# MingXiangL/AttentionShift

Measured on AMD Instinct MI355X. Metric: images/sec (1024^2, ViT-B) hot path: backbone attention fwd + attention-shift pseudo-labels, higher is better.
Workload: dtype bf16

## Files before the change

attentionshift_amd/_lib.py:

```python
import ctypes
import os

_HERE = os.path.dirname(os.path.abspath(__file__))
LIB_PATH = os.path.join(_HERE, "libattnshift_hip.so")

AS_F32, AS_BF16 = 0, 1

_c_void_p, _c_int, _c_float, _c_size_t = ctypes.c_void_p, ctypes.c_int, ctypes.c_float, ctypes.c_size_t
_c_double = ctypes.c_double

SIGNATURES = {
    "as_version": (_c_int, []),
    "as_last_error": (ctypes.c_char_p, []),
    "as_npad": (_c_int, [_c_int]),
    "as_linear_fwd": (_c_int, [_c_void_p] * 4 + [_c_int] * 5 + [_c_void_p]),
    "as_linear_small_fwd": (_c_int, [_c_void_p, _c_int, _c_void_p, _c_void_p, _c_void_p] + [_c_int] * 5 + [_c_void_p]),
    "as_linear_sk_workspace_bytes": (_c_size_t, [_c_int] * 3),
    "as_linear_sk_fwd": (_c_int, [_c_void_p] * 4 + [_c_int] * 5 + [_c_void_p, _c_size_t, _c_void_p]),
    "as_linear_gelu_fwd": (_c_int, [_c_void_p] * 5 + [_c_int] * 4 + [_c_void_p]),
    "as_linear_dgelu_fwd": (_c_int, [_c_void_p] * 4 + [_c_int] * 4 + [_c_void_p]),
    "as_deconv2x2_fwd": (_c_int, [_c_void_p] * 4 + [_c_int] * 6 + [_c_void_p]),
    "as_qkv_fwd": (_c_int, [_c_void_p] * 6 + [_c_int] * 5 + [_c_void_p]),
    "as_sdpa_fwd_workspace_bytes": (_c_size_t, [_c_int] * 4),
    "as_sdpa_fwd": (_c_int, [_c_void_p] * 6 + [_c_size_t] + [_c_int] * 4 + [_c_void_p]),
    "as_sdpa_bwd_workspace_bytes": (_c_size_t, [_c_int] * 4),
    "as_sdpa_bwd": (_c_int, [_c_void_p] * 8 + [_c_size_t] + [_c_int] * 4 + [_c_void_p]),
    "as_attn_bwd_workspace_bytes": (_c_size_t, [_c_int] * 5),
    "as_attn_bwd": (_c_int, [_c_void_p] * 15 + [_c_size_t] + [_c_int] * 5 + [_c_void_p]),
    "as_window_attn_fwd": (_c_int, [_c_void_p] * 5 + [_c_int] * 8 + [_c_void_p]),
    "as_add_layernorm_bwd_workspace_bytes": (_c_size_t, [_c_int] * 2),
    "as_add_layernorm_bwd": (_c_int, [_c_void_p] * 4 + [ctypes.c_float] + [_c_void_p] * 5 + [_c_size_t] + [_c_int] * 3 + [_c_void_p]),
    "as_add_layernorm": (_c_int, [_c_void_p] * 4 + [ctypes.c_float] + [_c_void_p] * 2 + [_c_int] * 3 + [_c_void_p]),
    "as_add_layernorm_scaled": (_c_int, [_c_void_p] * 4 + [ctypes.c_float] + [_c_void_p] * 2 + [_c_int] * 3 + [_c_void_p, _c_int, _c_void_p]),
    "as_add_layernorm_bwd_scaled": (_c_int, [_c_void_p] * 4 + [ctypes.c_float] + [_c_void_p] * 5 + [_c_size_t] + [_c_int] * 3
                                    + [_c_void_p, _c_int, _c_void_p]),
    "as_linear_splitk_workspace_bytes": (ctypes.c_size_t, [_c_int] * 3),
    "as_linear_splitk_fwd": (_c_int, [_c_void_p] * 3 + [_c_int] * 5 + [_c_void_p, ctypes.c_size_t, _c_void_p]),
    "as_linear_bwd_workspace_bytes": (ctypes.c_size_t, [_c_int] * 3),
    "as_linear_bwd": (_c_int, [_c_void_p] * 6 + [_c_int] * 5 + [_c_void_p, ctypes.c_size_t, _c_void_p]),
    "as_linear_bwd_dgelu": (_c_int, [_c_void_p] * 7 + [_c_int] * 5 + [_c_void_p, ctypes.c_size_t, _c_void_p]),
    "as_assemble_tokens": (_c_int, [_c_void_p] * 3 + [_c_int] * 5 + [_c_void_p]),
    "as_maxpool_nhwc": (_c_int, [_c_void_p] * 2 + [_c_int] * 5 + [ctypes.c_longlong, _c_void_p]),
    "as_mask_count": (_c_int, [_c_void_p] * 2 + [_c_int] * 2 + [_c_void_p]),
    "as_window_attn_bwd_workspace_bytes": (_c_size_t, [_c_int] * 5),
    "as_window_attn_bwd": (_c_int, [_c_void_p] * 8 + [_c_size_t] + [_c_int] * 8 + [_c_void_p]),
    "as_attn_fwd": (_c_int, [_c_void_p] * 12 + [_c_size_t] + [_c_int] * 5 + [_c_void_p]),
    "as_attn_mean_rows": (_c_int, [_c_void_p] * 4 + [_c_int] * 6 + [_c_void_p]),
    "as_rollout_rfrag_bytes": (_c_size_t, [_c_int] * 3),
    "as_rollout_pack": (_c_int, [_c_void_p] * 2 + [_c_int] * 4 + [_c_void_p]),
    "as_rollout_top": (_c_int, [_c_void_p] * 5 + [_c_int] * 5 + [_c_void_p]),
    "as_rollout_step_workspace_bytes": (_c_size_t, [_c_int] * 3),
    "as_rollout_step": (_c_int, [_c_void_p] * 8 + [_c_size_t] + [_c_int] * 5 + [_c_void_p]),
    "as_ccl_2d": (_c_int, [_c_void_p] * 2 + [_c_int] * 3 + [_c_void_p]),
    "as_cam_boxes_workspace_bytes": (_c_size_t, [_c_int] * 4),
    "as_cam_boxes": (_c_int, [_c_void_p] * 2 + [_c_float] * 2 + [_c_int] * 4 + [_c_void_p] * 5 + [_c_size_t, _c_void_p]),
    "as_cam_sample_masks_workspace_bytes": (_c_size_t, [_c_int] * 4),
    "as_cam_sample_masks": (_c_int, [_c_void_p] * 3 + [_c_int] * 4 + [_c_float] * 2 + [_c_void_p] * 3 + [_c_size_t, _c_void_p]),
    "as_mask_candidates_workspace_bytes": (_c_size_t, [_c_int] * 3),
    "as_mask_candidates": (_c_int, [_c_void_p] * 3 + [_c_float] * 3 + [_c_int] + [_c_void_p] * 5 + [_c_size_t]
                           + [_c_int] * 3 + [_c_void_p]),
    "as_part_select": (_c_int, [_c_void_p] * 7 + [_c_int] * 5 + [_c_void_p] * 8 + [_c_void_p]),
    "as_part_stats": (_c_int, [_c_void_p] * 3 + [_c_float] + [_c_void_p] * 4 + [_c_int] * 3 + [_c_void_p]),
    "as_filter_parts": (_c_int, [_c_void_p] * 2 + [_c_float] * 2 + [_c_void_p] + [_c_int] * 3 + [_c_void_p]),
    "as_draw_distinct": (_c_int, [_c_void_p, _c_int, _c_int] + [_c_void_p] * 5 + [_c_int] * 3 + [_c_void_p]),
    "as_mt_sample_ranks": (_c_int, [_c_void_p] * 4 + [_c_int] * 2 + [_c_void_p]),
    "as_mt_perm_ranks": (_c_int, [_c_void_p] * 4 + [_c_int] * 2 + [_c_void_p]),
    "as_small_attn_fwd": (_c_int, [_c_void_p] * 3 + [_c_int] * 5 + [_c_void_p]),
    "as_small_attn_bwd_workspace_bytes": (_c_size_t, [_c_int] * 3),
    "as_small_attn_bwd": (_c_int, [_c_void_p] * 6 + [_c_size_t] + [_c_int] * 5 + [_c_void_p]),
    "as_roi_align_fwd": (_c_int, [_c_void_p] * 3 + [_c_int] * 6 + [_c_float] + [_c_int] * 2 + [_c_void_p]),
    "as_roi_align_bwd": (_c_int, [_c_void_p] * 3 + [_c_int] * 6 + [_c_float] + [_c_int] * 2 + [_c_void_p]),
    "as_chamfer_2d_fwd": (_c_int, [_c_void_p] * 6 + [_c_int] * 3 + [_c_void_p]),
    "as_chamfer_2d_bwd": (_c_int, [_c_void_p] * 8 + [_c_int] * 3 + [_c_void_p]),
    "as_merge_plan": (_c_int, [_c_void_p] * 4 + [_c_int] * 2 + [_c_void_p]),
    "as_semantic_prestage": (_c_int, [_c_void_p, _c_float] + [_c_int] * 5 + [_c_void_p] * 4),
    "as_cosine_shift_workspace_bytes": (_c_size_t, [_c_int] * 6),
    "as_cosine_shift": (_c_int, [_c_void_p] * 5 + [_c_double] * 2 + [_c_int] + [_c_void_p] * 4 + [_c_size_t]
                        + [_c_int] * 6 + [_c_void_p]),
    "as_cosine_shift_strided": (_c_int, [_c_void_p, ctypes.c_longlong] + [_c_void_p] * 4 + [_c_double] * 2 + [_c_int] + [_c_void_p] * 4
                                + [_c_size_t] + [_c_int] * 6 + [_c_void_p]),
    "as_refine_similarity_workspace_bytes": (_c_size_t, [_c_int] * 3),
    "as_refine_similarity": (_c_int, [_c_void_p] * 3 + [_c_int] * 3 + [_c_float, _c_int] + [_c_void_p] * 3
                             + [_c_size_t] + [_c_int] * 3 + [_c_void_p]),
    "as_instance_maps_workspace_bytes": (_c_size_t, [_c_int] * 2),
    "as_crop_threshold_erode_workspace_bytes": (_c_size_t, [_c_int] * 3),
    "as_crop_threshold_erode": (_c_int, [_c_void_p] * 2 + [_c_float, _c_int, _c_int] + [_c_void_p] * 3 + [_c_size_t]
                                + [_c_int] * 3 + [_c_void_p]),
    "as_rank_select_workspace_bytes": (_c_size_t, [_c_int] * 2),
    "as_rank_select": (_c_int, [_c_void_p] * 4 + [_c_size_t] + [_c_int] * 3 + [_c_void_p]),
    "as_rank_select_xy": (_c_int, [_c_void_p] * 4 + [_c_size_t] + [_c_int] * 5 + [_c_void_p]),
    "as_merge_parts": (_c_int, [_c_void_p] * 2 + [_c_float] + [_c_void_p] * 3 + [_c_int] * 4 + [_c_void_p]),
    "as_select_median_boxes": (_c_int, [_c_void_p] * 2 + [_c_int] * 2 + [_c_void_p] * 8 + [_c_int, _c_void_p]),
    "as_rank_draw_xy": (_c_int, [_c_void_p, _c_int] + [_c_void_p] * 4 + [_c_int, _c_int, ctypes.c_int64, _c_int, _c_void_p, _c_size_t]
                        + [_c_int] * 5 + [_c_void_p]),
    "as_instance_maps": (_c_int, [_c_void_p] * 2 + [_c_int] * 6 + [_c_void_p] * 3 + [_c_size_t, _c_void_p]),
    "as_nms_workspace_bytes": (_c_size_t, [_c_int]),
    "as_nms": (_c_int, [_c_void_p, _c_int, _c_float, _c_int] + [_c_void_p] * 3 + [_c_size_t, _c_void_p]),
    "as_paste_masks": (_c_int, [_c_void_p] * 4 + [_c_int] * 8 + [_c_float, _c_void_p]),
    "as_rle_tile": (_c_int, [_c_void_p] * 2),
    "as_rle_workspace_bytes": (_c_size_t, [_c_int] * 3),
    "as_rle_count": (_c_int, [_c_void_p] + [_c_int] * 3 + [_c_void_p] * 2 + [_c_size_t, _c_void_p]),
    "as_rle_encode": (_c_int, [_c_void_p] + [_c_int] * 3 + [_c_void_p] * 2 + [_c_size_t, _c_void_p, _c_size_t, _c_void_p, _c_size_t,
                               _c_void_p, _c_void_p]),
    "as_rpn_candidates_workspace_bytes": (_c_size_t, [_c_int] * 2),
    "as_rpn_candidates": (_c_int, [_c_void_p] + [_c_int] * 3 + [_c_void_p] * 2 + [_c_int, _c_float, _c_void_p, _c_float, _c_int]
                          + [_c_void_p] * 7 + [_c_size_t, _c_void_p]),
    "as_rpn_assign_workspace_bytes": (_c_size_t, [_c_int] * 3),
    "as_rpn_assign": (_c_int, [_c_void_p] + [_c_int] * 3 + [_c_void_p] * 3 + [_c_int] * 2 + [_c_void_p] + [_c_float] * 3
                      + [_c_int] * 2 + [_c_void_p] * 4 + [_c_size_t, _c_void_p]),
    "as_rpn_sample": (_c_int, [_c_int] * 4 + [_c_void_p] * 4 + [_c_size_t, _c_void_p, _c_void_p]),
    "as_rpn_targets": (_c_int, [_c_void_p] + [_c_int] * 3 + [_c_void_p] * 3 + [_c_int] + [_c_void_p] * 2 + [_c_int] * 2
                       + [_c_void_p] * 3 + [_c_void_p]),
}


class RpnLevel(ctypes.Structure):
    _fields_ = [("cls", _c_void_p), ("reg", _c_void_p), ("H", _c_int), ("W", _c_int), ("stride_x", _c_int), ("stride_y", _c_int)]

_lib = None


class AttnShiftError(RuntimeError):
    pass


def load():
    global _lib
    if _lib is not None:
        return _lib
    if not os.path.exists(LIB_PATH):
        raise AttnShiftError(
            f"{LIB_PATH} is missing: build it with `python -m attentionshift_amd.csrc.build` "
            "(hipcc --offload-arch=gfx950).  There is no CPU fallback for the hot path.")
    lib = ctypes.CDLL(LIB_PATH)
    for name, (res, args) in SIGNATURES.items():
        fn = getattr(lib, name)
        fn.restype, fn.argtypes = res, args
    _lib = lib
    return lib


def check(rc, what):
    if rc != 0:
        msg = load().as_last_error()
        raise AttnShiftError(f"{what} failed (rc={rc}): {msg.decode() if msg else ''}")
```

attentionshift_amd/backbone.py:

```python
import math
import os

import torch
import torch.nn as nn
import torch.nn.functional as F

from . import ops
from .registry import BACKBONES


def trunc_normal_(tensor, std=0.02):
    return nn.init.trunc_normal_(tensor, std=std, a=-2 * std, b=2 * std)


class Mlp(nn.Module):
    def __init__(self, dim, hidden):
        super().__init__()
        self.fc1 = nn.Linear(dim, hidden)
        self.fc2 = nn.Linear(hidden, dim)


class Attention(nn.Module):
    def __init__(self, dim, num_heads, qkv_bias):
        super().__init__()
        self.num_heads = num_heads
        self.qkv = nn.Linear(dim, dim * 3, bias=qkv_bias)
        self.proj = nn.Linear(dim, dim)


class Block(nn.Module):

    def __init__(self, dim, num_heads, mlp_ratio, qkv_bias, eps):
        super().__init__()
        self.norm1 = nn.LayerNorm(dim, eps=eps)
        self.attn = Attention(dim, num_heads, qkv_bias)
        self.norm2 = nn.LayerNorm(dim, eps=eps)
        self.mlp = Mlp(dim, int(dim * mlp_ratio))


class PatchEmbed(nn.Module):
    def __init__(self, img_size, patch_size, in_chans, embed_dim):
        super().__init__()
        if isinstance(img_size, int):
            img_size = [img_size, img_size]
        self.num_patches = (img_size[0] // patch_size) * (img_size[1] // patch_size)
        self.patch_size = patch_size
        self.proj = nn.Conv2d(in_chans, embed_dim, kernel_size=patch_size, stride=patch_size)


class MLP(nn.Module):

    def __init__(self, input_dim, hidden_dim, output_dim, num_layers):
        super().__init__()
        self.num_layers = num_layers
        h = [hidden_dim] * (num_layers - 1)
        self.layers = nn.ModuleList(nn.Linear(n, k) for n, k in zip([input_dim] + h, h + [output_dim]))

    def forward(self, x):
        for i, layer in enumerate(self.layers):
            x = F.relu(layer(x)) if i < self.num_layers - 1 else layer(x)
        return x


class DeferredFPN:

    def __init__(self, backbone, features, taps):
        self._bb, self._features, self._taps = backbone, list(features), list(taps)
        self._out, self._event, self._joined = None, None, False

    def launch(self):
        if self._out is not None:
            return self
        bb = self._bb
        main = torch.cuda.current_stream()
        if bb._fpn_stream is None:
            bb._fpn_stream = torch.cuda.Stream()
        side = bb._fpn_stream
        side.wait_stream(main)
        with torch.cuda.stream(side):
            for t in self._features + self._taps:
                t.record_stream(side)
            self._out = tuple(bb._fpn(i, self._features[i], self._taps[i]) for i in range(len(self._features)))
            self._event = side.record_event()
        return self

    def result(self):
        self.launch()
        if not self._joined:
            main = torch.cuda.current_stream()
            main.wait_event(self._event)
            for t in self._out:
                t.record_stream(main)
            self._joined = True
            self._features, self._taps = [], []
        return self._out

    def __len__(self):
        return len(self._features) if self._out is None else len(self._out)

    def __iter__(self):
        return iter(self.result())

    def __getitem__(self, i):
        return self.result()[i]


@BACKBONES.register_module()
class VisionTransformerDet(nn.Module):
    def __init__(self, img_size, patch_size, embed_dim, in_chans=3, with_fpn=True, frozen_stages=-1,
                 out_indices=(3, 5, 7, 11), use_checkpoint=False, learnable_pos_embed=True, last_feat=False,
                 recompute_last_feat=False, point_tokens_num=100, num_classes=20, return_attention=False,
                 with_point_head=True, depth=12, num_heads=12, mlp_ratio=4., qkv_bias=False, qk_scale=None,
                 drop_rate=0., attn_drop_rate=0., drop_path_rate=0., norm_eps=1e-6, init_values=0,
                 compute_dtype=torch.bfloat16, **unused):
        super().__init__()
        assert not with_fpn or patch_size in (8, 16)
        assert not recompute_last_feat or last_feat
        if qk_scale is not None or attn_drop_rate or drop_rate or init_values:
            raise NotImplementedError("qk_scale / dropout / layer-scale are unused by every reference config")
        if embed_dim != num_heads * ops.HEAD_DIM:
            raise NotImplementedError(f"head dim must be {ops.HEAD_DIM}")
        self.embed_dim = self.num_features = embed_dim
        self.patch_size, self.depth, self.num_heads = patch_size, depth, num_heads
        self.last_feat, self.recompute_last_feat = last_feat, recompute_last_feat
        self.with_fpn, self.frozen_stages = with_fpn, frozen_stages
        self.out_indices = tuple(out_indices)
        self.use_checkpoint = use_checkpoint
        self.drop_path_rate = drop_path_rate
        self.return_attention = return_attention
        self.point_tokens_num = point_tokens_num
        self.with_point_head = with_point_head
        self.compute_dtype = compute_dtype
        self.defer_fpn = bool(unused.pop("defer_fpn", False))
        self._fpn_stream = None
        self._point_pack = None
        self.point_head_stream = bool(unused.pop("point_head_stream", False))
        self._point_stream = None

        self.patch_embed = PatchEmbed(img_size, patch_size, in_chans, embed_dim)
        n_patches = self.patch_embed.num_patches
        self.cls_token = nn.Parameter(torch.zeros(1, 1, embed_dim))
        self.pos_embed = nn.Parameter(torch.zeros(1, n_patches + 1, embed_dim), requires_grad=learnable_pos_embed)
        self.blocks = nn.ModuleList(Block(embed_dim, num_heads, mlp_ratio, qkv_bias, norm_eps) for _ in range(depth))
        if with_fpn and patch_size == 16:
            self.fpn1 = nn.Sequential(nn.ConvTranspose2d(embed_dim, embed_dim, 2, 2), nn.BatchNorm2d(embed_dim), nn.GELU(),
                                      nn.ConvTranspose2d(embed_dim, embed_dim, 2, 2))
            self.fpn2 = nn.Sequential(nn.ConvTranspose2d(embed_dim, embed_dim, 2, 2))
            self.fpn3 = nn.Identity()
            self.fpn4 = nn.MaxPool2d(2, 2)
        elif with_fpn and patch_size == 8:
            self.fpn1 = nn.Sequential(nn.ConvTranspose2d(embed_dim, embed_dim, 2, 2))
            self.fpn2 = nn.Identity()
            self.fpn3 = nn.Sequential(nn.MaxPool2d(2, 2))
            self.fpn4 = nn.Sequential(nn.MaxPool2d(4, 4))
        self.point_token = nn.Parameter(torch.zeros(1, point_tokens_num, embed_dim))
        self.point_pos_embed = nn.Parameter(torch.zeros(1, point_tokens_num, embed_dim))
        if with_point_head:
            self.class_embed = MLP(embed_dim, embed_dim, num_classes, 3)
            self.bbox_embed = MLP(embed_dim, embed_dim, 2, 3)
        trunc_normal_(self.pos_embed)
        trunc_normal_(self.cls_token)
        trunc_normal_(self.point_token)
        trunc_normal_(self.point_pos_embed)
        self.apply(self._init_weights)
        self._wcache = {}

    @staticmethod
    def _init_weights(m):
        if isinstance(m, nn.Linear):
            trunc_normal_(m.weight)
            if m.bias is not None:
                nn.init.constant_(m.bias, 0)
        elif isinstance(m, nn.LayerNorm):
            nn.init.constant_(m.bias, 0)
            nn.init.constant_(m.weight, 1.0)

    def init_weights(self, pretrained=None):
        if pretrained is not None and not isinstance(pretrained, str):
            raise TypeError("pretrained must be a str or None")
        self.apply(self._init_weights)
        if isinstance(pretrained, str):
            import os
            if os.path.isfile(pretrained):
                from .checkpoint import load_checkpoint
                load_checkpoint(self, pretrained, strict=False)
            else:
                print(f"checkpoint path {pretrained} is invalid, we skip it and initialize net randomly")
        self.invalidate_cache()

    def train(self, mode=True):
        super().train(mode)
        self._freeze_stages()
        return self

    def _freeze_stages(self):
        if self.frozen_stages >= 0:
            self.patch_embed.eval()
            for p in self.patch_embed.parameters():
                p.requires_grad = False
            self.cls_token.requires_grad = False
            self.pos_embed.requires_grad = False
        for i in range(1, self.frozen_stages + 1):
            m = self.blocks[i - 1]
            m.eval()
            for p in m.parameters():
                p.requires_grad = False

    def invalidate_cache(self):
        self._wcache = {}

    def _w(self, p):
        if p.dtype == self.compute_dtype:
            return p
        if torch.is_grad_enabled() and p.requires_grad:
            return p.to(self.compute_dtype)
        key = id(p)
        hit = self._wcache.get(key)
        if hit is None or hit[0] != p._version or hit[1].device != p.device:
            hit = (p._version, p.detach().to(self.compute_dtype).contiguous())
            self._wcache[key] = hit
        return hit[1]

    def _derived(self, p, tag, fn):
        if torch.is_grad_enabled() and p.requires_grad:
            return fn(p).to(self.compute_dtype).contiguous()
        key = (id(p), tag)
        hit = self._wcache.get(key)
        if hit is None or hit[0] != p._version or hit[1].device != p.device:
            hit = (p._version, fn(p.detach()).to(self.compute_dtype).contiguous())
            self._wcache[key] = hit
        return hit[1]

    def _deconv2x2(self, x_nhwc, conv, bn=None, act="none"):
        B, h, w, cin = x_nhwc.shape
        cout = conv.weight.shape[1]
        srcs = [conv.weight, conv.bias] + ([bn.weight, bn.bias, bn.running_mean, bn.running_var] if bn is not None else [])
        stamp = tuple(-1 if t is None else t._version for t in srcs) + (x_nhwc.device,)
        key = (id(conv), "deconv")
        hit = self._wcache.get(key)
        if hit is None or hit[0] != stamp:
            with torch.no_grad():
                wmat = conv.weight.detach().float().permute(2, 3, 1, 0).reshape(4 * cout, cin)
                bias = torch.zeros(cout, device=wmat.device) if conv.bias is None else conv.bias.detach().float()
                if bn is not None:
                    scale = bn.weight.detach().float() * torch.rsqrt(bn.running_var.float() + bn.eps)
                    wmat = wmat * scale.repeat(4)[:, None]
                    bias = (bias - bn.running_mean.float()) * scale + bn.bias.detach().float()
                hit = (stamp, wmat.to(self.compute_dtype).contiguous(), bias.repeat(4).contiguous())
            self._wcache[key] = hit
        _, wmat, bias4 = hit
        if x_nhwc.is_cuda and self.compute_dtype == torch.bfloat16 and cin % 32 == 0 and cout % 8 == 0:
            return ops.deconv2x2(x_nhwc.contiguous(), wmat, bias4, act=act)
        y = ops.linear(x_nhwc.reshape(B * h * w, cin), wmat, bias4, act=act)
        return y.reshape(B, h, w, 2, 2, cout).permute(0, 1, 3, 2, 4, 5).reshape(B, 2 * h, 2 * w, cout)

    def _deconv2x2_train(self, x_nhwc, conv):
        B, h, w, cin = x_nhwc.shape
        cout = conv.weight.shape[1]
        cd = self.compute_dtype
        from .autograd import linear_in
        wmat = conv.weight.permute(2, 3, 1, 0).reshape(4 * cout, cin)
        bias = None if conv.bias is None else conv.bias.repeat(4)
        y = linear_in(x_nhwc.reshape(B * h * w, cin), wmat, bias, cd)
        return y.reshape(B, h, w, 2, 2, cout).permute(0, 1, 3, 2, 4, 5).reshape(B, 2 * h, 2 * w, cout)

    def _fpn_train(self, i, feat_nchw, tok):
        B, D, hp, wp = feat_nchw.shape
        op = [self.fpn1, self.fpn2, self.fpn3, self.fpn4][i]
        if isinstance(op, nn.Sequential) and isinstance(op[0], nn.ConvTranspose2d):
            y = self._deconv2x2_train(tok.to(self.compute_dtype).reshape(B, hp, wp, D), op[0]).permute(0, 3, 1, 2)
            if len(op) == 4:
                y = op[2](op[1](y.float())).to(self.compute_dtype)
                y = self._deconv2x2_train(y.permute(0, 2, 3, 1), op[3]).permute(0, 3, 1, 2)
            return y
        return op(feat_nchw)

    def _fpn(self, i, feat_nchw, tok):
        B, D, hp, wp = feat_nchw.shape
        ops_ = [self.fpn1, self.fpn2, self.fpn3, self.fpn4]
        op = ops_[i]
        if isinstance(op, nn.Sequential) and isinstance(op[0], nn.ConvTranspose2d):
            x0 = tok.to(self.compute_dtype).reshape(B, hp, wp, D)
            if len(op) == 4:
                bn = op[1]
                if isinstance(bn, nn.modules.batchnorm._BatchNorm) and not bn.training and bn.running_mean is not None \
                        and isinstance(op[2], nn.GELU) and getattr(op[2], "approximate", "none") == "none":
                    y = self._deconv2x2(x0, op[0], bn=bn, act="gelu")
                else:
                    y = self._deconv2x2(x0, op[0]).permute(0, 3, 1, 2)
                    y = op[2](op[1](y.float())).to(self.compute_dtype).permute(0, 2, 3, 1)
                return self._deconv2x2(y, op[3]).permute(0, 3, 1, 2)
            return self._deconv2x2(x0, op[0]).permute(0, 3, 1, 2)
        pool = op[0] if isinstance(op, nn.Sequential) and len(op) == 1 else op
        if isinstance(pool, nn.MaxPool2d) and tok.is_cuda and tok.dtype == torch.float32 and tok.stride()[1:] == (D, 1):
            k = pool.kernel_size if isinstance(pool.kernel_size, int) else pool.kernel_size[0]
            s_ = pool.stride if isinstance(pool.stride, int) else pool.stride[0]
            if k == s_ and pool.padding in (0, (0, 0)) and not pool.ceil_mode and hp % k == 0 and wp % k == 0 and D % 4 == 0:
                return ops.maxpool_nhwc(tok.reshape(B, hp, wp, D), k).permute(0, 3, 1, 2)
        return op(feat_nchw)

    def _point_head_packable(self, x):
        ls = list(self.class_embed.layers) + list(self.bbox_embed.layers)
        return (len(self.class_embed.layers) == 3 and len(self.bbox_embed.layers) == 3 and hasattr(torch, "_addmm_activation")
                and all(l.weight.dtype == x.dtype and l.bias is not None for l in ls)
                and self.class_embed.layers[0].in_features == self.bbox_embed.layers[0].in_features)

    def _point_head_packed(self, x):
        c, b = self.class_embed.layers, self.bbox_embed.layers
        key = tuple((t.data_ptr(), t._version) for t in (c[0].weight, c[0].bias, b[0].weight, b[0].bias))
        pk = self._point_pack
        if pk is None or pk["key"] != key:
            with torch.no_grad():
                w1 = torch.cat((c[0].weight, b[0].weight)).contiguous()
                pk = dict(key=key, w1=w1, w1t=w1.t().contiguous(), b1=torch.cat((c[0].bias, b[0].bias)))
            self._point_pack = pk
        B, T, D = x.shape
        hc = c[0].out_features
        x2 = x.reshape(B * T, D)
        if ops.linear_small_applies(x2, pk["w1"]) and hc % 16 == 0 and hc >= 64:
            h1 = ops.linear_small(x2, pk["w1"], pk["b1"], act="relu")
            h2c = ops.linear_small(h1[:, :hc], c[1].weight, c[1].bias, act="relu")
            h2b = ops.linear_small(h1[:, hc:], b[1].weight, b[1].bias, act="relu")
            cls = ops.linear_small(h2c, c[2].weight, c[2].bias).reshape(B, T, -1)
            reg = ops.linear_small(h2b, b[2].weight, b[2].bias, act="sigmoid").reshape(B, T, -1)
            return cls, reg
        h1 = torch._addmm_activation(pk["b1"], x2, pk["w1t"])
        h2c = torch._addmm_activation(c[1].bias, h1[:, :hc], c[1].weight.t())
        h2b = torch._addmm_activation(b[1].bias, h1[:, hc:], b[1].weight.t())
        cls = torch.addmm(c[2].bias, h2c, c[2].weight.t()).reshape(B, T, -1)
        reg = torch.addmm(b[2].bias, h2b, b[2].weight.t()).reshape(B, T, -1).sigmoid()
        return cls, reg

    def interpolate_pos_encoding(self, n_patch_tokens, w, h):
        n0 = self.pos_embed.shape[1] - 1
        if n_patch_tokens == n0 and w == h:
            return self.pos_embed
        dim = self.pos_embed.shape[-1]
        w0, h0 = w // self.patch_size + 0.1, h // self.patch_size + 0.1
        s = int(math.sqrt(n0))
        grid = self.pos_embed[:, 1:].reshape(1, s, s, dim).permute(0, 3, 1, 2)
        grid = F.interpolate(grid, scale_factor=(w0 / math.sqrt(n0), h0 / math.sqrt(n0)), mode="bicubic")
        assert int(w0) == grid.shape[-2] and int(h0) == grid.shape[-1]
        return torch.cat((self.pos_embed[:, :1], grid.permute(0, 2, 3, 1).reshape(1, -1, dim)), dim=1)

    def prepare_tokens(self, img):
        B, C, w, h = img.shape
        ps = self.patch_size
        hp, wp = w // ps, h // ps
        patches = torch.empty(B, hp, wp, C, ps, ps, device=img.device, dtype=self.compute_dtype)
        patches.copy_(img.reshape(B, C, hp, ps, wp, ps).permute(0, 2, 4, 1, 3, 5))
        wmat = self._derived(self.patch_embed.proj.weight, "patch", lambda t: t.reshape(self.embed_dim, -1))
        emb = ops.linear(patches.view(B, hp * wp, C * ps * ps), wmat, self.patch_embed.proj.bias.float())
        return ops.assemble_tokens(emb, self._token_table(hp * wp, w, h))

    def _token_table(self, Np, w, h):
        srcs = (self.pos_embed, self.cls_token, self.point_token, self.point_pos_embed)
        stamp = tuple(t._version for t in srcs) + (Np, w, h, self.pos_embed.device)
        hit = self._wcache.get("token_table")
        if hit is None or hit[0] != stamp:
            with torch.no_grad():
                pos = self.interpolate_pos_encoding(Np, w, h)
                table = torch.cat((self.cls_token + pos[:, :1], pos[:, 1:], self.point_token + self.point_pos_embed), dim=1)
            hit = (stamp, table[0].float().contiguous())
            self._wcache["token_table"] = hit
        return hit[1]

    def _block(self, blk, x, delta, keep_state, need_x, on_full=None, full_out=None, x_out=None):
        cd = self.compute_dtype
        x, y = ops.add_layernorm(x, delta, blk.norm1.weight, blk.norm1.bias, blk.norm1.eps, cd,
                                 x_out=full_out if delta is not None else None)
        if on_full is not None:
            on_full(x)
        a, st = ops.attention_fwd(y, self._w(blk.attn.qkv.weight),
                                  None if blk.attn.qkv.bias is None else blk.attn.qkv.bias.float(),
                                  self._w(blk.attn.proj.weight), blk.attn.proj.bias.float(), self.num_heads,
                                  keep_state=keep_state)
        x, z = ops.add_layernorm(x, a, blk.norm2.weight, blk.norm2.bias, blk.norm2.eps, cd)
        z = ops.linear(z, self._w(blk.mlp.fc1.weight), blk.mlp.fc1.bias.float(), act="gelu")
        z = ops.linear(z, self._w(blk.mlp.fc2.weight), blk.mlp.fc2.bias.float())
        if need_x:
            x, _ = ops.add_layernorm(x, z, None, None, 0.0, cd, want_y=False, x_out=x_out)
            z = None
        return x, z, st

    def _grad_path(self):
        return torch.is_grad_enabled() and self.training and any(p.requires_grad for p in self.blocks.parameters())

    def _drop_path(self, x, i):
        rate = self.drop_path_rate * i / max(self.depth - 1, 1)
        if rate == 0.0 or not self.training:
            return x
        keep = 1.0 - rate
        mask = torch.rand(x.shape[0], 1, 1, device=x.device, dtype=x.dtype).add_(keep).floor_()
        return x / keep * mask

    def _drop_scale(self, batch, i, device):
        rate = self.drop_path_rate * i / max(self.depth - 1, 1)
        if rate == 0.0 or not self.training:
            return None
        keep = 1.0 - rate
        return torch.rand(batch, device=device, dtype=torch.float32).add_(keep).floor_().div_(keep)

    def _prepare_tokens_train(self, img):
        B, C, w, h = img.shape
        ps = self.patch_size
        hp, wp = w // ps, h // ps
        cd = self.compute_dtype
        patches = img.reshape(B, C, hp, ps, wp, ps).permute(0, 2, 4, 1, 3, 5).reshape(B, hp * wp, C * ps * ps)
        from .autograd import linear_in
        x = linear_in(patches.to(cd), self.patch_embed.proj.weight.reshape(self.embed_dim, -1), self.patch_embed.proj.bias,
                      cd).float()
        x = torch.cat((self.cls_token.expand(B, -1, -1), x), dim=1)
        x = x + self.interpolate_pos_encoding(x.shape[1] - 1, w, h)
        pt = (self.point_token + self.point_pos_embed).expand(B, -1, -1)
        return torch.cat((x, pt), dim=1)

    def _block_train(self, blk, x, delta, i, sink, delta_scale=None):
        from . import autograd as AG
        cd = self.compute_dtype
        sh = self._train_shadow
        w = lambda p: sh[id(p)] if id(p) in sh else p.to(cd)
        x, y = AG.add_layernorm(x, delta, blk.norm1.weight, blk.norm1.bias, blk.norm1.eps, cd, delta_scale)
        a = AG.attention(y, w(blk.attn.qkv.weight), None if blk.attn.qkv.bias is None else blk.attn.qkv.bias.float(),
                         w(blk.attn.proj.weight), blk.attn.proj.bias.float(), self.num_heads, sink)
        x, z = AG.add_layernorm(x, a, blk.norm2.weight, blk.norm2.bias, blk.norm2.eps, cd, self._drop_scale(x.shape[0], i, x.device))
        if AG.mlp_applies(z, w(blk.mlp.fc1.weight), w(blk.mlp.fc2.weight)):
            z = AG.mlp(z, w(blk.mlp.fc1.weight), blk.mlp.fc1.bias, w(blk.mlp.fc2.weight), blk.mlp.fc2.bias)
        elif AG.linear_applies(z, w(blk.mlp.fc1.weight)):
            z = F.gelu(AG.linear(z, w(blk.mlp.fc1.weight), blk.mlp.fc1.bias))
            z = AG.linear(z, w(blk.mlp.fc2.weight), blk.mlp.fc2.bias)
        else:
            z = F.gelu(F.linear(z, w(blk.mlp.fc1.weight), w(blk.mlp.fc1.bias)))
            z = F.linear(z, w(blk.mlp.fc2.weight), w(blk.mlp.fc2.bias))
        return x, z, self._drop_scale(x.shape[0], i, x.device)

    def forward(self, x):
        B, _, H, W = x.shape
        hp, wp = H // self.patch_size, W // self.patch_size
        T = self.point_tokens_num
        grad_path = self._grad_path()
        x = self._prepare_tokens_train(x) if grad_path else self.prepare_tokens(x)
        if self.recompute_last_feat:
            last_feat = x
        features, taps, attns = [], [], []
        store = []
        delta = None
        dscale = None
        if not grad_path:
            x = x.contiguous()

        def take_tap(xf):
            taps.append(xf[:, 1:-T])
            tap = xf[:, 1:, :][:, :-T].permute(0, 2, 1).unflatten(2, (hp, wp))
            if grad_path:
                features.append(tap if os.environ.get("AS_TAP_VIEW", "1") != "0" else tap.contiguous())
                return
            if xf.data_ptr() != tap_slot(len(features)).data_ptr():
                tap_slot(len(features)).copy_(xf)
            features.append(store[0][len(features)][:, 1:-T].unflatten(1, (hp, wp)).permute(0, 3, 1, 2))

        def tap_slot(k):
            if not store:
                store.append(torch.empty(len(self.out_indices), *x.shape, device=x.device, dtype=torch.float32))
            return store[0][k]

        tap_due = False
        nblk = len(self.blocks)
        self._train_shadow = {}
        if grad_path and self.compute_dtype != torch.float32 and not os.environ.get("AS_NO_PARAM_SHADOW"):
            from .autograd import cast_params
            from . import autograd as _AG
            lib_mlp = _AG._LIBRARY_LINEAR or self.embed_dim % 32 != 0
            ps = []
            for blk in self.blocks:
                ps += [blk.attn.qkv.weight, blk.attn.proj.weight, blk.mlp.fc1.weight, blk.mlp.fc2.weight]
                if lib_mlp:
                    ps += [blk.mlp.fc1.bias, blk.mlp.fc2.bias]
            self._train_shadow = cast_params([p for p in ps if p.dtype != self.compute_dtype], self.compute_dtype)
        for i, blk in enumerate(self.blocks):
            if grad_path:
                sink = [] if self.return_attention else None
                x, delta, dscale = self._block_train(blk, x.float() if x.dtype != torch.float32 else x, delta, i, sink, dscale)
                if i in self.out_indices or i == nblk - 1:
                    x = x + (delta if dscale is None else delta * dscale[:, None, None])
                    delta, dscale = None, None
                st = sink[0] if sink else None
                if i in self.out_indices:
                    take_tap(x)
            else:
                last_tap = i in self.out_indices and i == nblk - 1
                x, delta, st = self._block(blk, x, delta, self.return_attention, i == nblk - 1,
                                           take_tap if tap_due else None,
                                           full_out=tap_slot(len(features)) if tap_due and x.dtype == torch.float32 else None,
                                           x_out=tap_slot(len(features) + int(tap_due)) if last_tap and x.dtype == torch.float32
                                           else None)
                tap_due = i in self.out_indices and i != nblk - 1
                if i in self.out_indices and i == nblk - 1:
                    take_tap(x)
            if self.return_attention:
                attns.append(st)
            if self.last_feat and not self.recompute_last_feat and i == nblk - 1:
                last_feat = x[:, :-T]
        self._train_shadow = {}
        org_features = store[0][:, :, 1:-T].unflatten(2, (hp, wp)).permute(1, 0, 4, 2, 3) if store else None
        if org_features is None:
            org_features = torch.stack(features, dim=1)
        if self.with_fpn and grad_path:
            features = [self._fpn_train(i, features[i], taps[i]) for i in range(len(features))]
        elif self.with_fpn and self.defer_fpn and x.is_cuda:
            features = DeferredFPN(self, features, taps)
        elif self.with_fpn:
            features = [self._fpn(i, features[i], taps[i]) for i in range(len(features))]
        point_tokens = x[:, -T:]
        out = dict(org_feats=org_features, feature=features if isinstance(features, DeferredFPN) else tuple(features),
                   point_tokens=point_tokens)
        if self.with_point_head and not grad_path and point_tokens.is_cuda and self._point_head_packable(point_tokens):
            if self.point_head_stream:
                if self._point_stream is None:
                    self._point_stream = torch.cuda.Stream()
                main = torch.cuda.current_stream()
                self._point_stream.wait_stream(main)
                with torch.cuda.stream(self._point_stream):
                    cls, reg = self._point_head_packed(point_tokens)
                    out["point_head_ready"] = self._point_stream.record_event()
                for t in (point_tokens, cls, reg):
                    t.record_stream(main)
                    t.record_stream(self._point_stream)
            else:
                cls, reg = self._point_head_packed(point_tokens)
            out.update(outputs_class=cls, outputs_coord=reg)
        elif self.with_point_head:
            out.update(outputs_class=self.class_embed(point_tokens), outputs_coord=self.bbox_embed(point_tokens).sigmoid())
        if self.return_attention and self.last_feat:
            out.update(attns=attns)
        if self.last_feat:
            out.update(last_feat=last_feat)
        return out
```

attentionshift_amd/csrc/layernorm.hip:

```cpp
#include "common.h"

namespace {

template <typename T, int VPL>
__global__ __launch_bounds__(256) void add_layernorm_kernel(const float* __restrict__ x_in, const T* __restrict__ delta,
                                                            const float* __restrict__ gamma, const float* __restrict__ beta,
                                                            float* __restrict__ x_out, T* __restrict__ y_out, int M, int D,
                                                            float eps, const float* __restrict__ dscale, int rps) {
  const int row = blockIdx.x * 4 + (threadIdx.x >> 6), lane = threadIdx.x & 63;
  if (row >= M) return;
  const size_t base = (size_t)row * D;
  const float ds = dscale != nullptr ? dscale[row / rps] : 1.0f;
  float v[VPL][4];
  float s = 0.0f;
#pragma unroll
  for (int i = 0; i < VPL; ++i) {
    const int c = (i * 64 + lane) * 4;
    if (c < D) {
      const float4 a = *reinterpret_cast<const float4*>(x_in + base + c);
      v[i][0] = a.x; v[i][1] = a.y; v[i][2] = a.z; v[i][3] = a.w;
      if (delta != nullptr) {
#pragma unroll
        for (int t = 0; t < 4; ++t) v[i][t] = dscale != nullptr ? fmaf(ds, to_f32<T>(delta[base + c + t]), v[i][t])
                                                                     : v[i][t] + to_f32<T>(delta[base + c + t]);
      }
      s += (v[i][0] + v[i][1]) + (v[i][2] + v[i][3]);
    } else {
      v[i][0] = v[i][1] = v[i][2] = v[i][3] = 0.0f;
    }
  }
  const float mean = wave_sum(s) / (float)D;
  float q = 0.0f;
#pragma unroll
  for (int i = 0; i < VPL; ++i) {
    const int c = (i * 64 + lane) * 4;
    if (c < D) {
#pragma unroll
      for (int t = 0; t < 4; ++t) {
        const float d = v[i][t] - mean;
        q = fmaf(d, d, q);
      }
    }
  }
  const float rstd = rsqrtf(wave_sum(q) / (float)D + eps);
#pragma unroll
  for (int i = 0; i < VPL; ++i) {
    const int c = (i * 64 + lane) * 4;
    if (c < D) {
      if (x_out != nullptr) *reinterpret_cast<float4*>(x_out + base + c) = make_float4(v[i][0], v[i][1], v[i][2], v[i][3]);
      if (y_out != nullptr) {
        const float4 g = *reinterpret_cast<const float4*>(gamma + c);
        const float4 b = *reinterpret_cast<const float4*>(beta + c);
        const float y0 = (v[i][0] - mean) * rstd * g.x + b.x, y1 = (v[i][1] - mean) * rstd * g.y + b.y;
        const float y2 = (v[i][2] - mean) * rstd * g.z + b.z, y3 = (v[i][3] - mean) * rstd * g.w + b.w;
        T* yp = y_out + base + c;
        yp[0] = from_f32<T>(y0); yp[1] = from_f32<T>(y1); yp[2] = from_f32<T>(y2); yp[3] = from_f32<T>(y3);
      }
    }
  }
}

template <typename T>
int launch_add_ln(const float* x_in, const void* delta, const float* gamma, const float* beta, float* x_out, void* y_out,
                  int M, int D, float eps, const float* dscale, int rps, hipStream_t s) {
  const int vpl = as_ceil_div(D, 256);
  dim3 grid(as_ceil_div(M, 4));
#define AS_LN(V)                                                                                                   \
  hipLaunchKernelGGL((add_layernorm_kernel<T, V>), grid, dim3(256), 0, s, x_in, (const T*)delta, gamma, beta, x_out, \
                     (T*)y_out, M, D, eps, dscale, rps)
  switch (vpl) {
    case 1: AS_LN(1); break;
    case 2: AS_LN(2); break;
    case 3: AS_LN(3); break;
    case 4: AS_LN(4); break;
    case 5: AS_LN(5); break;
    case 6: AS_LN(6); break;
    case 7: AS_LN(7); break;
    case 8: AS_LN(8); break;
    case 9: case 10: AS_LN(10); break;
    case 11: case 12: AS_LN(12); break;
    default: AS_REQUIRE(false, AS_E_UNSUPPORTED, "as_add_layernorm: D=%d (max 3072)", D);
  }
#undef AS_LN
  AS_CHECK_LAUNCH("add_layernorm");
  return AS_OK;
}

}

namespace {

template <typename T, int VPL>
__global__ __launch_bounds__(256) void add_layernorm_bwd_kernel(const float* __restrict__ x, const T* __restrict__ dy,
                                                                const float* __restrict__ dx_res,
                                                                const float* __restrict__ gamma, float* __restrict__ dx_out,
                                                                T* __restrict__ ddelta_out, float* __restrict__ part, int M,
                                                                int D, float eps, const float* __restrict__ dscale, int rps) {
  __shared__ float red[2][4][VPL * 256];
  const int wave = threadIdx.x >> 6, lane = threadIdx.x & 63;
  float dg[VPL][4], db[VPL][4], gm[VPL][4];
#pragma unroll
  for (int i = 0; i < VPL; ++i) {
    const int c = (i * 64 + lane) * 4;
#pragma unroll
    for (int t = 0; t < 4; ++t) { dg[i][t] = 0.0f; db[i][t] = 0.0f; gm[i][t] = (gamma != nullptr && c < D) ? gamma[c + t] : 1.0f; }
  }
  for (int row = blockIdx.x * 4 + wave; row < M; row += gridDim.x * 4) {
    const size_t base = (size_t)row * D;
    float v[VPL][4], g[VPL][4];
    float s = 0.0f;
#pragma unroll
    for (int i = 0; i < VPL; ++i) {
      const int c = (i * 64 + lane) * 4;
      if (c < D) {
        const float4 a = *reinterpret_cast<const float4*>(x + base + c);
        v[i][0] = a.x; v[i][1] = a.y; v[i][2] = a.z; v[i][3] = a.w;
        if (dy == nullptr) {
#pragma unroll
          for (int t = 0; t < 4; ++t) g[i][t] = 0.0f;
        } else if constexpr (sizeof(T) == 2) {
          const bf16x4 d4 = *reinterpret_cast<const bf16x4*>(dy + base + c);
#pragma unroll
          for (int t = 0; t < 4; ++t) g[i][t] = (float)d4[t];
        } else {
          const float4 d4 = *reinterpret_cast<const float4*>(dy + base + c);
          g[i][0] = d4.x; g[i][1] = d4.y; g[i][2] = d4.z; g[i][3] = d4.w;
        }
        s += (v[i][0] + v[i][1]) + (v[i][2] + v[i][3]);
      } else {
#pragma unroll
        for (int t = 0; t < 4; ++t) { v[i][t] = 0.0f; g[i][t] = 0.0f; }
      }
    }
    const float mean = wave_sum(s) / (float)D;
    float q = 0.0f;
#pragma unroll
    for (int i = 0; i < VPL; ++i) {
      const int c = (i * 64 + lane) * 4;
      if (c < D) {
#pragma unroll
        for (int t = 0; t < 4; ++t) { const float d = v[i][t] - mean; q = fmaf(d, d, q); }
      }
    }
    const float rstd = rsqrtf(wave_sum(q) / (float)D + eps);
    float sg = 0.0f, sgx = 0.0f;
#pragma unroll
    for (int i = 0; i < VPL; ++i) {
      const int c = (i * 64 + lane) * 4;
      if (c < D) {
#pragma unroll
        for (int t = 0; t < 4; ++t) {
          const float xh = (v[i][t] - mean) * rstd;
          dg[i][t] = fmaf(g[i][t], xh, dg[i][t]);
          db[i][t] += g[i][t];
          const float gg = g[i][t] * gm[i][t];
          g[i][t] = gg;
          v[i][t] = xh;
          sg += gg;
          sgx = fmaf(gg, xh, sgx);
        }
      }
    }
    const float mg = wave_sum(sg) / (float)D, mgx = wave_sum(sgx) / (float)D;
#pragma unroll
    for (int i = 0; i < VPL; ++i) {
      const int c = (i * 64 + lane) * 4;
      if (c < D) {
        float o[4];
        float4 r4 = make_float4(0.0f, 0.0f, 0.0f, 0.0f);
        if (dx_res != nullptr) r4 = *reinterpret_cast<const float4*>(dx_res + base + c);
        const float r[4] = {r4.x, r4.y, r4.z, r4.w};
#pragma unroll
        for (int t = 0; t < 4; ++t) {
          o[t] = rstd * (g[i][t] - mg - v[i][t] * mgx);
          if (dx_res != nullptr) o[t] += r[t];
        }
        if (dx_out != nullptr) *reinterpret_cast<float4*>(dx_out + base + c) = make_float4(o[0], o[1], o[2], o[3]);
        if (ddelta_out != nullptr) {
          const float ds = dscale != nullptr ? dscale[row / rps] : 1.0f;
          if constexpr (sizeof(T) == 2) {
            bf16x4 w4;
#pragma unroll
            for (int t = 0; t < 4; ++t) w4[t] = (__bf16)(ds * o[t]);
            *reinterpret_cast<bf16x4*>(ddelta_out + base + c) = w4;
          } else {
            *reinterpret_cast<float4*>(ddelta_out + base + c) = make_float4(ds * o[0], ds * o[1], ds * o[2], ds * o[3]);
          }
        }
      }
    }
  }
#pragma unroll
  for (int i = 0; i < VPL; ++i)
#pragma unroll
    for (int t = 0; t < 4; ++t) {
      red[0][wave][(i * 64 + lane) * 4 + t] = dg[i][t];
      red[1][wave][(i * 64 + lane) * 4 + t] = db[i][t];
    }
  __syncthreads();
  for (int c = threadIdx.x; c < D; c += 256) {
    part[((size_t)blockIdx.x * 2 + 0) * D + c] = ((red[0][0][c] + red[0][1][c]) + red[0][2][c]) + red[0][3][c];
    part[((size_t)blockIdx.x * 2 + 1) * D + c] = ((red[1][0][c] + red[1][1][c]) + red[1][2][c]) + red[1][3][c];
  }
}

__global__ __launch_bounds__(1024) void add_layernorm_bwd_reduce_kernel(const float* __restrict__ part,
                                                                        float* __restrict__ dgamma, float* __restrict__ dbeta,
                                                                        int nblk, int D) {
  __shared__ float red[16][64];
  const int cl = threadIdx.x & 63, grp = threadIdx.x >> 6, c = blockIdx.x * 64 + cl, which = blockIdx.y;
  float a0 = 0.0f, a1 = 0.0f, a2 = 0.0f, a3 = 0.0f;
  if (c < D) {
    int i = grp;
    for (; i + 48 < nblk; i += 64) {
      a0 += part[((size_t)i * 2 + which) * D + c];
      a1 += part[((size_t)(i + 16) * 2 + which) * D + c];
      a2 += part[((size_t)(i + 32) * 2 + which) * D + c];
      a3 += part[((size_t)(i + 48) * 2 + which) * D + c];
    }
    for (; i < nblk; i += 16) a0 += part[((size_t)i * 2 + which) * D + c];
  }
  red[grp][cl] = (a0 + a1) + (a2 + a3);
  __syncthreads();
  if (grp != 0 || c >= D) return;
  float t = 0.0f;
#pragma unroll
  for (int g = 0; g < 16; ++g) t += red[g][cl];
  float* dst = which == 0 ? dgamma : dbeta;
  if (dst != nullptr) dst[c] = t;
}

constexpr int LNB_BLOCKS = 1024;

template <typename T>
int launch_add_ln_bwd(const float* x, const void* dy, const float* dx_res, const float* gamma, float* dx_out, void* ddelta,
                      float* dgamma, float* dbeta, float* part, int M, int D, float eps, const float* dscale, int rps,
                      hipStream_t s) {
  const int vpl = as_ceil_div(D, 256);
  const int nblk = as_ceil_div(M, 4) < LNB_BLOCKS ? as_ceil_div(M, 4) : LNB_BLOCKS;
#define AS_LNB(V)                                                                                                    \
  hipLaunchKernelGGL((add_layernorm_bwd_kernel<T, V>), dim3(nblk), dim3(256), 0, s, x, (const T*)dy, dx_res, gamma, dx_out, \
                     (T*)ddelta, part, M, D, eps, dscale, rps)
  switch (vpl) {
    case 1: AS_LNB(1); break;
    case 2: AS_LNB(2); break;
    case 3: AS_LNB(3); break;
    case 4: AS_LNB(4); break;
    case 5: AS_LNB(5); break;
    case 6: AS_LNB(6); break;
    case 7: AS_LNB(7); break;
    case 8: AS_LNB(8); break;
    default: AS_REQUIRE(false, AS_E_UNSUPPORTED, "as_add_layernorm_bwd: D=%d (max 2048)", D);
  }
#undef AS_LNB
  AS_CHECK_LAUNCH("add_layernorm_bwd");
  if (dgamma != nullptr || dbeta != nullptr) {
    hipLaunchKernelGGL(add_layernorm_bwd_reduce_kernel, dim3(as_ceil_div(D, 64), 2), dim3(1024), 0, s, (const float*)part,
                       dgamma, dbeta, nblk, D);
    AS_CHECK_LAUNCH("add_layernorm_bwd_reduce");
  }
  return AS_OK;
}

}

extern "C" size_t as_add_layernorm_bwd_workspace_bytes(int M, int D) {
  if (M <= 0 || D <= 0) return 0;
  return (size_t)LNB_BLOCKS * 2 * D * sizeof(float);
}

extern "C" int as_add_layernorm_bwd(const float* x, const void* dy, const float* dx_res, const float* gamma, float eps,
                                    float* dx_out, void* ddelta_out, float* dgamma, float* dbeta, void* workspace,
                                    size_t workspace_bytes, int M, int D, int dtype, as_stream_t stream) {
  return as_add_layernorm_bwd_scaled(x, dy, dx_res, gamma, eps, dx_out, ddelta_out, dgamma, dbeta, workspace, workspace_bytes,
                                     M, D, dtype, nullptr, 1, stream);
}

extern "C" int as_add_layernorm_bwd_scaled(const float* x, const void* dy, const float* dx_res, const float* gamma, float eps,
                                           float* dx_out, void* ddelta_out, float* dgamma, float* dbeta, void* workspace,
                                           size_t workspace_bytes, int M, int D, int dtype, const float* delta_scale,
                                           int rows_per_scale, as_stream_t stream) {
  AS_REQUIRE(x && (dy || dx_res) && (dx_out || ddelta_out) && workspace, AS_E_BADARG, "as_add_layernorm_bwd: null pointer");
  AS_REQUIRE(rows_per_scale > 0, AS_E_BADARG, "as_add_layernorm_bwd: rows_per_scale must be positive");
  AS_REQUIRE(M > 0 && D > 0 && D % 4 == 0, AS_E_BADARG, "as_add_layernorm_bwd: need M > 0 and D %% 4 == 0 (D=%d)", D);
  AS_REQUIRE(workspace_bytes >= as_add_layernorm_bwd_workspace_bytes(M, D), AS_E_WORKSPACE,
             "as_add_layernorm_bwd: workspace too small");
  hipStream_t s = (hipStream_t)stream;
  if (dtype == AS_BF16)
    return launch_add_ln_bwd<__bf16>(x, dy, dx_res, gamma, dx_out, ddelta_out, dgamma, dbeta, (float*)workspace, M, D, eps,
                                     delta_scale, rows_per_scale, s);
  if (dtype == AS_F32)
    return launch_add_ln_bwd<float>(x, dy, dx_res, gamma, dx_out, ddelta_out, dgamma, dbeta, (float*)workspace, M, D, eps,
                                    delta_scale, rows_per_scale, s);
  AS_REQUIRE(false, AS_E_UNSUPPORTED, "as_add_layernorm_bwd: dtype %d", dtype);
}

extern "C" int as_add_layernorm(const float* x_in, const void* delta, const float* gamma, const float* beta, float eps,
                                float* x_out, void* y_out, int M, int D, int dtype, as_stream_t stream) {
  return as_add_layernorm_scaled(x_in, delta, gamma, beta, eps, x_out, y_out, M, D, dtype, nullptr, 1, stream);
}

extern "C" int as_add_layernorm_scaled(const float* x_in, const void* delta, const float* gamma, const float* beta, float eps,
                                       float* x_out, void* y_out, int M, int D, int dtype, const float* delta_scale,
                                       int rows_per_scale, as_stream_t stream) {
  AS_REQUIRE(x_in && (x_out || y_out), AS_E_BADARG, "as_add_layernorm: null pointer");
  AS_REQUIRE(rows_per_scale > 0 && (!delta_scale || delta), AS_E_BADARG, "as_add_layernorm: delta_scale needs delta, rows_per_scale > 0");
  AS_REQUIRE(!y_out || (gamma && beta), AS_E_BADARG, "as_add_layernorm: y_out needs gamma and beta");
  AS_REQUIRE(M > 0 && D > 0 && D % 4 == 0, AS_E_BADARG, "as_add_layernorm: need M > 0 and D %% 4 == 0 (D=%d)", D);
  hipStream_t s = (hipStream_t)stream;
  if (dtype == AS_BF16) return launch_add_ln<__bf16>(x_in, delta, gamma, beta, x_out, y_out, M, D, eps, delta_scale, rows_per_scale, s);
  if (dtype == AS_F32) return launch_add_ln<float>(x_in, delta, gamma, beta, x_out, y_out, M, D, eps, delta_scale, rows_per_scale, s);
  AS_REQUIRE(false, AS_E_UNSUPPORTED, "as_add_layernorm: dtype %d", dtype);
}


namespace {
__global__ __launch_bounds__(256) void maxpool_nhwc_kernel(const float* __restrict__ x, float* __restrict__ out, int B, int H,
                                                           int W, int C, int k, size_t xbs) {
  const int Ho = H / k, Wo = W / k, C4 = C >> 2;
  const size_t total = (size_t)B * Ho * Wo * C4;
  for (size_t i = (size_t)blockIdx.x * blockDim.x + threadIdx.x; i < total; i += (size_t)gridDim.x * blockDim.x) {
    const int c4 = (int)(i % C4);
    size_t r = i / C4;
    const int ow = (int)(r % Wo);
    r /= Wo;
    const int oh = (int)(r % Ho), b = (int)(r / Ho);
    const float* src = x + (size_t)b * xbs + (((size_t)oh * k) * W + (size_t)ow * k) * C + c4 * 4;
    float4 m = *reinterpret_cast<const float4*>(src);
    for (int dy = 0; dy < k; ++dy)
      for (int dx = 0; dx < k; ++dx) {
        const float4 v = *reinterpret_cast<const float4*>(src + ((size_t)dy * W + dx) * C);
        m.x = (v.x > m.x || v.x != v.x) ? v.x : m.x; m.y = (v.y > m.y || v.y != v.y) ? v.y : m.y;
        m.z = (v.z > m.z || v.z != v.z) ? v.z : m.z; m.w = (v.w > m.w || v.w != v.w) ? v.w : m.w;
      }
    *reinterpret_cast<float4*>(out + i * 4) = m;
  }
}
}

extern "C" int as_maxpool_nhwc(const float* x, float* out, int B, int H, int W, int C, int k, long long x_batch_stride,
                               as_stream_t stream) {
  AS_REQUIRE(x && out, AS_E_BADARG, "as_maxpool_nhwc: null pointer");
  AS_REQUIRE(B > 0 && H > 0 && W > 0 && C > 0 && k > 0, AS_E_BADARG, "as_maxpool_nhwc: bad sizes");
  AS_REQUIRE(x_batch_stride >= (long long)H * W * C && x_batch_stride % 4 == 0, AS_E_BADARG,
             "as_maxpool_nhwc: batch stride %lld (elements) must be >= H*W*C and a multiple of 4", x_batch_stride);
  AS_REQUIRE(C % 4 == 0 && H % k == 0 && W % k == 0, AS_E_UNSUPPORTED,
             "as_maxpool_nhwc: C %% 4 == 0 and H, W multiples of k only (C=%d H=%d W=%d k=%d)", C, H, W, k);
  const size_t total = (size_t)B * (H / k) * (W / k) * (C / 4);
  const int grid = (int)((total + 255) / 256 < 4096 ? (total + 255) / 256 : 4096);
  hipLaunchKernelGGL(maxpool_nhwc_kernel, dim3(grid), dim3(256), 0, (hipStream_t)stream, x, out, B, H, W, C, k,
                     (size_t)x_batch_stride);
  AS_CHECK_LAUNCH("maxpool_nhwc");
  return AS_OK;
}

namespace {
template <typename T>
__global__ __launch_bounds__(256) void assemble_tokens_kernel(const T* __restrict__ emb, const float* __restrict__ table,
                                                              float* __restrict__ out, int B, int Np, int N, int D) {
  const int D4 = D >> 2;
  const size_t total = (size_t)B * N * D4;
  for (size_t i = (size_t)blockIdx.x * blockDim.x + threadIdx.x; i < total; i += (size_t)gridDim.x * blockDim.x) {
    const int c = (int)(i % D4) * 4;
    const size_t r = i / D4;
    const int n = (int)(r % N), b = (int)(r / N);
    float4 v = *reinterpret_cast<const float4*>(table + (size_t)n * D + c);
    if (n >= 1 && n <= Np) {
      const T* e = emb + ((size_t)b * Np + (n - 1)) * D + c;
      if (sizeof(T) == 2) {
        const bf16x4 e4 = *reinterpret_cast<const bf16x4*>(e);
        v.x = (float)e4[0] + v.x; v.y = (float)e4[1] + v.y; v.z = (float)e4[2] + v.z; v.w = (float)e4[3] + v.w;
      } else {
        const float4 e4 = *reinterpret_cast<const float4*>(e);
        v.x = e4.x + v.x; v.y = e4.y + v.y; v.z = e4.z + v.z; v.w = e4.w + v.w;
      }
    }
    *reinterpret_cast<float4*>(out + i * 4) = v;
  }
}
}

extern "C" int as_assemble_tokens(const void* emb, const float* table, float* out, int B, int Np, int N, int D, int dtype,
                                  as_stream_t stream) {
  AS_REQUIRE(emb && table && out, AS_E_BADARG, "as_assemble_tokens: null pointer");
  AS_REQUIRE(B > 0 && Np > 0 && N > Np && D > 0 && D % 4 == 0, AS_E_BADARG, "as_assemble_tokens: B=%d Np=%d N=%d D=%d", B, Np, N, D);
  const size_t total = (size_t)B * N * (D / 4);
  const int grid = (int)((total + 255) / 256 < 8192 ? (total + 255) / 256 : 8192);
  if (dtype == AS_BF16)
    hipLaunchKernelGGL(assemble_tokens_kernel<__bf16>, dim3(grid), dim3(256), 0, (hipStream_t)stream, (const __bf16*)emb, table, out,
                       B, Np, N, D);
  else if (dtype == AS_F32)
    hipLaunchKernelGGL(assemble_tokens_kernel<float>, dim3(grid), dim3(256), 0, (hipStream_t)stream, (const float*)emb, table, out,
                       B, Np, N, D);
  else
    AS_REQUIRE(false, AS_E_UNSUPPORTED, "as_assemble_tokens: dtype %d", dtype);
  AS_CHECK_LAUNCH("assemble_tokens");
  return AS_OK;
}
```

attentionshift_amd/csrc/rollout.hip:

```cpp
#include <stdlib.h>
#include "common.h"
#include "lds_asm.h"

namespace {

constexpr int HD = 64, RO_NT = 256;
constexpr float LOG2E = 1.44269504088896340736f;

template <typename T> struct KjCfg { static constexpr int PITCH = HD * (int)sizeof(T) + 16; };

__device__ __forceinline__ size_t rf_slot(int b, int nkb, int i, int k) {
  const int rem = k & 31, s2 = rem >> 4, r16 = rem & 15;
  const int lane = (i & 31) + 32 * ((r16 & 7) >> 2), t = (r16 >> 3) * 4 + (r16 & 3);
  return ((((((size_t)b * nkb + (k >> 5)) * 4 + (i >> 5)) * 2 + s2) * 64) + lane) * 8 + t;
}
__device__ __forceinline__ size_t rf_frag(int b, int nkb, int kb, int ib, int s2, int lane) {
  return ((((((size_t)b * nkb + kb) * 4 + ib) * 2 + s2) * 64) + lane) * 8;
}

template <typename T>
__device__ __forceinline__ f32x16 pbar_tile(const T* __restrict__ q, const T* __restrict__ k,
                                            const float* __restrict__ lse, const char* kj_lds, int b, int h,
                                            int N, int Npad, int i0, int j0, int li, int half) {
  f32x16 pbar;
#pragma unroll
  for (int r = 0; r < 16; ++r) pbar[r] = 0.0f;
  const int irow = min(i0 + li, N - 1);
  const int jrow = min(j0 + li, N - 1);
  for (int hh = 0; hh < h; ++hh) {
    const size_t bh = (size_t)b * h + hh;
    f32x16 s;
#pragma unroll
    for (int r = 0; r < 16; ++r) s[r] = 0.0f;
#pragma unroll
    for (int ks = 0; ks < 4; ++ks) {
      Frag<T> fa, fb;
      fa.load16B(q + qf_frag(bh, Npad, irow, ks, half));
      if (kj_lds != nullptr)
        fb.load16B(reinterpret_cast<const T*>(kj_lds + ((size_t)hh * 32 + li) * KjCfg<T>::PITCH) + ks * 16 + half * 8);
      else
        fb.load16B(k + (bh * Npad + jrow) * HD + ks * 16 + half * 8);
      s = mma32(fa, fb, s);
    }
    const float* lrow = lse + bh * N;
#pragma unroll
    for (int r = 0; r < 16; ++r) {
      const int row = min(i0 + acc_row(r, half), N - 1);
      pbar[r] += __builtin_amdgcn_exp2f(s[r] - lrow[row] * LOG2E);
    }
  }
  const float inv_h = 1.0f / (float)h;
#pragma unroll
  for (int r = 0; r < 16; ++r) pbar[r] *= inv_h;
  return pbar;
}

template <typename T, bool TOP>
__global__ __launch_bounds__(RO_NT) void attn_mean_rows_kernel(const T* __restrict__ q, const T* __restrict__ k,
                                                               const float* __restrict__ lse,
                                                               float* __restrict__ out, T* __restrict__ rf_out, int B,
                                                               int N, int Npad, int h, int row0, int nrows) {
  const int lane = threadIdx.x & 63, wave = threadIdx.x >> 6;
  const int li = lane & 31, half = lane >> 5;
  const int jb = blockIdx.x * 4 + wave, ib = blockIdx.y, b = blockIdx.z;
  const int j0 = jb * 32, i0 = ib * 32;
  if (j0 >= N) return;
  const f32x16 p = pbar_tile<T>(q, k, lse, nullptr, b, h, N, Npad, row0 + i0, j0, li, half);
  const int j = j0 + li;
  const int nkb = (N + 31) / 32;
#pragma unroll
  for (int r = 0; r < 16; ++r) {
    const int i = i0 + acc_row(r, half);
    float v = p[r];
    if (TOP) v = 0.5f * (v + ((row0 + i) == j ? 1.0f : 0.0f));
    const bool live = i < nrows && j < N;
    if (live) out[((size_t)b * nrows + i) * N + j] = v;
    if (rf_out != nullptr && i < 128) rf_out[rf_slot(b, nkb, i, j)] = from_f32<T>(live ? v : 0.0f);
  }
}

template <typename T> struct Kj2 {
  static constexpr int PITCH = sizeof(T) == 2 ? 128 : (HD * 4 + 16);
  __device__ static __forceinline__ int off(int row, int elem) {
    if (sizeof(T) == 2) return row * 128 + ((((elem >> 3) ^ (row & 7))) << 4);
    return row * PITCH + elem * 4;
  }
};

template <typename T, int HPW>
__global__ __launch_bounds__(RO_NT) void rollout_step2_kernel(const T* __restrict__ q, const T* __restrict__ k,
                                                              const float* __restrict__ lse,
                                                              const float* __restrict__ Rin, const T* __restrict__ rf_in,
                                                              float* __restrict__ Rout, T* __restrict__ rf_out,
                                                              float* __restrict__ part, int B, int N, int Npad, int h,
                                                              int Trows, int nsplit, int xbufs) {
  extern __shared__ __attribute__((aligned(16))) char smem[];
  constexpr bool PREFETCH = sizeof(T) == 2;
  const int tid = threadIdx.x, lane = tid & 63, wave = tid >> 6;
  const int li = lane & 31, half = lane >> 5;
  const int j0 = blockIdx.x * 32, b = blockIdx.y, split = blockIdx.z;
  char* kj = smem;
  float4* xchg = reinterpret_cast<float4*>(smem + (size_t)h * 32 * Kj2<T>::PITCH);

  {
    constexpr int CPR = HD * (int)sizeof(T) / 16;
    const int total = h * 32 * CPR;
    for (int c = tid; c < total; c += RO_NT) {
      const int hh = c / (32 * CPR), rem = c % (32 * CPR);
      const int jr = rem / CPR, ch = rem % CPR;
      const int jrow = min(j0 + jr, N - 1);
      const uint4 u = *reinterpret_cast<const uint4*>(
          reinterpret_cast<const char*>(k + (((size_t)b * h + hh) * Npad + jrow) * HD) + ch * 16);
      const int elem = ch * (16 / (int)sizeof(T));
      const int base = Kj2<T>::off(hh * 32 + jr, elem & ~7);
      *reinterpret_cast<uint4*>(kj + base + (elem & 7) * (int)sizeof(T)) = u;
    }
  }
  __syncthreads();

  const int nkb = (N + 31) / 32;
  const float inv_h = 1.0f / (float)h;
  const bool own_rows = wave * 32 < Trows;

  f32x16 acc;
#pragma unroll
  for (int r = 0; r < 16; ++r) acc[r] = 0.0f;

  struct Fetch {
    Frag<T> fq[HPW][4];
    float l8[HPW];
    Frag<T> fr[2];
  };
  auto fetch = [&](int kb, Fetch& f) {
    const int row = min(kb * 32 + li, N - 1);
#pragma unroll
    for (int t = 0; t < HPW; ++t) {
      const int hh = min(wave + 4 * t, h - 1);
#pragma unroll
      for (int ks = 0; ks < 4; ++ks) f.fq[t][ks].load16B(q + qf_frag((size_t)b * h + hh, Npad, row, ks, half));
      f.l8[t] = -LOG2E * lse[((size_t)b * h + hh) * N + row];
    }
    if (own_rows) {
#pragma unroll
      for (int s2 = 0; s2 < 2; ++s2) f.fr[s2].load16B(rf_in + rf_frag(b, nkb, kb, wave, s2, lane));
    }
  };
  const int kb0 = (int)((long long)nkb * split / nsplit), kb1 = (int)((long long)nkb * (split + 1) / nsplit);
  Fetch cur, nxt;
  if (PREFETCH && kb0 < kb1) fetch(kb0, nxt);

  for (int kb = kb0; kb < kb1; ++kb) {
    const int k0 = kb * 32;
    if (PREFETCH) {
      cur = nxt;
      if (kb + 1 < kb1) fetch(kb + 1, nxt);
    } else {
      fetch(kb, cur);
    }

    f32x16 pbar;
#pragma unroll
    for (int r = 0; r < 16; ++r) pbar[r] = 0.0f;
#pragma unroll
    for (int t = 0; t < HPW; ++t) {
      const int hh = wave + 4 * t;
      if (hh < h) {
        const float l8 = cur.l8[t];
        f32x16 sc;
#pragma unroll
        for (int r = 0; r < 16; ++r) sc[r] = 0.0f;
        sc = __builtin_amdgcn_mfma_f32_32x32x2f32(half == 0 ? l8 : 0.0f, 1.0f, sc, 0, 0, 0);
#pragma unroll
        for (int ks = 0; ks < 4; ++ks) {
          Frag<T> fk;
          fk.load16B(reinterpret_cast<const T*>(kj + Kj2<T>::off(hh * 32 + li, ks * 16 + half * 8)));
          sc = mma32(cur.fq[t][ks], fk, sc);
        }
#pragma unroll
        for (int r = 0; r < 16; ++r) pbar[r] += __builtin_amdgcn_exp2f(sc[r]);
      }
    }
    float4* slab = xchg + (size_t)(xbufs == 2 ? (kb - kb0) & 1 : 0) * 4 * 4 * 64;
#pragma unroll
    for (int g = 0; g < 4; ++g)
      slab[(wave * 4 + g) * 64 + lane] = make_float4(pbar[4 * g], pbar[4 * g + 1], pbar[4 * g + 2], pbar[4 * g + 3]);
    __syncthreads();
    if (own_rows) {
      Frag<T> fp[2];
#pragma unroll
      for (int g = 0; g < 4; ++g) {
        float4 v = slab[(0 * 4 + g) * 64 + lane];
#pragma unroll
        for (int w = 1; w < 4; ++w) {
          const float4 u = slab[(w * 4 + g) * 64 + lane];
          v.x += u.x; v.y += u.y; v.z += u.z; v.w += u.w;
        }
        const float e[4] = {v.x, v.y, v.z, v.w};
#pragma unroll
        for (int x = 0; x < 4; ++x) {
          const int r = 4 * g + x;
          const bool live = k0 + acc_row(r, half) < N;
          fp[r >> 3].set(r & 7, live ? e[x] * inv_h : 0.0f);
        }
      }
#pragma unroll
      for (int s2 = 0; s2 < 2; ++s2) acc = mma32(cur.fr[s2], fp[s2], acc);
    }
    if (xbufs == 1) __syncthreads();
  }

  if (own_rows) {
    const int j = j0 + li;
#pragma unroll
    for (int r = 0; r < 16; ++r) {
      const int i = wave * 32 + acc_row(r, half);
      const bool live = i < Trows && j < N;
      if (nsplit > 1) {
        if (live) part[(((size_t)split * B + b) * Trows + i) * N + j] = acc[r];
        continue;
      }
      float v = 0.0f;
      if (live) {
        const size_t idx = ((size_t)b * Trows + i) * N + j;
        v = 0.5f * (acc[r] + Rin[idx]);
        Rout[idx] = v;
      }
      if (rf_out != nullptr) rf_out[rf_slot(b, nkb, i, j)] = from_f32<T>(v);
    }
  }
}

#ifndef AS_ROLLOUT_ABLATE
#define AS_ROLLOUT_ABLATE 0
#endif
template <typename T> __device__ __forceinline__ f32x16 inject_rows(float x, int half);
template <> __device__ __forceinline__ f32x16 inject_rows<float>(float x, int half) {
  f32x16 z;
#pragma unroll
  for (int r = 0; r < 16; ++r) z[r] = 0.0f;
  return __builtin_amdgcn_mfma_f32_32x32x2f32(half == 0 ? x : 0.0f, 1.0f, z, 0, 0, 0);
}
template <> __device__ __forceinline__ f32x16 inject_rows<__bf16>(float x, int half) {
  f32x16 z;
#pragma unroll
  for (int r = 0; r < 16; ++r) z[r] = 0.0f;
  x = half == 0 ? x : 0.0f;
  const __bf16 hi = (__bf16)x;
  const float r1 = x - (float)hi;
  const __bf16 mid = (__bf16)r1;
  const __bf16 lo = (__bf16)(r1 - (float)mid);
  const __bf16 zero = (__bf16)0.0f, one = (__bf16)1.0f;
  Frag<__bf16> fa, fb;
  fa.v = bf16x8{hi, mid, lo, zero, zero, zero, zero, zero};
  fb.v = bf16x8{one, one, one, zero, zero, zero, zero, zero};
  return mma32(fa, fb, z);
}

template <typename T>
__global__ __launch_bounds__(RO_NT, 3) void rollout_step3_kernel(const T* __restrict__ q, const T* __restrict__ k,
                                                                 const float* __restrict__ lse,
                                                                 const float* __restrict__ Rin, const T* __restrict__ rf_in,
                                                                 float* __restrict__ Rout, T* __restrict__ rf_out,
                                                                 float* __restrict__ part, int B, int N, int Npad, int h,
                                                                 int Trows, int nsplit) {
  extern __shared__ __attribute__((aligned(16))) char smem[];
  const int tid = threadIdx.x, lane = tid & 63, wave = tid >> 6;
  const int li = lane & 31, half = lane >> 5;
  const int j0 = blockIdx.x * 32, b = blockIdx.y, split = blockIdx.z;
  char* kj = smem;
  {
    constexpr int CPR = HD * (int)sizeof(T) / 16;
    const int total = h * 32 * CPR;
    for (int c = tid; c < total; c += RO_NT) {
      const int hh = c / (32 * CPR), rem = c % (32 * CPR);
      const int jr = rem / CPR, ch = rem % CPR;
      const int jrow = min(j0 + jr, N - 1);
      const uint4 u = *reinterpret_cast<const uint4*>(
          reinterpret_cast<const char*>(k + (((size_t)b * h + hh) * Npad + jrow) * HD) + ch * 16);
      const int elem = ch * (16 / (int)sizeof(T));
      const int base = Kj2<T>::off(hh * 32 + jr, elem & ~7);
      *reinterpret_cast<uint4*>(kj + base + (elem & 7) * (int)sizeof(T)) = u;
    }
  }
  __syncthreads();

  const int nkb = (N + 31) / 32;
  const int nib = (Trows + 31) / 32;
  const float inv_h = 1.0f / (float)h;
  const int kb0 = (int)((long long)nkb * split / nsplit), kb1 = (int)((long long)nkb * (split + 1) / nsplit);

  f32x16 acc[4];
#pragma unroll
  for (int ib = 0; ib < 4; ++ib)
#pragma unroll
    for (int r = 0; r < 16; ++r) acc[ib][r] = 0.0f;

  for (int kb = kb0 + wave; kb < kb1; kb += 4) {
    const int k0 = kb * 32;
    const int row = min(k0 + li, N - 1);
    Frag<T> fq[4];
    float l8;
#pragma unroll
    for (int ks = 0; ks < 4; ++ks) fq[ks].load16B(q + qf_frag((size_t)b * h, Npad, row, ks, half));
    l8 = -LOG2E * lse[((size_t)b * h) * N + row];
    f32x16 pbar;
#pragma unroll
    for (int r = 0; r < 16; ++r) pbar[r] = 0.0f;
    auto head = [&](int hh) {
      f32x16 sc = inject_rows<T>(AS_ROLLOUT_ABLATE == 3 ? 0.0f : l8, half);
#pragma unroll
      for (int ks = 0; ks < 4; ++ks) {
        Frag<T> fk;
        fk.load16B(reinterpret_cast<const T*>(kj + Kj2<T>::off(hh * 32 + li, ks * 16 + half * 8)));
        if (AS_ROLLOUT_ABLATE != 4) sc = mma32(fq[ks], fk, sc);
        else sc[ks] += (float)fk.v[0];
      }
#pragma unroll
      for (int r = 0; r < 16; ++r) pbar[r] += AS_ROLLOUT_ABLATE == 2 ? sc[r] : __builtin_amdgcn_exp2f(sc[r]);
    };
    for (int hh = 0; hh + 1 < h; ++hh) {
      Frag<T> fn[4];
#pragma unroll
      for (int ks = 0; ks < 4; ++ks) {
        if (AS_ROLLOUT_ABLATE == 1) fn[ks] = fq[ks];
        else fn[ks].load16B(q + qf_frag((size_t)b * h + hh + 1, Npad, row, ks, half));
      }
      const float l8n = AS_ROLLOUT_ABLATE == 1 ? l8 : -LOG2E * lse[((size_t)b * h + hh + 1) * N + row];
      head(hh);
#pragma unroll
      for (int ks = 0; ks < 4; ++ks) fq[ks] = fn[ks];
      l8 = l8n;
    }
    Frag<T> fr[4][2];
#pragma unroll
    for (int ib = 0; ib < 4; ++ib) {
      const int ibc = min(ib, nib - 1);
#pragma unroll
      for (int s2 = 0; s2 < 2; ++s2) fr[ib][s2].load16B(rf_in + rf_frag(b, nkb, kb, ibc, s2, lane));
    }
    head(h - 1);
    Frag<T> fp[2];
#pragma unroll
    for (int r = 0; r < 16; ++r) {
      const bool live = k0 + acc_row(r, half) < N;
      fp[r >> 3].set(r & 7, live ? pbar[r] * inv_h : 0.0f);
    }
#pragma unroll
    for (int ib = 0; ib < 4; ++ib)
      if (ib < nib) {
#pragma unroll
        for (int s2 = 0; s2 < 2; ++s2) acc[ib] = mma32(fr[ib][s2], fp[s2], acc[ib]);
      }
  }

  float* red = reinterpret_cast<float*>(smem);
  f32x16 mine;
#pragma unroll
  for (int r = 0; r < 16; ++r) mine[r] = 0.0f;
#pragma unroll
  for (int pass = 0; pass < 2; ++pass) {
    __syncthreads();
#pragma unroll
    for (int x = 0; x < 2; ++x)
#pragma unroll
      for (int r = 0; r < 16; ++r) red[((wave * 2 + x) * 16 + r) * 64 + lane] = acc[pass * 2 + x][r];
    __syncthreads();
    if ((wave >> 1) == pass) {
      const int x = wave & 1;
#pragma unroll
      for (int r = 0; r < 16; ++r)
        mine[r] = ((red[((0 * 2 + x) * 16 + r) * 64 + lane] + red[((1 * 2 + x) * 16 + r) * 64 + lane]) +
                   red[((2 * 2 + x) * 16 + r) * 64 + lane]) + red[((3 * 2 + x) * 16 + r) * 64 + lane];
    }
  }
  if (wave * 32 < Trows) {
    const int j = j0 + li;
#pragma unroll
    for (int r = 0; r < 16; ++r) {
      const int i = wave * 32 + acc_row(r, half);
      const bool live = i < Trows && j < N;
      if (nsplit > 1) {
        if (live) part[(((size_t)split * B + b) * Trows + i) * N + j] = mine[r];
        continue;
      }
      float v = 0.0f;
      if (live) {
        const size_t idx = ((size_t)b * Trows + i) * N + j;
        v = 0.5f * (mine[r] + Rin[idx]);
        Rout[idx] = v;
      }
      if (rf_out != nullptr) rf_out[rf_slot(b, nkb, i, j)] = from_f32<T>(v);
    }
  }
}

constexpr int R4_HPG = 4;
constexpr int R4_QBYTES = R4_HPG * 4 * 1024;
constexpr int R4_LSE = R4_QBYTES + 8 * 1024;
constexpr int R4_STAGE = R4_LSE + 1024;
#ifndef AS_R4_OCC1
#define AS_R4_OCC1 3
#endif
template <int NIB> struct R4Cfg { static constexpr int NSTAGE = NIB == 1 ? 2 : 3, OCC = NIB == 1 ? AS_R4_OCC1 : 2; };


template <int NIB>
__global__ __launch_bounds__(RO_NT, R4Cfg<NIB>::OCC) void rollout_step4_kernel(const __bf16* __restrict__ q, const __bf16* __restrict__ k,
                                                                 const float* __restrict__ lse, const __bf16* __restrict__ rf_in,
                                                                 float* __restrict__ part, int B, int N, int Npad, int h,
                                                                 int Trows, int ksplit) {
  extern __shared__ __attribute__((aligned(16))) char smem[];
  constexpr int R4_NSTAGE = R4Cfg<NIB>::NSTAGE;
  const int tid = threadIdx.x, lane = tid & 63, wave = __builtin_amdgcn_readfirstlane(tid >> 6);
  const int li = lane & 31, half = lane >> 5;
  const int ngroups = h / R4_HPG;
  const int j0 = blockIdx.x * 128 + wave * 32, b = blockIdx.y;
  const int hg = blockIdx.z % ngroups, split = blockIdx.z / ngroups;
  const int nkb = (N + 31) / 32;
  const int nib = min((Trows + 31) / 32, NIB);
  const int kb0 = (int)((long long)nkb * split / ksplit), kb1 = (int)((long long)nkb * (split + 1) / ksplit);
  const int nblk = kb1 - kb0;
  const size_t bh0 = (size_t)b * h + hg * R4_HPG;

  Frag<__bf16> fk[R4_HPG][4];
  {
    const int jrow = min(j0 + li, N - 1);
#pragma unroll
    for (int hh = 0; hh < R4_HPG; ++hh)
#pragma unroll
      for (int ks = 0; ks < 4; ++ks) fk[hh][ks].load16B(k + ((bh0 + hh) * Npad + jrow) * HD + ks * 16 + half * 8);
  }
  const int ibw = min(wave, nib - 1);
  const unsigned smem_u = lds_addr(smem);
  const unsigned voff = lane * 16;
  const char* q_w = reinterpret_cast<const char*>(q) + ((bh0 + wave) * (size_t)(Npad >> 5)) * 4096;
  const char* r_w = reinterpret_cast<const char*>(rf_in) + rf_frag(b, nkb, 0, ibw, 0, 0) * sizeof(__bf16);
  const char* l_w = reinterpret_cast<const char*>(lse + (bh0 + wave) * N);
  auto stage = [&](int kb, int buf) {
    const unsigned base = smem_u + buf * R4_STAGE;
    const char* qs = q_w + (size_t)kb * 4096;
#pragma unroll
    for (int ks = 0; ks < 4; ++ks) lds_dma16(voff, qs + ks * 1024, base + (wave * 4 + ks) * 1024);
    if (NIB == 4 || wave == 0) {
      const char* rs = r_w + (size_t)kb * (4 * 2 * 1024);
#pragma unroll
      for (int s2 = 0; s2 < 2; ++s2) lds_dma16(voff, rs + s2 * 1024, base + R4_QBYTES + (wave * 2 + s2) * 1024);
    }
    lds_dma4((unsigned)min(kb * 32 + li, N - 1) * 4u, l_w, base + R4_LSE + wave * 256);
  };

  f32x16 acc[NIB];
#pragma unroll
  for (int ib = 0; ib < NIB; ++ib)
#pragma unroll
    for (int r = 0; r < 16; ++r) acc[ib][r] = 0.0f;
  const float inv_h = 1.0f / (float)h;
  const unsigned lbase = lds_addr(smem) + lane * 16;

  if (nblk > 0) stage(kb0, 0);
  if (R4_NSTAGE > 2 && nblk > 1) stage(kb0 + 1, 1);

  for (int it = 0; it < nblk; ++it) {
    const int kb = kb0 + it, buf = it % R4_NSTAGE;
    if (AS_ROLLOUT_ABLATE != 11) {
      if (R4_NSTAGE == 2 || it + 1 >= nblk) asm volatile("s_waitcnt vmcnt(0)" ::: "memory");
      else if (NIB == 4 || wave == 0) asm volatile("s_waitcnt vmcnt(7)" ::: "memory");
      else asm volatile("s_waitcnt vmcnt(5)" ::: "memory");
    }
    {
      float own;
      const unsigned a_own = lds_addr(smem) + buf * R4_STAGE + R4_LSE + wave * 256 + lane * 4;
      asm volatile("ds_read_b32 %0, %1\n\ts_waitcnt lgkmcnt(0)" : "=v"(own) : "v"(a_own) : "memory");
      own *= -LOG2E;
      asm volatile("ds_write_b32 %0, %1\n\ts_waitcnt lgkmcnt(0)" :: "v"(a_own), "v"(own) : "memory");
    }
    if (AS_ROLLOUT_ABLATE != 14) __builtin_amdgcn_s_barrier();
    if (AS_ROLLOUT_ABLATE != 11 && it + R4_NSTAGE - 1 < nblk) stage(kb + R4_NSTAGE - 1, (it + R4_NSTAGE - 1) % R4_NSTAGE);
    const unsigned sb = lbase + buf * R4_STAGE;
    const unsigned cb = lds_addr(smem) + buf * R4_STAGE + R4_LSE + half * 16;
    u32x4 fc[2][4];
    auto read_c = [&](int hh, u32x4 (&c)[4]) {
      const unsigned a = cb + hh * 256;
      lds_read128(c[0], a);
      lds_read128_i<32>(c[1], a);
      lds_read128_i<64>(c[2], a);
      lds_read128_i<96>(c[3], a);
    };
    f32x16 pbar;
#pragma unroll
    for (int r = 0; r < 16; ++r) pbar[r] = 0.0f;
    u32x4 fa[2][4];
    read_c(0, fc[0]);
    lds_read128(fa[0][0], sb);
    lds_read128_i<1024>(fa[0][1], sb);
    lds_read128_i<2048>(fa[0][2], sb);
    lds_read128_i<3072>(fa[0][3], sb);
    {
      const unsigned a1 = sb + 4096;
      read_c(1, fc[1]);
      lds_read128(fa[1][0], a1);
      lds_read128_i<1024>(fa[1][1], a1);
      lds_read128_i<2048>(fa[1][2], a1);
      lds_read128_i<3072>(fa[1][3], a1);
    }
    lds_wait<8>(fa[0][0], fa[0][1], fa[0][2], fa[0][3], fc[0][0], fc[0][1], fc[0][2], fc[0][3]);
    auto qk = [&](int hh, u32x4 (&f)[4], u32x4 (&c)[4]) {
      f32x16 sc;
#pragma unroll
      for (int r = 0; r < 16; ++r) sc[r] = __uint_as_float(c[r >> 2][r & 3]);
#pragma unroll
      for (int ks = 0; ks < 4; ++ks) {
        Frag<__bf16> fq;
        fq.v = *reinterpret_cast<bf16x8*>(&f[ks]);
        if (AS_ROLLOUT_ABLATE != 13) sc = mma32(fq, fk[hh][ks], sc);
        else sc[ks] += (float)fq.v[0];
      }
      return sc;
    };
    f32x16 sc_cur = qk(0, fa[0], fc[0]);
    u32x4 fr[NIB][2];
#pragma unroll
    for (int hh = 0; hh < R4_HPG; ++hh) {
      f32x16 sc_next;
      if (hh + 1 < R4_HPG) {
        const int nx = (hh + 1) & 1;
        lds_wait<0>(fa[nx][0], fa[nx][1], fa[nx][2], fa[nx][3], fc[nx][0], fc[nx][1], fc[nx][2], fc[nx][3]);
        sc_next = qk(hh + 1, fa[nx], fc[nx]);
        if (hh + 2 < R4_HPG) {
          const unsigned a2 = sb + (hh + 2) * 4096;
          read_c(hh + 2, fc[hh & 1]);
          lds_read128(fa[hh & 1][0], a2);
          lds_read128_i<1024>(fa[hh & 1][1], a2);
          lds_read128_i<2048>(fa[hh & 1][2], a2);
          lds_read128_i<3072>(fa[hh & 1][3], a2);
        }
      } else {
#pragma unroll
        for (int ib = 0; ib < NIB; ++ib) {
          const unsigned a = sb + R4_QBYTES + min(ib, nib - 1) * 2048;
          lds_read128(fr[ib][0], a);
          lds_read128_i<1024>(fr[ib][1], a);
        }
      }
#pragma unroll
      for (int r = 0; r < 16; ++r) pbar[r] += AS_ROLLOUT_ABLATE == 12 ? sc_cur[r] : __builtin_amdgcn_exp2f(sc_cur[r]);
      if (hh + 1 < R4_HPG) sc_cur = sc_next;
    }
    Frag<__bf16> fp[2];
    if (kb * 32 + 32 <= N) {
#pragma unroll
      for (int r = 0; r < 16; ++r) fp[r >> 3].set(r & 7, pbar[r]);
    } else {
#pragma unroll
      for (int r = 0; r < 16; ++r) fp[r >> 3].set(r & 7, kb * 32 + acc_row(r, half) < N ? pbar[r] : 0.0f);
    }
    if constexpr (NIB == 1) lds_wait<0>(fr[0][0], fr[0][1]);
    else lds_wait<0>(fr[0][0], fr[0][1], fr[1][0], fr[1][1], fr[2][0], fr[2][1], fr[3][0], fr[3][1]);
#pragma unroll
    for (int s2 = 0; s2 < 2; ++s2)
#pragma unroll
      for (int ib = 0; ib < NIB; ++ib)
        if (ib < nib) {
          Frag<__bf16> f;
          f.v = *reinterpret_cast<bf16x8*>(&fr[ib][s2]);
          if (AS_ROLLOUT_ABLATE != 15) acc[ib] = mma32(f, fp[s2], acc[ib]);
          else acc[ib][0] += (float)f.v[0] + (float)fp[s2].v[0];
        }
  }

  const int pidx = split * ngroups + hg;
  const int j = j0 + li;
  if (j < N) {
#pragma unroll
    for (int ib = 0; ib < NIB; ++ib)
#pragma unroll
      for (int r = 0; r < 16; ++r) {
        const int i = ib * 32 + acc_row(r, half);
        if (i < Trows) part[(((size_t)pidx * B + b) * Trows + i) * N + j] = acc[ib][r] * inv_h;
      }
  }
}

bool rollout_force_v3() {
  static const bool v = getenv("AS_ROLLOUT_V3") != nullptr;
  return v;
}

constexpr int R4_MAXPARTS = 16;
int rollout4_ksplit(int B, int N, int h, int slots) {
  static const int forced = [] { const char* e = getenv("AS_R4_KS"); return e ? atoi(e) : 0; }();
  if (forced > 0 && forced * (h / R4_HPG) <= 16) return forced;
  const int units = as_ceil_div(N, 128) * B * (h / R4_HPG);
  int best = 1;
  float best_eff = 0.0f;
  for (int ks = 1; ks * (h / R4_HPG) <= R4_MAXPARTS && ks <= 8; ++ks) {
    const int wgs = units * ks;
    const float eff = (float)wgs / (float)(as_ceil_div(wgs, slots) * slots);
    if (eff > best_eff + 0.02f) { best_eff = eff; best = ks; }
  }
  return best;
}

template <typename T>
__global__ __launch_bounds__(64) void rollout_finish_kernel(const float* __restrict__ part, const float* __restrict__ Rin,
                                                            float* __restrict__ Rout, T* __restrict__ rf_out, int B, int N,
                                                            int Trows, int nsplit) {
  const int nkb = (N + 31) / 32;
  const int j = blockIdx.x * 64 + threadIdx.x, i = blockIdx.y, b = blockIdx.z;
  if (j >= nkb * 32) return;
  float v = 0.0f;
  if (i < Trows && j < N) {
    const size_t idx = ((size_t)b * Trows + i) * N + j;
    float a = 0.0f;
    for (int sp = 0; sp < nsplit; ++sp) a += part[(size_t)sp * B * Trows * N + idx];
    v = 0.5f * (a + Rin[idx]);
    Rout[idx] = v;
  }
  if (rf_out != nullptr) rf_out[rf_slot(b, nkb, i, j)] = from_f32<T>(v);
}

template <typename T>
int launch_rollout_step2(const void* q, const void* k, const float* lse, const float* Rin, const void* rf_in, float* Rout,
                         void* rf_out, float* part, int nsplit, int B, int N, int h, int Trows, hipStream_t s) {
  const int Npad = as_round_up(N, 64);
  const int hpw = as_ceil_div(h, 4);
  dim3 grid(as_ceil_div(N, 32), B, nsplit);
  const size_t kbytes = (size_t)h * 32 * Kj2<T>::PITCH, slab = 4 * 4 * 64 * sizeof(float4);
  const int xbufs = kbytes + 2 * slab <= 160 * 1024 ? 2 : 1;
  const size_t lds = kbytes + xbufs * slab;
  AS_REQUIRE(lds <= 160 * 1024, AS_E_UNSUPPORTED, "rollout_step: LDS %zu B exceeds 160 KiB (h=%d)", lds, h);
#define AS_RO2(HPW)                                                                                            \
  do {                                                                                                         \
    (void)hipFuncSetAttribute((const void*)rollout_step2_kernel<T, HPW>, hipFuncAttributeMaxDynamicSharedMemorySize, \
                              (int)lds);                                                                       \
    hipLaunchKernelGGL((rollout_step2_kernel<T, HPW>), grid, dim3(RO_NT), lds, s, (const T*)q, (const T*)k, lse, Rin, \
                       (const T*)rf_in, Rout, (T*)rf_out, part, B, N, Npad, h, Trows, nsplit, xbufs);          \
  } while (0)
  if (sizeof(T) == 2 && h % R4_HPG == 0 && part != nullptr && nsplit == R4_MAXPARTS && !rollout_force_v3()) {
    const int ng = h / R4_HPG;
    const int ks = rollout4_ksplit(B, N, h, 512);
    const size_t lds4 = (size_t)(Trows <= 32 ? R4Cfg<1>::NSTAGE : R4Cfg<4>::NSTAGE) * R4_STAGE;
    if (Trows <= 32) {
      (void)hipFuncSetAttribute((const void*)rollout_step4_kernel<1>, hipFuncAttributeMaxDynamicSharedMemorySize, (int)lds4);
      hipLaunchKernelGGL(rollout_step4_kernel<1>, dim3(as_ceil_div(N, 128), B, ks * ng), dim3(RO_NT), lds4, s, (const __bf16*)q,
                         (const __bf16*)k, lse, (const __bf16*)rf_in, part, B, N, Npad, h, Trows, ks);
    } else {
      (void)hipFuncSetAttribute((const void*)rollout_step4_kernel<4>, hipFuncAttributeMaxDynamicSharedMemorySize, (int)lds4);
      hipLaunchKernelGGL(rollout_step4_kernel<4>, dim3(as_ceil_div(N, 128), B, ks * ng), dim3(RO_NT), lds4, s, (const __bf16*)q,
                         (const __bf16*)k, lse, (const __bf16*)rf_in, part, B, N, Npad, h, Trows, ks);
    }
    AS_CHECK_LAUNCH("rollout_step4");
    dim3 fg(as_ceil_div(as_ceil_div(N, 32) * 32, 64), as_round_up(Trows, 32), B);
    hipLaunchKernelGGL((rollout_finish_kernel<T>), fg, dim3(64), 0, s, (const float*)part, Rin, Rout, (T*)rf_out, B, N,
                       Trows, ks * ng);
    AS_CHECK_LAUNCH("rollout_finish");
    return AS_OK;
  }
  if (sizeof(T) == 2 && h >= 8 && (getenv("AS_ROLLOUT_V2") == nullptr)) {
    const size_t lds3 = (size_t)h * 32 * Kj2<T>::PITCH;
    (void)hipFuncSetAttribute((const void*)rollout_step3_kernel<T>, hipFuncAttributeMaxDynamicSharedMemorySize, (int)lds3);
    hipLaunchKernelGGL((rollout_step3_kernel<T>), grid, dim3(RO_NT), lds3, s, (const T*)q, (const T*)k, lse, Rin,
                       (const T*)rf_in, Rout, (T*)rf_out, part, B, N, Npad, h, Trows, nsplit);
  } else {
  switch (hpw) {
    case 1: AS_RO2(1); break;
    case 2: AS_RO2(2); break;
    case 3: AS_RO2(3); break;
    case 4: AS_RO2(4); break;
    default: AS_REQUIRE(false, AS_E_UNSUPPORTED, "rollout_step: h=%d heads (max 16)", h);
  }
  }
#undef AS_RO2
  AS_CHECK_LAUNCH("rollout_step2");
  if (nsplit > 1) {
    dim3 fg(as_ceil_div(as_ceil_div(N, 32) * 32, 64), as_round_up(Trows, 32), B);
    hipLaunchKernelGGL((rollout_finish_kernel<T>), fg, dim3(64), 0, s, (const float*)part, Rin, Rout, (T*)rf_out, B, N,
                       Trows, nsplit);
    AS_CHECK_LAUNCH("rollout_finish");
  }
  return AS_OK;
}

int rollout_nsplit(int B, int N) {
  const int wgs = as_ceil_div(N, 32) * B;
  int ns = 1;
  while (ns < 16 && wgs * ns < 2048) ns *= 2;
  return wgs >= 2048 ? 1 : ns;
}

template <typename T>
int launch_mean_rows(const void* q, const void* k, const float* lse, float* out, void* rf_out, int B, int N, int h,
                     int row0, int nrows, bool top, hipStream_t s) {
  const int Npad = as_round_up(N, 64);
  dim3 grid(as_ceil_div(as_ceil_div(N, 32), 4), as_ceil_div(nrows, 32), B);
  if (top)
    hipLaunchKernelGGL((attn_mean_rows_kernel<T, true>), grid, dim3(RO_NT), 0, s, (const T*)q, (const T*)k, lse,
                       out, (T*)rf_out, B, N, Npad, h, row0, nrows);
  else
    hipLaunchKernelGGL((attn_mean_rows_kernel<T, false>), grid, dim3(RO_NT), 0, s, (const T*)q, (const T*)k, lse,
                       out, (T*)rf_out, B, N, Npad, h, row0, nrows);
  AS_CHECK_LAUNCH("attn_mean_rows");
  return AS_OK;
}

}

extern "C" size_t as_rollout_rfrag_bytes(int B, int N, int dtype) {
  if (B <= 0 || N <= 0) return 0;
  return (size_t)B * as_ceil_div(N, 32) * 4 * 2 * 64 * 8 * (dtype == AS_BF16 ? 2 : 4);
}

extern "C" int as_attn_mean_rows(const void* q, const void* k, const float* lse, float* out, int B, int N, int h,
                                 int row0, int nrows, int dtype, as_stream_t stream) {
  AS_REQUIRE(q && k && lse && out, AS_E_BADARG, "as_attn_mean_rows: null pointer");
  AS_REQUIRE(B > 0 && N > 0 && h > 0 && row0 >= 0 && nrows > 0 && row0 + nrows <= N, AS_E_BADARG,
             "as_attn_mean_rows: bad row range %d+%d of %d", row0, nrows, N);
  hipStream_t s = (hipStream_t)stream;
  if (dtype == AS_BF16) return launch_mean_rows<__bf16>(q, k, lse, out, nullptr, B, N, h, row0, nrows, false, s);
  if (dtype == AS_F32) return launch_mean_rows<float>(q, k, lse, out, nullptr, B, N, h, row0, nrows, false, s);
  AS_REQUIRE(false, AS_E_UNSUPPORTED, "as_attn_mean_rows: dtype %d", dtype);
}

extern "C" int as_rollout_top(const void* q, const void* k, const float* lse, float* R_out, void* rf_out, int B, int N,
                              int h, int T, int dtype, as_stream_t stream) {
  AS_REQUIRE(q && k && lse && R_out, AS_E_BADARG, "as_rollout_top: null pointer");
  AS_REQUIRE(B > 0 && h > 0 && T > 0 && T <= N && T <= 128, AS_E_BADARG, "as_rollout_top: bad sizes N=%d T=%d", N, T);
  hipStream_t s = (hipStream_t)stream;
  if (dtype == AS_BF16) return launch_mean_rows<__bf16>(q, k, lse, R_out, rf_out, B, N, h, N - T, T, true, s);
  if (dtype == AS_F32) return launch_mean_rows<float>(q, k, lse, R_out, rf_out, B, N, h, N - T, T, true, s);
  AS_REQUIRE(false, AS_E_UNSUPPORTED, "as_rollout_top: dtype %d", dtype);
}

namespace {
template <typename T>
__global__ __launch_bounds__(64) void rollout_pack_kernel(const float* __restrict__ R, T* __restrict__ rf, int B, int N, int Trows) {
  const int nkb = (N + 31) / 32;
  const int j = blockIdx.x * 64 + threadIdx.x, i = blockIdx.y, b = blockIdx.z;
  if (j >= nkb * 32) return;
  const float v = (i < Trows && j < N) ? R[((size_t)b * Trows + i) * N + j] : 0.0f;
  rf[rf_slot(b, nkb, i, j)] = from_f32<T>(v);
}
}

extern "C" int as_rollout_pack(const float* R, void* rf, int B, int N, int T, int dtype, as_stream_t stream) {
  AS_REQUIRE(R && rf, AS_E_BADARG, "as_rollout_pack: null pointer");
  AS_REQUIRE(B > 0 && N > 0 && T > 0 && T <= 128, AS_E_BADARG, "as_rollout_pack: bad sizes N=%d T=%d", N, T);
  dim3 grid(as_ceil_div(as_ceil_div(N, 32) * 32, 64), as_round_up(T, 32), B);
  if (dtype == AS_BF16)
    hipLaunchKernelGGL(rollout_pack_kernel<__bf16>, grid, dim3(64), 0, (hipStream_t)stream, R, (__bf16*)rf, B, N, T);
  else if (dtype == AS_F32)
    hipLaunchKernelGGL(rollout_pack_kernel<float>, grid, dim3(64), 0, (hipStream_t)stream, R, (float*)rf, B, N, T);
  else
    AS_REQUIRE(false, AS_E_UNSUPPORTED, "as_rollout_pack: dtype %d", dtype);
  AS_CHECK_LAUNCH("rollout_pack");
  return AS_OK;
}

extern "C" size_t as_rollout_step_workspace_bytes(int B, int N, int T) {
  if (B <= 0 || N <= 0 || T <= 0) return 0;
  return (size_t)R4_MAXPARTS * B * T * N * sizeof(float);
}

extern "C" int as_rollout_step(const void* q, const void* k, const float* lse, const float* R_in, const void* rf_in,
                               float* R_out, void* rf_out, void* workspace, size_t workspace_bytes, int B, int N, int h,
                               int T, int dtype, as_stream_t stream) {
  AS_REQUIRE(q && k && lse && R_in && rf_in && R_out && R_in != R_out && rf_in != rf_out, AS_E_BADARG,
             "as_rollout_step: null/aliased pointer");
  AS_REQUIRE(B > 0 && h > 0 && h <= 16 && T > 0 && T <= N && T <= 128, AS_E_BADARG,
             "as_rollout_step: bad sizes N=%d T=%d h=%d", N, T, h);
  hipStream_t s = (hipStream_t)stream;
  const size_t need = as_rollout_step_workspace_bytes(B, N, T);
  const bool have_ws = workspace != nullptr && workspace_bytes >= need && need > 0;
  const bool stream4 = have_ws && dtype == AS_BF16 && h % R4_HPG == 0 && !rollout_force_v3();
  const int ns = stream4 ? R4_MAXPARTS : (have_ws ? rollout_nsplit(B, N) : 1);
  float* part = ns > 1 ? (float*)workspace : nullptr;
  if (dtype == AS_BF16)
    return launch_rollout_step2<__bf16>(q, k, lse, R_in, rf_in, R_out, rf_out, part, ns, B, N, h, T, s);
  if (dtype == AS_F32) return launch_rollout_step2<float>(q, k, lse, R_in, rf_in, R_out, rf_out, part, ns, B, N, h, T, s);
  AS_REQUIRE(false, AS_E_UNSUPPORTED, "as_rollout_step: dtype %d", dtype);
}
```

attentionshift_amd/ops.py:

```python
import ctypes
import os

import threading

import numpy as np
import torch

from . import _lib
from ._lib import AS_BF16, AS_F32, AttnShiftError

HEAD_DIM = 64


def _dt(t):
    if t.dtype == torch.float32:
        return AS_F32
    if t.dtype == torch.bfloat16:
        return AS_BF16
    raise AttnShiftError(f"unsupported dtype {t.dtype} (float32 or bfloat16)")


def _chk(*tensors, dtype=None):
    for t in tensors:
        if t is None:
            continue
        if not t.is_cuda:
            raise AttnShiftError("hot-path ops need device (HBM) tensors; there is no CPU fallback")
        if not t.is_contiguous():
            raise AttnShiftError("hot-path ops need contiguous row-major tensors")
        if dtype is not None and t.dtype != dtype:
            raise AttnShiftError(f"expected {dtype}, got {t.dtype}")


def _p(t):
    return 0 if t is None else t.data_ptr()


_RAW_STREAM = getattr(torch._C, "_cuda_getCurrentRawStream", None)
_DEV = [None]


def _stream():
    if _RAW_STREAM is None:
        return torch.cuda.current_stream().cuda_stream
    d = _DEV[0]
    if d is None:
        d = _DEV[0] = torch.cuda.current_device()
    return _RAW_STREAM(d)


_TIMED = None


def enable_timing(names):
    global _TIMED
    _TIMED = {n: [] for n in names}


def disable_timing():
    global _TIMED
    _TIMED = None


def collect_timing():
    out = {}
    for n, evs in (_TIMED or {}).items():
        if n.endswith(":bytes"):
            out[n] = (len(evs), float(sum(evs)) / max(len(evs), 1))
        elif evs:
            ms = [a.elapsed_time(b) for a, b in evs]
            out[n] = (len(ms), sum(ms) / len(ms))
    return out


class _timed:
    def __init__(self, name):
        self.on = _TIMED is not None and name in _TIMED
        self.name = name

    def __enter__(self):
        if self.on:
            self.a, self.b = torch.cuda.Event(enable_timing=True), torch.cuda.Event(enable_timing=True)
            self.a.record(torch.cuda.current_stream())

    def __exit__(self, *exc):
        if self.on:
            self.b.record(torch.cuda.current_stream())
            _TIMED[self.name].append((self.a, self.b))


def npad(n):
    return _lib.load().as_npad(int(n))


_SK_BYTES = {}
_SK_WS = {}


def _sk_bytes(lib, M, Nout, K):
    key = (M, Nout, K, os.environ.get("AS_GEMM_SK"))
    v = _SK_BYTES.get(key)
    if v is None:
        v = _SK_BYTES[key] = int(lib.as_linear_sk_workspace_bytes(M, Nout, K))
    return v


def _sk_workspace(device, nbytes):
    key = (device, torch.cuda.current_stream(device).cuda_stream)
    ws = _SK_WS.get(key)
    if ws is None or ws.numel() < nbytes:
        ws = _SK_WS[key] = torch.empty(nbytes, device=device, dtype=torch.uint8)
    return ws


def linear(x, weight, bias=None, act="none"):
    lib = _lib.load()
    K = x.shape[-1]
    x2 = x.reshape(-1, K)
    _chk(x2, weight)
    if bias is not None:
        _chk(bias, dtype=torch.float32)
    if weight.dtype != x.dtype or weight.shape[1] != K:
        raise AttnShiftError("linear: weight must be [Nout, K] in the dtype of x")
    out = torch.empty(x2.shape[0], weight.shape[0], device=x.device, dtype=x.dtype)
    code = {"none": 0, "gelu": 1, "relu": 4}[act]
    M, Nout = x2.shape[0], weight.shape[0]
    need = _sk_bytes(lib, M, Nout, K) if x.dtype == torch.bfloat16 else 0
    if need:
        ws = _sk_workspace(x.device, need)
        _lib.check(lib.as_linear_sk_fwd(_p(x2), _p(weight), _p(bias), _p(out), M, Nout, K, _dt(x), code, _p(ws), ws.numel(),
                                        _stream()), "as_linear_sk_fwd")
    else:
        _lib.check(lib.as_linear_fwd(_p(x2), _p(weight), _p(bias), _p(out), M, Nout, K, _dt(x), code, _stream()), "as_linear_fwd")
    return out.reshape(*x.shape[:-1], Nout)


def linear_small(x, weight, bias=None, act="none", out=None):
    lib = _lib.load()
    if x.dim() != 2 or x.dtype != torch.float32 or weight.dtype != torch.float32 or x.stride(1) != 1 or not weight.is_contiguous():
        raise AttnShiftError("linear_small: x [M, K] fp32 with unit column stride, weight [Nout, K] fp32 contiguous")
    M, K = x.shape
    Nout = weight.shape[0]
    if weight.shape[1] != K:
        raise AttnShiftError("linear_small: weight must be [Nout, K]")
    if bias is not None:
        _chk(bias, dtype=torch.float32)
    if out is None:
        out = torch.empty(M, Nout, device=x.device, dtype=torch.float32)
    elif out.shape != (M, Nout) or out.dtype != torch.float32 or out.stride(1) != 1:
        raise AttnShiftError("linear_small: out must be [M, Nout] fp32 with unit column stride")
    code = {"none": 0, "gelu": 1, "relu": 4, "sigmoid": 5}[act]
    _lib.check(lib.as_linear_small_fwd(_p(x), x.stride(0), _p(weight), _p(bias), _p(out), out.stride(0), M, Nout, K, code, _stream()),
               "as_linear_small_fwd")
    return out


def linear_small_applies(x, weight):
    return (x.is_cuda and x.dtype == torch.float32 and weight.dtype == torch.float32 and x.dim() == 2 and 0 < x.shape[0] <= 1024
            and x.shape[1] >= 64 and x.shape[1] % 16 == 0 and x.stride(1) == 1 and x.stride(0) % 4 == 0 and weight.is_contiguous()
            and x.data_ptr() % 16 == 0 and weight.data_ptr() % 16 == 0)


def linear_gelu(x, weight, bias=None):
    lib = _lib.load()
    _chk(x, weight, dtype=torch.bfloat16)
    if bias is not None:
        _chk(bias, dtype=torch.float32)
    M, K = x.shape
    Nout = weight.shape[0]
    if weight.shape[1] != K:
        raise AttnShiftError("linear_gelu: weight must be [Nout, K]")
    out = torch.empty(M, Nout, device=x.device, dtype=torch.bfloat16)
    pre = torch.empty_like(out)
    _lib.check(lib.as_linear_gelu_fwd(_p(x), _p(weight), _p(bias), _p(out), _p(pre), M, Nout, K, AS_BF16, _stream()),
               "as_linear_gelu_fwd")
    return out, pre


def linear_gelu_applies(x, weight):
    return x.is_cuda and x.numel() > 0 and weight.shape[0] % 32 == 0 and weight.shape[1] % 32 == 0


def linear_splitk(x, weight, out_dtype=None):
    lib = _lib.load()
    _chk(x, weight, dtype=torch.bfloat16)
    M, K = x.shape
    Nout = weight.shape[0]
    if weight.shape[1] != K:
        raise AttnShiftError("linear_splitk: weight must be [Nout, K]")
    out_dtype = out_dtype or torch.bfloat16
    out = torch.empty(M, Nout, device=x.device, dtype=out_dtype)
    nbytes = int(lib.as_linear_splitk_workspace_bytes(M, Nout, K))
    ws = torch.empty(max(nbytes, 4) // 4, device=x.device, dtype=torch.float32)
    _lib.check(lib.as_linear_splitk_fwd(_p(x), _p(weight), _p(out), M, Nout, K, AS_BF16, 1 if out_dtype == torch.float32 else 0,
                                        _p(ws), nbytes, _stream()), "as_linear_splitk_fwd")
    return out


_LINEAR_BWD_WS = {}


def linear_bwd(x, weight, dy, need_dx=True, need_dw=True, need_db=True, dw_dtype=None, gelu_pre=None):
    lib = _lib.load()
    _chk(x, weight, dy, dtype=torch.bfloat16)
    M, K = x.shape
    Nout = weight.shape[0]
    if weight.shape[1] != K or tuple(dy.shape) != (M, Nout):
        raise AttnShiftError("linear_bwd: shapes must be x [M,K], weight [Nout,K], dy [M,Nout]")
    dw_dtype = dw_dtype or torch.bfloat16
    dx = torch.empty(M, K, device=x.device, dtype=torch.bfloat16) if need_dx else None
    dW = torch.empty(Nout, K, device=x.device, dtype=dw_dtype) if need_dw else None
    db = torch.empty(Nout, device=x.device, dtype=torch.float32) if need_db else None
    nbytes = int(lib.as_linear_bwd_workspace_bytes(M, Nout, K))
    key = (x.device, torch.cuda.current_stream(x.device).cuda_stream)
    ws = _LINEAR_BWD_WS.get(key)
    if ws is None or ws.numel() * 4 < nbytes:
        ws = _LINEAR_BWD_WS[key] = torch.empty((nbytes + 3) // 4, device=x.device, dtype=torch.float32)
    if gelu_pre is not None:
        _chk(gelu_pre, dtype=torch.bfloat16)
        if tuple(gelu_pre.shape) != (M, K) or not need_dx:
            raise AttnShiftError("linear_bwd: gelu_pre must be [M,K] and needs dx")
        _lib.check(lib.as_linear_bwd_dgelu(_p(x), _p(weight), _p(dy), _p(gelu_pre), _p(dx), _p(dW), _p(db), M, Nout, K, AS_BF16,
                                           1 if dw_dtype == torch.float32 else 0, _p(ws), nbytes, _stream()), "as_linear_bwd_dgelu")
        return dx, dW, db
    _lib.check(lib.as_linear_bwd(_p(x), _p(weight), _p(dy), _p(dx), _p(dW), _p(db), M, Nout, K, AS_BF16,
                                 1 if dw_dtype == torch.float32 else 0, _p(ws), nbytes, _stream()), "as_linear_bwd")
    return dx, dW, db


def deconv2x2(x_nhwc, w4, bias4=None, act="none"):
    lib = _lib.load()
    B, h, w, cin = x_nhwc.shape
    cout = w4.shape[0] // 4
    _chk(x_nhwc, w4)
    if bias4 is not None:
        _chk(bias4, dtype=torch.float32)
    out = torch.empty(B, 2 * h, 2 * w, cout, device=x_nhwc.device, dtype=x_nhwc.dtype)
    _lib.check(lib.as_deconv2x2_fwd(_p(x_nhwc), _p(w4), _p(bias4), _p(out), B * h * w, w, cin, cout, _dt(x_nhwc),
                                    1 if act == "gelu" else 0, _stream()), "as_deconv2x2_fwd")
    return out


def _scale_arg(delta_scale, x, delta):
    if delta_scale is None:
        return None, 1
    if delta is None or x.dim() != 3 or delta_scale.numel() != x.shape[0]:
        raise AttnShiftError("add_layernorm: delta_scale needs delta and x [B, N, D] with one scale per image")
    _chk(delta_scale, dtype=torch.float32)
    return delta_scale, x.shape[1]


def add_layernorm(x, delta, gamma, beta, eps, out_dtype, want_x=True, want_y=True, delta_scale=None, x_out=None):
    lib = _lib.load()
    D = x.shape[-1]
    x2 = x.reshape(-1, D)
    _chk(x2, dtype=torch.float32)
    _chk(delta)
    _chk(gamma, beta, dtype=torch.float32)
    if delta is not None and delta.dtype != out_dtype:
        raise AttnShiftError("add_layernorm: delta must have the output dtype")
    if x_out is not None:
        if not (want_x and delta is not None) or x_out.shape != x.shape:
            raise AttnShiftError("add_layernorm: x_out needs want_x, a delta and x's shape")
        _chk(x_out, dtype=torch.float32)
        x_out = x_out.view(-1, D)
    else:
        x_out = torch.empty_like(x2) if (want_x and delta is not None) else None
    y = torch.empty(x2.shape, device=x.device, dtype=out_dtype) if want_y else None
    dt = AS_BF16 if out_dtype == torch.bfloat16 else AS_F32
    sc, rps = _scale_arg(delta_scale, x, delta)
    _lib.check(lib.as_add_layernorm_scaled(_p(x2), _p(delta), _p(gamma), _p(beta), float(eps), _p(x_out), _p(y), x2.shape[0], D,
                                           dt, _p(sc), rps, _stream()), "as_add_layernorm")
    xo = x if (delta is None or not want_x) else x_out.reshape(x.shape)
    return (xo if want_x else None), (None if y is None else y.reshape(x.shape))


def assemble_tokens(emb, table):
    lib = _lib.load()
    emb = emb.contiguous()
    _chk(emb)
    _chk(table, dtype=torch.float32)
    B, Np, D = emb.shape
    N = table.shape[0]
    x = torch.empty(B, N, D, device=emb.device, dtype=torch.float32)
    _lib.check(lib.as_assemble_tokens(_p(emb), _p(table), _p(x), B, Np, N, D, _dt(emb), _stream()), "as_assemble_tokens")
    return x


def maxpool_nhwc(x_nhwc, k):
    lib = _lib.load()
    B, H, W, C = x_nhwc.shape
    if not (x_nhwc.is_cuda and x_nhwc.dtype == torch.float32):
        raise AttnShiftError("maxpool_nhwc: fp32 device tensor expected")
    if x_nhwc.stride()[1:] != (W * C, C, 1) or (B > 1 and x_nhwc.stride(0) % 4):
        x_nhwc = x_nhwc.contiguous()
    bs = x_nhwc.stride(0) if B > 1 else H * W * C
    out = torch.empty(B, H // k, W // k, C, device=x_nhwc.device, dtype=torch.float32)
    _lib.check(lib.as_maxpool_nhwc(_p(x_nhwc), _p(out), B, H, W, C, int(k), int(bs), _stream()), "as_maxpool_nhwc")
    return out


def add_layernorm_bwd(x_out, dy, dx_res, gamma, eps, dtype, want_dx=True, want_ddelta=True, want_affine=True, delta_scale=None):
    lib = _lib.load()
    D = x_out.shape[-1]
    x2 = x_out.reshape(-1, D)
    _chk(x2, dx_res, gamma, dtype=torch.float32)
    _chk(dy, dtype=dtype)
    M = x2.shape[0]
    dev = x_out.device
    scratch = not want_dx and not want_ddelta
    dx = torch.empty_like(x2) if (want_dx or scratch) else None
    dd = torch.empty(x2.shape, device=dev, dtype=dtype) if want_ddelta else None
    affine = want_affine and dy is not None
    dg = torch.empty(D, device=dev, dtype=torch.float32) if affine else None
    db = torch.empty(D, device=dev, dtype=torch.float32) if affine else None
    nbytes = lib.as_add_layernorm_bwd_workspace_bytes(M, D)
    ws = torch.empty(nbytes, device=dev, dtype=torch.uint8)
    dt = AS_BF16 if dtype == torch.bfloat16 else AS_F32
    sc, rps = (None, 1) if delta_scale is None else (delta_scale, x_out.shape[1] if x_out.dim() == 3 else 1)
    if sc is not None and (x_out.dim() != 3 or sc.numel() != x_out.shape[0]):
        raise AttnShiftError("add_layernorm_bwd: delta_scale needs x_out [B, N, D] with one scale per image")
    _lib.check(lib.as_add_layernorm_bwd_scaled(_p(x2), _p(dy), _p(dx_res), _p(gamma), float(eps), _p(dx), _p(dd), _p(dg), _p(db),
                                               _p(ws), nbytes, M, D, dt, _p(sc), rps, _stream()), "as_add_layernorm_bwd")
    return (None if dx is None or scratch else dx.reshape(x_out.shape), None if dd is None else dd.reshape(x_out.shape), dg, db)


class AttnLayerState:

    __slots__ = ("q", "k", "vt", "lse", "B", "N", "h", "dtype", "o")

    def __init__(self, q, k, vt, lse, B, N, h, dtype, o=None):
        self.q, self.k, self.vt, self.lse, self.B, self.N, self.h, self.dtype = q, k, vt, lse, B, N, h, dtype
        self.o = o


def _sdpa_ws(lib, B, N, h, like):
    n = lib.as_sdpa_fwd_workspace_bytes(B, N, h, _dt(like))
    return (torch.empty(n, device=like.device, dtype=torch.uint8), n) if n else (None, 0)


def attention_fwd(x, w_qkv, b_qkv, w_proj, b_proj, num_heads, keep_state=True, keep_o=False):
    lib = _lib.load()
    B, N, D = x.shape
    _chk(x, w_qkv, w_proj)
    if D != num_heads * HEAD_DIM:
        raise AttnShiftError(f"head dim must be {HEAD_DIM} (D={D}, heads={num_heads})")
    Np_ = npad(N)
    dev, dt = x.device, x.dtype
    q = torch.empty(B, num_heads, Np_, HEAD_DIM, device=dev, dtype=dt)
    k = torch.empty_like(q)
    vt = torch.empty(B, num_heads, HEAD_DIM, Np_, device=dev, dtype=dt)
    o = torch.empty(B, N, D, device=dev, dtype=dt)
    out = torch.empty(B, N, D, device=dev, dtype=dt)
    lse = torch.empty(B, num_heads, N, device=dev, dtype=torch.float32)
    ws, wbytes = _sdpa_ws(lib, B, N, num_heads, x)
    if _TIMED is None:
        _lib.check(lib.as_attn_fwd(_p(x), _p(w_qkv), _p(b_qkv), _p(w_proj), _p(b_proj), _p(out), _p(lse), _p(q), _p(k),
                                   _p(vt), _p(o), _p(ws), wbytes, B, N, D, num_heads, _dt(x), _stream()), "as_attn_fwd")
    else:
        with _timed("qkv_gemm"):
            _lib.check(lib.as_qkv_fwd(_p(x), _p(w_qkv), _p(b_qkv), _p(q), _p(k), _p(vt), B, N, D, num_heads, _dt(x),
                                      _stream()), "as_qkv_fwd")
        with _timed("sdpa_fwd"):
            _lib.check(lib.as_sdpa_fwd(_p(q), _p(k), _p(vt), _p(o), _p(lse), _p(ws), wbytes, B, N, num_heads, _dt(x),
                                       _stream()), "as_sdpa_fwd")
        with _timed("proj_gemm"):
            _lib.check(lib.as_linear_fwd(_p(o), _p(w_proj), _p(b_proj), _p(out), B * N, D, D, _dt(x), 0, _stream()),
                       "as_linear_fwd")
    return out, (AttnLayerState(q, k, vt, lse, B, N, num_heads, dt, o if keep_o else None) if keep_state else None)


def attention_bwd(x, w_qkv, w_proj, dout, state, want_bias=(True, True)):
    lib = _lib.load()
    B, N, D = x.shape
    if state.o is None:
        raise AttnShiftError("attention_bwd needs the forward's pre-projection output: call attention_fwd(keep_o=True)")
    _chk(x, w_qkv, w_proj, dout, state.q, state.k, state.vt, state.o, state.lse)
    dev, dt = x.device, x.dtype
    dx = torch.empty_like(x)
    dwqkv = torch.empty_like(w_qkv)
    dwproj = torch.empty_like(w_proj)
    dbqkv = torch.empty(3 * D, device=dev, dtype=torch.float32) if want_bias[0] else None
    dbproj = torch.empty(D, device=dev, dtype=torch.float32) if want_bias[1] else None
    nbytes = lib.as_attn_bwd_workspace_bytes(B, N, D, state.h, _dt(x))
    ws = torch.empty(nbytes, device=dev, dtype=torch.uint8)
    with _timed("attn_bwd"):
        _lib.check(lib.as_attn_bwd(_p(x), _p(w_qkv), _p(w_proj), _p(dout), _p(state.q), _p(state.k), _p(state.vt),
                                   _p(state.o), _p(state.lse), _p(dx), _p(dwqkv), _p(dbqkv), _p(dwproj), _p(dbproj),
                                   _p(ws), nbytes, B, N, D, state.h, _dt(x), _stream()), "as_attn_bwd")
    return dx, dwqkv, dbqkv, dwproj, dbproj


QSCALE = 0.125 * 1.4426950408889634
LN2 = 0.6931471805599453


def q_to_fragment_major(q_rows):
    B, h, Np_, d = q_rows.shape
    t = q_rows.reshape(B, h, Np_ // 32, 32, 4, 2, 8)
    return t.permute(0, 1, 2, 4, 5, 3, 6).contiguous().reshape(B, h, Np_, d)


def q_from_fragment_major(q_frag):
    B, h, Np_, d = q_frag.shape
    t = q_frag.reshape(B, h, Np_ // 32, 4, 2, 32, 8)
    return t.permute(0, 1, 2, 5, 3, 4, 6).contiguous().reshape(B, h, Np_, d)


def qkv_fwd(x, w_qkv, b_qkv, num_heads):
    lib = _lib.load()
    B, N, D = x.shape
    _chk(x, w_qkv)
    Np_ = npad(N)
    q = torch.empty(B, num_heads, Np_, HEAD_DIM, device=x.device, dtype=x.dtype)
    k = torch.empty_like(q)
    vt = torch.empty(B, num_heads, HEAD_DIM, Np_, device=x.device, dtype=x.dtype)
    _lib.check(lib.as_qkv_fwd(_p(x), _p(w_qkv), _p(b_qkv), _p(q), _p(k), _p(vt), B, N, D, num_heads, _dt(x), _stream()),
               "as_qkv_fwd")
    return q, k, vt


def sdpa_fwd(q, k, vt, N):
    lib = _lib.load()
    B, h = q.shape[0], q.shape[1]
    _chk(q, k, vt)
    o = torch.empty(B, N, h * HEAD_DIM, device=q.device, dtype=q.dtype)
    lse = torch.empty(B, h, N, device=q.device, dtype=torch.float32)
    ws, wbytes = _sdpa_ws(lib, B, N, h, q)
    _lib.check(lib.as_sdpa_fwd(_p(q), _p(k), _p(vt), _p(o), _p(lse), _p(ws), wbytes, B, N, h, _dt(q), _stream()),
               "as_sdpa_fwd")
    return o, lse


def sdpa_bwd(q, k, vt, o, d_o, lse, N):
    lib = _lib.load()
    B, h = q.shape[0], q.shape[1]
    _chk(q, k, vt, o, d_o, lse)
    dqkv = torch.empty(B, N, 3 * h * HEAD_DIM, device=q.device, dtype=q.dtype)
    nbytes = lib.as_sdpa_bwd_workspace_bytes(B, N, h, _dt(q))
    ws = torch.empty(nbytes, device=q.device, dtype=torch.uint8)
    _lib.check(lib.as_sdpa_bwd(_p(q), _p(k), _p(vt), _p(o), _p(d_o), _p(lse), _p(dqkv), _p(ws), nbytes, B, N, h,
                               _dt(q), _stream()), "as_sdpa_bwd")
    return dqkv


def window_attention_fwd(qkv, b_qkv, table, num_heads, ws, shift, return_attn=False):
    lib = _lib.load()
    B, H, W, C3 = qkv.shape
    C = C3 // 3
    _chk(qkv)
    _chk(b_qkv, table, dtype=torch.float32)
    out = torch.empty(B, H, W, C, device=qkv.device, dtype=qkv.dtype)
    nW = -(-H // ws) * -(-W // ws)
    attn = torch.empty(B * nW, num_heads, ws * ws, ws * ws, device=qkv.device, dtype=torch.float32) if return_attn else None
    with _timed("window_attn_fwd"):
        _lib.check(lib.as_window_attn_fwd(_p(qkv), _p(b_qkv), _p(table), _p(out), _p(attn), B, H, W, C, num_heads, int(ws),
                                          int(shift), _dt(qkv), _stream()), "as_window_attn_fwd")
    if _TIMED is not None and "window_attn_fwd" in _TIMED:
        _TIMED.setdefault("window_attn_fwd:bytes", []).append(qkv.numel() * qkv.element_size() + out.numel() * out.element_size())
    return out, attn


def window_attention_bwd(qkv, b_qkv, table, d_out, num_heads, ws, shift):
    lib = _lib.load()
    B, H, W, C3 = qkv.shape
    C = C3 // 3
    _chk(qkv, d_out)
    _chk(b_qkv, table, dtype=torch.float32)
    dqkv = torch.zeros_like(qkv)
    dtable = torch.empty_like(table)
    dpad = torch.empty(C3, device=qkv.device, dtype=torch.float32)
    nbytes = lib.as_window_attn_bwd_workspace_bytes(B, H, W, num_heads, int(ws))
    wsbuf = torch.empty(nbytes, device=qkv.device, dtype=torch.uint8)
    _lib.check(lib.as_window_attn_bwd(_p(qkv), _p(b_qkv), _p(table), _p(d_out), _p(dqkv), _p(dtable), _p(dpad), _p(wsbuf),
                                      nbytes, B, H, W, C, num_heads, int(ws), int(shift), _dt(qkv), _stream()),
               "as_window_attn_bwd")
    return dqkv, dtable, dpad


def attn_mean_rows(state, row0, nrows):
    lib = _lib.load()
    out = torch.empty(state.B, nrows, state.N, device=state.q.device, dtype=torch.float32)
    _lib.check(lib.as_attn_mean_rows(_p(state.q), _p(state.k), _p(state.lse), _p(out), state.B, state.N, state.h,
                                     int(row0), int(nrows), _dt(state.q), _stream()), "as_attn_mean_rows")
    return out


def rollout_rows(states, num_point_tokens, rows=None, use_workspace=True):
    lib = _lib.load()
    top = states[-1]
    T = int(num_point_tokens)
    dev, dt = top.q.device, _dt(top.q)
    nbytes = lib.as_rollout_rfrag_bytes(top.B, top.N, dt)
    outs = []
    R = torch.empty(top.B, T, top.N, device=dev, dtype=torch.float32)
    lower = list(reversed(states[:-1]))
    subset = rows is not None and len(lower) > 0
    rf = torch.empty(nbytes, device=dev, dtype=torch.uint8) if not subset else None
    _lib.check(lib.as_rollout_top(_p(top.q), _p(top.k), _p(top.lse), _p(R), _p(rf), top.B, top.N, top.h, T, dt, _stream()),
               "as_rollout_top")
    if rows is not None:
        R = torch.gather(R, 1, rows[:, :, None].expand(-1, -1, top.N)).contiguous()
        T = R.shape[1]
        if subset:
            rf = torch.empty(nbytes, device=dev, dtype=torch.uint8)
            _lib.check(lib.as_rollout_pack(_p(R), _p(rf), top.B, top.N, T, dt, _stream()), "as_rollout_pack")
    outs.append(R)
    wbytes = lib.as_rollout_step_workspace_bytes(top.B, top.N, T) if (lower and use_workspace) else 0
    ws = torch.empty(wbytes, device=dev, dtype=torch.uint8) if wbytes else None
    for n, st in enumerate(lower):
        Rn = torch.empty_like(R)
        rfn = torch.empty_like(rf) if n + 1 < len(lower) else None
        _lib.check(lib.as_rollout_step(_p(st.q), _p(st.k), _p(st.lse), _p(R), _p(rf), _p(Rn), _p(rfn), _p(ws), wbytes,
                                       st.B, st.N, st.h, T, dt, _stream()), "as_rollout_step")
        outs.append(Rn)
        R, rf = Rn, rfn
    return torch.stack(outs, dim=1)


def rollout_rows_dense(states, num_point_tokens, rows=None):
    T = int(num_point_tokens)
    run, outs = None, []
    for st in reversed(states):
        a = attn_mean_rows(st, 0, st.N)
        a.diagonal(dim1=1, dim2=2).add_(1.0)
        a /= a.sum(-1, keepdim=True)
        if run is None:
            run = a[:, st.N - T:, :]
            if rows is not None:
                run = torch.gather(run, 1, rows[:, :, None].expand(-1, -1, st.N))
        else:
            run = torch.bmm(run, a)
        outs.append(run.contiguous())
        del a
    return torch.stack(outs, dim=1)


def ccl_2d(binary):
    lib = _lib.load()
    squeeze = binary.dim() == 2
    img = binary[None] if squeeze else binary
    _chk(img, dtype=torch.uint8)
    M, H, W = img.shape
    labels = torch.empty(M, H, W, device=img.device, dtype=torch.int32)
    _lib.check(lib.as_ccl_2d(_p(img), _p(labels), M, H, W, _stream()), "as_ccl_2d")
    return labels[0] if squeeze else labels


def cam_boxes(cams, points, cam_thr, area_ratio, up=16, return_upsampled=False, return_minmax=False):
    lib = _lib.load()
    _chk(cams, points, dtype=torch.float32)
    M, Hp, Wp = cams.shape
    boxes = torch.empty(M, 4, device=cams.device, dtype=torch.float32)
    status = torch.empty(M, device=cams.device, dtype=torch.int32)
    cams_up = torch.empty(M, Hp * up, Wp * up, device=cams.device, dtype=torch.float32) if return_upsampled else None
    minmax = torch.empty(M, 2, device=cams.device, dtype=torch.float32) if (return_upsampled or return_minmax) else None
    nbytes = lib.as_cam_boxes_workspace_bytes(M, Hp, Wp, up)
    ws = torch.empty(nbytes, device=cams.device, dtype=torch.uint8)
    _lib.check(lib.as_cam_boxes(_p(cams), _p(points), float(cam_thr), float(area_ratio), M, Hp, Wp, up, _p(boxes),
                                _p(status), _p(cams_up), _p(minmax), _p(ws), nbytes, _stream()), "as_cam_boxes")
    if return_upsampled:
        return boxes, status, cams_up, minmax
    return (boxes, status, minmax) if return_minmax else (boxes, status)


def cam_sample_masks(cams, map_idx, minmax, thr_bg, thr_fg, up=16, want_counts=True):
    lib = _lib.load()
    _chk(cams, minmax, dtype=torch.float32)
    _chk(map_idx, dtype=torch.int32)
    M, Hp, Wp = cams.shape
    G = map_idx.shape[0]
    masks = torch.empty(2 * G + 1, Hp * up, Wp * up, device=cams.device, dtype=torch.uint8)
    counts = torch.empty(2 * G + 1, device=cams.device, dtype=torch.int32) if want_counts else None
    nbytes = lib.as_cam_sample_masks_workspace_bytes(G, Hp, Wp, up)
    ws = torch.empty(nbytes, device=cams.device, dtype=torch.uint8) if nbytes else None
    _lib.check(lib.as_cam_sample_masks(_p(cams), _p(map_idx), _p(minmax), G, Hp, Wp, up, float(thr_bg), float(thr_fg),
                                       _p(masks), _p(counts), _p(ws), nbytes, _stream()), "as_cam_sample_masks")
    return masks, counts


def semantic_prestage(map_fg, thr, k=11, up=16, want_counts=True):
    lib = _lib.load()
    _chk(map_fg, dtype=torch.float32)
    G, H, W = map_fg.shape
    hp, wp = H // up, W // up
    fg_inter = torch.empty(G, hp, wp, device=map_fg.device, dtype=torch.float32)
    mask = torch.empty(G, hp, wp, device=map_fg.device, dtype=torch.uint8)
    counts = torch.empty(G, device=map_fg.device, dtype=torch.int32) if want_counts else None
    _lib.check(lib.as_semantic_prestage(_p(map_fg), float(thr), int(k), G, hp, wp, up, _p(fg_inter), _p(mask), _p(counts),
                                        _stream()), "as_semantic_prestage")
    return fg_inter, mask, counts


_shift_ws = {}
_shift_ws_lock = threading.Lock()
_SHIFT_WS_MAX_BYTES = 256 << 20


def cosine_shift(feat, box_patch, obj_img, prot, n_shift, hp, wp, tau0=0.1, temp=0.1, return_trace=False):
    lib = _lib.load()
    _chk(prot, dtype=torch.float32)
    _chk(box_patch, obj_img, dtype=torch.int32)
    B, Np_, C = feat.shape
    G, P, _ = prot.shape
    if Np_ != hp * wp:
        raise AttnShiftError("cosine_shift: Np != hp*wp")
    if not (feat.is_cuda and feat.dtype == torch.float32 and feat.stride(2) == 1 and feat.stride(1) == C
            and (B == 1 or (feat.stride(0) >= Np_ * C and feat.stride(0) % 4 == 0)) and feat.data_ptr() % 16 == 0):
        raise AttnShiftError("cosine_shift: feat must be fp32 [B,Np,C] on the device with contiguous, 16-byte aligned image blocks")
    fbs = feat.stride(0) if B > 1 else Np_ * C
    prot_out = torch.empty_like(prot)
    sim = torch.empty(G, P, Np_, device=feat.device, dtype=torch.float32)
    assign = torch.empty(max(n_shift, 1), G, Np_, device=feat.device, dtype=torch.int32) if return_trace else None
    tau = torch.empty(max(n_shift, 1), G, P, device=feat.device, dtype=torch.float32) if return_trace else None
    key = (feat.device, torch.cuda.current_stream(feat.device).cuda_stream, B, C, hp, wp, G, P)
    with _shift_ws_lock:
        ws = _shift_ws.get(key)
        if ws is None:
            nbytes = lib.as_cosine_shift_workspace_bytes(B, C, hp, wp, G, P)
            if sum(t.numel() for t in _shift_ws.values()) + nbytes > _SHIFT_WS_MAX_BYTES:
                _shift_ws.clear()
            ws = torch.empty(nbytes, device=feat.device, dtype=torch.uint8)
            _shift_ws[key] = ws
    with _timed("cosine_shift"):
        _lib.check(lib.as_cosine_shift_strided(_p(feat), int(fbs), _p(box_patch), _p(obj_img), _p(prot), _p(prot_out), float(tau0),
                                               float(temp), int(n_shift), _p(sim), _p(assign), _p(tau), _p(ws), ws.numel(), B, C,
                                               hp, wp, G, P, _stream()), "as_cosine_shift")
    if return_trace:
        return prot_out, sim, assign[:n_shift], tau[:n_shift]
    return prot_out, sim


def refine_similarity(feat, seeds, boxes_patch, num_obj, refine_times, tau, is_select, hp, wp):
    lib = _lib.load()
    _chk(feat, seeds, dtype=torch.float32)
    if boxes_patch is not None:
        _chk(boxes_patch, dtype=torch.int32)
    Np_, C = feat.shape
    Gp = seeds.shape[0]
    maps = torch.empty(refine_times + 1, Gp, Np_, device=feat.device, dtype=torch.float32)
    seeds_out = seeds if refine_times == 0 else torch.empty(Gp, C, device=feat.device, dtype=torch.float32)
    nbytes = lib.as_refine_similarity_workspace_bytes(C, Np_, Gp)
    ws = torch.empty(nbytes, device=feat.device, dtype=torch.uint8)
    n_select = (Gp if is_select else 0) if isinstance(is_select, bool) else int(is_select)
    _lib.check(lib.as_refine_similarity(_p(feat), _p(seeds), _p(boxes_patch), int(num_obj), Gp, int(refine_times),
                                        float(tau), n_select, _p(maps), _p(seeds_out), _p(ws), nbytes, C,
                                        hp, wp, _stream()), "as_refine_similarity")
    return maps, seeds_out


def instance_maps(sim_fg, sim_bg, num_obj, hp, wp, up=16):
    lib = _lib.load()
    _chk(sim_fg, sim_bg, dtype=torch.float32)
    L, Gp, _ = sim_fg.shape
    G = int(num_obj)
    H, W = hp * up, wp * up
    map_fg = torch.empty(L, G, H, W, device=sim_fg.device, dtype=torch.float32)
    map_bg = torch.empty(L, G, H, W, device=sim_fg.device, dtype=torch.float32)
    nbytes = lib.as_instance_maps_workspace_bytes(L, G)
    ws = torch.empty(nbytes, device=sim_fg.device, dtype=torch.uint8)
    _lib.check(lib.as_instance_maps(_p(sim_fg), _p(sim_bg), L, G, Gp, hp, wp, up, _p(map_fg), _p(map_bg), _p(ws), nbytes,
                                    _stream()), "as_instance_maps")
    return map_fg, map_bg


def crop_threshold_erode(maps, crops, thr, relative, k):
    lib = _lib.load()
    _chk(maps, dtype=torch.float32)
    if crops is not None:
        _chk(crops, dtype=torch.int32)
    M, H, W = maps.shape
    mask = torch.empty(M, H, W, device=maps.device, dtype=torch.uint8)
    counts = torch.empty(M, device=maps.device, dtype=torch.int32)
    nbytes = lib.as_crop_threshold_erode_workspace_bytes(M, H, W)
    ws = torch.empty(nbytes, device=maps.device, dtype=torch.uint8)
    _lib.check(lib.as_crop_threshold_erode(_p(maps), _p(crops), float(thr), 1 if relative else 0, int(k), _p(mask),
                                           _p(counts), _p(ws), nbytes, M, H, W, _stream()), "as_crop_threshold_erode")
    return mask, counts


def mask_candidates(map_fg, map_bg, crops, pos_thr, neg_thr, mask_thr, k):
    lib = _lib.load()
    _chk(map_fg, map_bg, dtype=torch.float32)
    _chk(crops, dtype=torch.int32)
    G, H, W = map_fg.shape
    pos, neg, pseudo = (torch.empty(G, H, W, device=map_fg.device, dtype=torch.uint8) for _ in range(3))
    counts = torch.empty(3, G, device=map_fg.device, dtype=torch.int32)
    nbytes = lib.as_mask_candidates_workspace_bytes(G, H, W)
    ws = torch.empty(nbytes, device=map_fg.device, dtype=torch.uint8)
    _lib.check(lib.as_mask_candidates(_p(map_fg), _p(map_bg), _p(crops), float(pos_thr), float(neg_thr), float(mask_thr),
                                      int(k), _p(pos), _p(neg), _p(pseudo), _p(counts), _p(ws), nbytes, G, H, W,
                                      _stream()), "as_mask_candidates")
    return pos, neg, pseudo, counts


def part_stats_raw(maps, rois, owner, stride=16):
    lib = _lib.load()
    maps = maps.contiguous()
    rois = rois.contiguous().float()
    own = owner.to(torch.int32).contiguous()
    _chk(maps, rois, dtype=torch.float32)
    M, hp, wp = maps.shape
    c = torch.empty(M, 2, device=maps.device, dtype=torch.float32)
    yx = torch.empty(M, 2, device=maps.device, dtype=torch.int32)
    area = torch.empty(M, device=maps.device, dtype=torch.int32)
    inside = torch.empty(M, device=maps.device, dtype=torch.uint8)
    _lib.check(lib.as_part_stats(_p(maps), _p(rois), _p(own), float(stride), _p(c), _p(yx), _p(area), _p(inside), M, hp, wp,
                                 _stream()), "as_part_stats")
    return c, yx, area, inside


def part_stats(maps, rois, owner, stride=16):
    c, yx, area, inside = part_stats_raw(maps, rois, owner, stride)
    return c, yx.long(), area.long(), inside.bool()


def part_select(area, inside, ngroups, c, yx, labels, feat_tok, G, P, wp, num_points):
    lib = _lib.load()
    _chk(c, feat_tok, dtype=torch.float32)
    _chk(area, yx, ngroups, dtype=torch.int32)
    _chk(inside, dtype=torch.uint8)
    _chk(labels, dtype=torch.int64)
    dev, M, C = c.device, G * P, feat_tok.shape[-1]
    coords = torch.empty(2, M, 2, device=dev, dtype=torch.float32)
    lab = torch.empty(3, M, device=dev, dtype=torch.int64)
    feats = torch.empty(M, C, device=dev, dtype=torch.float32)
    ints = torch.empty(M + G + 1, device=dev, dtype=torch.int32)
    _lib.check(lib.as_part_select(_p(area), _p(inside), _p(ngroups), _p(c), _p(yx), _p(labels), _p(feat_tok), G, P, C, int(wp),
                                  int(num_points), _p(coords[0]), _p(coords[1]), _p(lab[0]), _p(lab[1]), _p(lab[2]), _p(feats),
                                  _p(ints[:M]), _p(ints[M:]), _stream()), "as_part_select")
    return coords[0], coords[1], lab[0], lab[1], lab[2], feats, ints[M:]


def filter_parts(sim, fg_inter, sim_thr=0.8, pos_thr=0.85):
    lib = _lib.load()
    sim = sim.contiguous()
    fg = fg_inter.contiguous()
    _chk(sim, fg, dtype=torch.float32)
    G, P = sim.shape[:2]
    keep = torch.empty(G, P, device=sim.device, dtype=torch.uint8)
    _lib.check(lib.as_filter_parts(_p(sim), _p(fg), float(sim_thr), float(pos_thr), _p(keep), G, P, sim[0, 0].numel(),
                                   _stream()), "as_filter_parts")
    return keep.view(torch.bool)


def draw_distinct(counts, u, k, flag=None):
    lib = _lib.load()
    if counts.dtype != torch.int32:
        counts = counts.to(torch.int32)
    if tuple(counts.shape) != (u.shape[0], 2):
        raise AttnShiftError(f"draw_distinct: counts {tuple(counts.shape)} for {u.shape[0]} objects")
    sg, sk = counts.stride()
    if sg <= 0 or sk <= 0:
        counts = counts.contiguous()
        sg, sk = 2, 1
    if not counts.is_cuda:
        raise AttnShiftError("hot-path ops need device (HBM) tensors; there is no CPU fallback")
    u = u.contiguous()
    _chk(u, dtype=torch.float32)
    G, M = u.shape
    rp = torch.empty(G, k, device=u.device, dtype=torch.int32)
    rn = torch.empty(G, k, device=u.device, dtype=torch.int32)
    ip = torch.empty(G, k, device=u.device, dtype=torch.uint8)
    if flag is None:
        flag = torch.zeros(1, device=u.device, dtype=torch.int32)
    _lib.check(lib.as_draw_distinct(_p(counts), sg, sk, _p(u), _p(rp), _p(rn), _p(ip), _p(flag), G, M, int(k), _stream()),
               "as_draw_distinct")
    return rp, rn, ip.view(torch.bool), flag


def small_attention_fwd(qkv):
    lib = _lib.load()
    qkv = qkv.contiguous()
    _chk(qkv)
    Bp, N, _, h, d = qkv.shape
    out = torch.empty(Bp, N, h * d, device=qkv.device, dtype=qkv.dtype)
    lse = torch.empty(Bp, h, N, device=qkv.device, dtype=torch.float32)
    _lib.check(lib.as_small_attn_fwd(_p(qkv), _p(out), _p(lse), Bp, N, h, d, _dt(qkv), _stream()), "as_small_attn_fwd")
    return out, lse


def small_attention_bwd(qkv, out, d_out, lse):
    lib = _lib.load()
    qkv, out, d_out = qkv.contiguous(), out.contiguous(), d_out.contiguous().to(qkv.dtype)
    _chk(qkv, out, d_out)
    Bp, N, _, h, d = qkv.shape
    dqkv = torch.empty_like(qkv)
    nbytes = lib.as_small_attn_bwd_workspace_bytes(Bp, N, h)
    ws = torch.empty(nbytes, device=qkv.device, dtype=torch.uint8)
    _lib.check(lib.as_small_attn_bwd(_p(qkv), _p(out), _p(d_out), _p(lse), _p(dqkv), _p(ws), nbytes, Bp, N, h, d, _dt(qkv),
                                     _stream()), "as_small_attn_bwd")
    return dqkv


def chamfer_2d_fwd(xyz1, xyz2):
    lib = _lib.load()
    xyz1, xyz2 = xyz1.contiguous(), xyz2.contiguous()
    _chk(xyz1, xyz2, dtype=torch.float32)
    B, n, _ = xyz1.shape
    m = xyz2.shape[1]
    d1 = torch.empty(B, n, device=xyz1.device, dtype=torch.float32)
    d2 = torch.empty(B, m, device=xyz1.device, dtype=torch.float32)
    i1 = torch.empty(B, n, device=xyz1.device, dtype=torch.int32)
    i2 = torch.empty(B, m, device=xyz1.device, dtype=torch.int32)
    _lib.check(lib.as_chamfer_2d_fwd(_p(xyz1), _p(xyz2), _p(d1), _p(d2), _p(i1), _p(i2), B, n, m, _stream()), "as_chamfer_2d_fwd")
    return d1, d2, i1, i2


def chamfer_2d_bwd(xyz1, xyz2, g1, g2, idx1, idx2):
    lib = _lib.load()
    xyz1, xyz2, g1, g2 = xyz1.contiguous(), xyz2.contiguous(), g1.contiguous().float(), g2.contiguous().float()
    _chk(xyz1, xyz2, g1, g2, dtype=torch.float32)
    _chk(idx1, idx2, dtype=torch.int32)
    B, n, _ = xyz1.shape
    m = xyz2.shape[1]
    gx1, gx2 = torch.empty_like(xyz1), torch.empty_like(xyz2)
    _lib.check(lib.as_chamfer_2d_bwd(_p(xyz1), _p(xyz2), _p(g1), _p(g2), _p(idx1), _p(idx2), _p(gx1), _p(gx2), B, n, m,
                                     _stream()), "as_chamfer_2d_bwd")
    return gx1, gx2


def merge_plan(keep, link):
    lib = _lib.load()
    k8 = keep.to(torch.uint8).contiguous()
    l8 = link.to(torch.uint8).contiguous()
    _chk(k8, l8)
    G, P = k8.shape
    groups = torch.empty(G, P, device=k8.device, dtype=torch.int32)
    ngroups = torch.empty(G, device=k8.device, dtype=torch.int32)
    _lib.check(lib.as_merge_plan(_p(k8), _p(l8), _p(groups), _p(ngroups), G, P, _stream()), "as_merge_plan")
    return groups, ngroups


def merge_parts(prot, keep, thr, slots, flag=None):
    lib = _lib.load()
    prot = prot.contiguous()
    _chk(prot, dtype=torch.float32)
    k8 = keep.view(torch.uint8) if keep.dtype == torch.bool else keep
    k8 = k8.contiguous()
    _chk(k8, dtype=torch.uint8)
    G, P, C = prot.shape
    merged = torch.empty(G, slots, C, device=prot.device, dtype=torch.float32)
    ngroups = torch.empty(G, device=prot.device, dtype=torch.int32)
    _lib.check(lib.as_merge_parts(_p(prot), _p(k8), float(thr), _p(merged), _p(ngroups), _p(flag), G, P, C, int(slots),
                                  _stream()), "as_merge_parts")
    return merged, ngroups


def select_median_boxes(boxes, meta, Lc, stride, status=None, bad=None, pick_in=None):
    lib = _lib.load()
    _chk(boxes, dtype=torch.float32)
    _chk(meta, status, bad, dtype=torch.int32)
    _chk(pick_in, dtype=torch.int64)
    n = meta.shape[0]
    pick = torch.empty(n, device=boxes.device, dtype=torch.int64)
    chosen = torch.empty(n, 4, device=boxes.device, dtype=torch.float32)
    map_idx = torch.empty(n, device=boxes.device, dtype=torch.int32)
    ints = torch.empty(2, n, 4, device=boxes.device, dtype=torch.int32)
    if pick_in is not None and pick_in.numel() != n:
        raise AttnShiftError(f"select_median_boxes: {pick_in.numel()} choices for {n} objects")
    _lib.check(lib.as_select_median_boxes(_p(boxes), _p(meta), int(Lc), int(stride), _p(pick_in), _p(pick), _p(chosen), _p(map_idx),
                                          _p(ints[0]), _p(ints[1]), _p(status), _p(bad), n, _stream()),
               "as_select_median_boxes")
    return pick, chosen, map_idx, ints[0], ints[1]


def mask_count(mask):
    lib = _lib.load()
    m = mask.view(torch.uint8) if mask.dtype == torch.bool else mask
    _chk(m, dtype=torch.uint8)
    M, HW = m.shape
    out = torch.empty(M, device=m.device, dtype=torch.int32)
    _lib.check(lib.as_mask_count(_p(m), _p(out), M, HW, _stream()), "as_mask_count")
    return out


def mt_sample_ranks(state, counts, k):
    lib = _lib.load()
    _chk(state, counts, dtype=torch.int32)
    S = counts.numel()
    ranks = torch.zeros(S, k, device=counts.device, dtype=torch.int32)
    flag = torch.empty(1, device=counts.device, dtype=torch.int32)
    _lib.check(lib.as_mt_sample_ranks(_p(state), _p(counts), _p(ranks), _p(flag), S, int(k), _stream()), "as_mt_sample_ranks")
    return ranks, flag


def mt_perm_ranks(state, counts2, k):
    lib = _lib.load()
    _chk(state, counts2, dtype=torch.int32)
    G = counts2.shape[0]
    ranks = torch.zeros(G, k, device=counts2.device, dtype=torch.int32)
    flag = torch.empty(1, device=counts2.device, dtype=torch.int32)
    _lib.check(lib.as_mt_perm_ranks(_p(state), _p(counts2), _p(ranks), _p(flag), G, int(k), _stream()), "as_mt_perm_ranks")
    return ranks, flag


def rank_select(mask, ranks):
    lib = _lib.load()
    _chk(mask, dtype=torch.uint8)
    r32 = ranks.to(torch.int32).contiguous()
    _chk(r32)
    M, HW = mask.shape
    K = r32.shape[1]
    out = torch.empty(M, K, device=mask.device, dtype=torch.int32)
    nbytes = lib.as_rank_select_workspace_bytes(M, HW)
    ws = torch.empty(nbytes, device=mask.device, dtype=torch.uint8)
    _lib.check(lib.as_rank_select(_p(mask), _p(r32), _p(out), _p(ws), nbytes, M, HW, K, _stream()), "as_rank_select")
    return out.long()


def rank_select_xy(mask, ranks, W, yx=False):
    lib = _lib.load()
    _chk(mask, dtype=torch.uint8)
    r32 = ranks if ranks.dtype == torch.int32 and ranks.is_contiguous() else ranks.to(torch.int32).contiguous()
    _chk(r32)
    M, HW = mask.shape
    K = r32.shape[1]
    out = torch.empty(M, K, 2, device=mask.device, dtype=torch.int64)
    nbytes = lib.as_rank_select_workspace_bytes(M, HW)
    ws = torch.empty(nbytes, device=mask.device, dtype=torch.uint8)
    _lib.check(lib.as_rank_select_xy(_p(mask), _p(r32), _p(out), _p(ws), nbytes, M, HW, K, int(W), 1 if yx else 0, _stream()),
               "as_rank_select_xy")
    return out


def rank_draw_xy(mask, K, W, u=None, flag=None, yx=False, patch=None, want_xy=True):
    lib = _lib.load()
    _chk(mask, dtype=torch.uint8)
    M, HW = mask.shape
    if u is not None:
        _chk(u, dtype=torch.float32)
        if tuple(u.shape) != (M, K):
            raise AttnShiftError("rank_draw_xy: u must be [M, K]")
    if flag is not None and (flag.dtype != torch.int32 or flag.numel() != 1 or not flag.is_cuda):
        raise AttnShiftError("rank_draw_xy: flag must be one int32 on the device")
    out = torch.empty(M, K, 2, device=mask.device, dtype=torch.int64) if want_xy or patch is None else None
    pout, pdiv, pw, pbase, prot = None, 1, 1, 0, 0
    if patch is not None:
        pout, pdiv, pw, pbase, prot = patch
        if pout is None:
            pout = torch.empty(M, K, device=mask.device, dtype=torch.int64)
        if pout.dtype != torch.int64 or pout.numel() != M * K or not pout.is_contiguous():
            raise AttnShiftError("rank_draw_xy: patch output must be a contiguous int64 [M, K]")
    nbytes = lib.as_rank_select_workspace_bytes(M, HW)
    ws = torch.empty(nbytes, device=mask.device, dtype=torch.uint8)
    _lib.check(lib.as_rank_draw_xy(_p(mask), 1 if u is not None else 2, _p(u), _p(flag), _p(out), _p(pout), int(pdiv), int(pw),
                                   int(pbase), int(prot), _p(ws), nbytes, M, HW, int(K), int(W), 1 if yx else 0, _stream()),
               "as_rank_draw_xy")
    return out if patch is None else (out, pout)


def roi_align_fwd(feat_nhwc, rois, out_size, spatial_scale, sampling_ratio=0, aligned=True):
    lib = _lib.load()
    _chk(feat_nhwc, rois, dtype=torch.float32)
    B, H, W, C = feat_nhwc.shape
    R = rois.shape[0]
    out = torch.empty(R, out_size * out_size, C, device=feat_nhwc.device, dtype=torch.float32)
    _lib.check(lib.as_roi_align_fwd(_p(feat_nhwc), _p(rois), _p(out), B, H, W, C, R, int(out_size), float(spatial_scale),
                                    int(sampling_ratio), int(bool(aligned)), _stream()), "as_roi_align_fwd")
    return out


def roi_align_bwd(dout, rois, shape, out_size, spatial_scale, sampling_ratio=0, aligned=True):
    lib = _lib.load()
    _chk(dout, rois, dtype=torch.float32)
    B, H, W, C = shape
    dfeat = torch.empty(B, H, W, C, device=dout.device, dtype=torch.float32)
    _lib.check(lib.as_roi_align_bwd(_p(dout), _p(rois), _p(dfeat), B, H, W, C, rois.shape[0], int(out_size),
                                    float(spatial_scale), int(sampling_ratio), int(bool(aligned)), _stream()), "as_roi_align_bwd")
    return dfeat


def nms(boxes_sorted, iou_threshold, max_keep=-1):
    lib = _lib.load()
    _chk(boxes_sorted, dtype=torch.float32)
    if boxes_sorted.dim() != 2 or boxes_sorted.shape[1] != 4:
        raise AttnShiftError(f"nms: boxes must be [n, 4], got {tuple(boxes_sorted.shape)}")
    n = boxes_sorted.shape[0]
    keep = torch.empty(n, device=boxes_sorted.device, dtype=torch.int64)
    if n == 0:
        return keep
    count = torch.empty(1, device=boxes_sorted.device, dtype=torch.int32)
    nbytes = lib.as_nms_workspace_bytes(n)
    ws = torch.empty(nbytes, device=boxes_sorted.device, dtype=torch.uint8)
    _lib.check(lib.as_nms(_p(boxes_sorted), n, float(iou_threshold), int(max_keep), _p(keep), _p(count), _p(ws), nbytes,
                          _stream()), "as_nms")
    return keep[:int(count.item())]


def paste_masks(src, labels, boxes, H, W, apply_sigmoid, out_mode, thr=0.5):
    lib = _lib.load()
    _chk(src, boxes, dtype=torch.float32)
    _chk(labels, dtype=torch.int64)
    if src.dim() != 4 or tuple(boxes.shape) != (src.shape[0], 4) or (labels is not None and labels.numel() != src.shape[0]):
        raise AttnShiftError("paste_masks: src [n,K,h,w], boxes [n,4], labels [n]")
    if out_mode not in (0, 1, 2):
        raise AttnShiftError(f"paste_masks: out_mode {out_mode}")
    n, K, h, w = src.shape
    out = torch.empty(n, int(H), int(W), device=src.device, dtype=(torch.float32, torch.bool, torch.uint8)[out_mode])
    if out.numel():
        _lib.check(lib.as_paste_masks(_p(src), _p(labels), _p(boxes), _p(out), n, K, h, w, int(H), int(W),
                                      int(bool(apply_sigmoid)), int(out_mode), float(thr), _stream()), "as_paste_masks")
    return out


def rle_tile():
    rows, cols = ctypes.c_int(0), ctypes.c_int(0)
    _lib.check(_lib.load().as_rle_tile(ctypes.addressof(rows), ctypes.addressof(cols)), "as_rle_tile")
    return rows.value, cols.value


def rle_encode(masks):
    lib = _lib.load()
    _chk(masks)
    if masks.dtype not in (torch.bool, torch.uint8):
        raise AttnShiftError(f"rle_encode: masks must be bool or uint8, got {masks.dtype}")
    if masks.dim() != 3:
        raise AttnShiftError(f"rle_encode: masks must be [n, H, W], got {tuple(masks.shape)}")
    n, H, W = masks.shape
    if n == 0:
        return []
    if H * W == 0:
        return [b"0"] * n
    dev = masks.device
    nbytes = lib.as_rle_workspace_bytes(n, H, W)
    ws = torch.empty(nbytes, device=dev, dtype=torch.uint8)
    totals = torch.empty(n, device=dev, dtype=torch.int32)
    _lib.check(lib.as_rle_count(_p(masks), n, H, W, _p(totals), _p(ws), nbytes, _stream()), "as_rle_count")
    tot = totals.cpu().numpy().astype(np.int64)
    runs = int(tot.sum())
    pos = torch.empty(runs, device=dev, dtype=torch.int32)
    cap = 7 * (runs + n)
    out = torch.empty(8 * n + cap, device=dev, dtype=torch.uint8)
    _lib.check(lib.as_rle_encode(_p(masks), n, H, W, _p(totals), _p(ws), nbytes, _p(pos) if runs else 0, runs,
                                 out.data_ptr() + 8 * n, cap, _p(out), _stream()), "as_rle_encode")
    host = out.cpu().numpy()
    lens = host[:8 * n].view(np.uint64).astype(np.int64)
    starts = 8 * n + 7 * (np.cumsum(tot) - tot + np.arange(n))
    return [host[a:a + l].tobytes() for a, l in zip(starts.tolist(), lens.tolist())]


_IMG_SHAPES = {}


def _img_shapes(img_shapes, device):
    key = (tuple((float(s[0]), float(s[1])) for s in img_shapes), device)
    t = _IMG_SHAPES.get(key)
    if t is None:
        if len(_IMG_SHAPES) > 256:
            _IMG_SHAPES.clear()
        t = _IMG_SHAPES[key] = torch.tensor(key[0], dtype=torch.float32).reshape(-1, 2).to(device)
    return t


def rpn_candidate_count(cls_scores, nms_pre):
    ns = [int(c.shape[1] * c.shape[2] * c.shape[3]) for c in cls_scores]
    return sum(n if nms_pre <= 0 else min(int(nms_pre), n) for n in ns)


def rpn_candidates(cls_scores, bbox_preds, base_anchors, strides, img_shapes, nms_pre, min_bbox_size=0, means=(0., 0., 0., 0.),
                   stds=(1., 1., 1., 1.), wh_ratio_clip=16 / 1000):
    lib = _lib.load()
    L = len(cls_scores)
    if L == 0 or len(bbox_preds) != L or len(strides) != L:
        raise AttnShiftError("rpn_candidates: cls_scores, bbox_preds and strides need one entry per level (at least one)")
    _chk(*cls_scores, *bbox_preds, dtype=torch.float32)
    B, A = int(cls_scores[0].shape[0]), int(cls_scores[0].shape[1])
    for c, r in zip(cls_scores, bbox_preds):
        if c.dim() != 4 or r.dim() != 4 or c.shape[0] != B or c.shape[1] != A or tuple(r.shape) != (B, 4 * A, c.shape[2], c.shape[3]):
            raise AttnShiftError("rpn_candidates: cls_scores[l] [B,A,H,W] and bbox_preds[l] [B,4A,H,W] with one B and A")
    if len(img_shapes) != B:
        raise AttnShiftError(f"rpn_candidates: {len(img_shapes)} image shapes for {B} images")
    dev = cls_scores[0].device
    base = base_anchors.to(device=dev, dtype=torch.float32).contiguous()
    if tuple(base.shape) != (L, A, 4):
        raise AttnShiftError(f"rpn_candidates: base_anchors must be [{L}, {A}, 4], got {tuple(base.shape)}")
    levels = (_lib.RpnLevel * L)()
    for l, (c, r, s) in enumerate(zip(cls_scores, bbox_preds, strides)):
        sx, sy = (s, s) if isinstance(s, int) else (s[0], s[1])
        levels[l] = _lib.RpnLevel(_p(c), _p(r), int(c.shape[2]), int(c.shape[3]), int(sx), int(sy))
    C = rpn_candidate_count(cls_scores, nms_pre)
    shapes = _img_shapes(img_shapes, dev)
    ms = (ctypes.c_float * 8)(*[float(v) for v in means], *[float(v) for v in stds])
    cand_box = torch.empty(B, C, 4, device=dev, dtype=torch.float32)
    cand_nms_box = torch.empty(B, C, 4, device=dev, dtype=torch.float32)
    cand_score = torch.empty(B, C, device=dev, dtype=torch.float32)
    cand_level = torch.empty(B, C, device=dev, dtype=torch.int32)
    cand_index = torch.empty(B, C, device=dev, dtype=torch.int32)
    cand_count = torch.empty(B, device=dev, dtype=torch.int32)
    if B == 0:
        return cand_box, cand_nms_box, cand_score, cand_level, cand_index, cand_count
    nbytes = lib.as_rpn_candidates_workspace_bytes(B, C)
    ws = torch.empty(max(nbytes, 16), device=dev, dtype=torch.uint8)
    _lib.check(lib.as_rpn_candidates(ctypes.addressof(levels), L, B, A, _p(base), _p(shapes), int(nms_pre), float(min_bbox_size),
                                     ctypes.addressof(ms), abs(float(np.log(wh_ratio_clip))), C, _p(cand_box), _p(cand_nms_box),
                                     _p(cand_score), _p(cand_level), _p(cand_index), _p(cand_count), _p(ws), nbytes, _stream()),
               "as_rpn_candidates")
    return cand_box, cand_nms_box, cand_score, cand_level, cand_index, cand_count


def _rpn_grid_levels(featmap_sizes, strides):
    L = len(featmap_sizes)
    if L == 0 or len(strides) != L:
        raise AttnShiftError("rpn targets: featmap_sizes and strides need one entry per level (at least one)")
    levels = (_lib.RpnLevel * L)()
    for l, (fs, s) in enumerate(zip(featmap_sizes, strides)):
        sx, sy = (s, s) if isinstance(s, int) else (s[0], s[1])
        levels[l] = _lib.RpnLevel(None, None, int(fs[0]), int(fs[1]), int(sx), int(sy))
    return levels


def rpn_assign(base_anchors, featmap_sizes, strides, gt_boxes, gt_offsets, sum_g, max_g, shapes, pos_iou_thr, neg_iou_thr,
               min_pos_iou, match_low_quality, allowed_border, workspace=None):
    lib = _lib.load()
    _chk(base_anchors, gt_boxes, dtype=torch.float32)
    _chk(gt_offsets, shapes, dtype=torch.int32)
    L, A = int(base_anchors.shape[0]), int(base_anchors.shape[1])
    B = int(shapes.shape[0])
    if len(featmap_sizes) != L or tuple(base_anchors.shape) != (L, A, 4):
        raise AttnShiftError(f"rpn_assign: base_anchors {tuple(base_anchors.shape)} for {len(featmap_sizes)} levels")
    if gt_offsets.numel() != B + 1 or tuple(shapes.shape) != (B, 4) or tuple(gt_boxes.shape) != (int(sum_g), 4):
        raise AttnShiftError("rpn_assign: gt_boxes [sum_g,4], gt_offsets [B+1], shapes [B,4]")
    levels = _rpn_grid_levels(featmap_sizes, strides)
    T = sum(A * int(fs[0]) * int(fs[1]) for fs in featmap_sizes)
    dev = base_anchors.device
    assigned = torch.empty(B, T, device=dev, dtype=torch.int32)
    max_iou = torch.empty(B, T, device=dev, dtype=torch.float32)
    counts = torch.empty(B, 2, device=dev, dtype=torch.int32)
    nbytes = lib.as_rpn_assign_workspace_bytes(B, T, int(sum_g))
    ws = torch.empty(max(nbytes, 16), device=dev, dtype=torch.uint8) if workspace is None else workspace
    _chk(ws, dtype=torch.uint8)
    if ws.numel() < nbytes:
        raise AttnShiftError(f"rpn_assign: workspace of {ws.numel()} bytes, {nbytes} needed")
    _lib.check(lib.as_rpn_assign(ctypes.addressof(levels), L, B, A, _p(base_anchors), _p(gt_boxes) if sum_g else 0, _p(gt_offsets),
                                 int(sum_g), int(max_g), _p(shapes), float(pos_iou_thr), float(neg_iou_thr), float(min_pos_iou),
                                 int(bool(match_low_quality)), int(allowed_border), _p(assigned), _p(max_iou), _p(counts), _p(ws),
                                 nbytes, _stream()), "as_rpn_assign")
    return assigned, max_iou, counts, ws


def rpn_sample(assigned, plan, ranks, workspace, sum_g):
    lib = _lib.load()
    _chk(assigned, plan, ranks, dtype=torch.int32)
    _chk(workspace, dtype=torch.uint8)
    B, T = assigned.shape
    num = int(ranks.shape[2])
    if tuple(plan.shape) != (B, 4) or tuple(ranks.shape) != (B, 2, num):
        raise AttnShiftError("rpn_sample: plan [B,4], ranks [B,2,num]")
    inds = torch.empty(B, 2, num, device=assigned.device, dtype=torch.int32)
    _lib.check(lib.as_rpn_sample(B, T, int(sum_g), num, _p(assigned), _p(plan), _p(ranks), _p(workspace), workspace.numel(), _p(inds),
                                 _stream()), "as_rpn_sample")
    return inds


def rpn_targets(base_anchors, featmap_sizes, strides, gt_boxes, gt_offsets, sum_g, assigned, inds, means=(0., 0., 0., 0.),
                stds=(1., 1., 1., 1.)):
    lib = _lib.load()
    _chk(base_anchors, gt_boxes, dtype=torch.float32)
    _chk(gt_offsets, assigned, inds, dtype=torch.int32)
    L, A = int(base_anchors.shape[0]), int(base_anchors.shape[1])
    B, T = assigned.shape
    num = int(inds.shape[2])
    if tuple(inds.shape) != (B, 2, num) or gt_offsets.numel() != B + 1 or len(featmap_sizes) != L:
        raise AttnShiftError("rpn_targets: inds [B,2,num], gt_offsets [B+1], one feature map size per level")
    if T != sum(A * int(fs[0]) * int(fs[1]) for fs in featmap_sizes):
        raise AttnShiftError("rpn_targets: assigned does not have the geometry's number of anchors")
    levels = _rpn_grid_levels(featmap_sizes, strides)
    ms = (ctypes.c_float * 8)(*[float(v) for v in means], *[float(v) for v in stds])
    pos_gt = torch.empty(B, num, device=assigned.device, dtype=torch.int32)
    pos_delta = torch.empty(B, num, 4, device=assigned.device, dtype=torch.float32)
    _lib.check(lib.as_rpn_targets(ctypes.addressof(levels), L, B, A, _p(base_anchors), _p(gt_boxes) if sum_g else 0, _p(gt_offsets),
                                  int(sum_g), _p(assigned), _p(inds), 2 * num, num, ctypes.addressof(ms), _p(pos_gt), _p(pos_delta),
                                  _stream()), "as_rpn_targets")
    return pos_gt, pos_delta
```

include/attnshift.h:

```cpp
#ifndef ATTNSHIFT_H
#define ATTNSHIFT_H

#include <stddef.h>
#include <stdint.h>

#ifdef __cplusplus
extern "C" {
#endif

#define AS_VERSION 100
#define AS_OK 0
#define AS_E_BADARG (-1)
#define AS_E_UNSUPPORTED (-2)
#define AS_E_LAUNCH (-3)
#define AS_E_WORKSPACE (-4)

#define AS_F32 0
#define AS_BF16 1

#define AS_HEAD_DIM 64

typedef void* as_stream_t;

int as_version(void);
const char* as_last_error(void);


int as_npad(int N);

int as_linear_fwd(const void* x, const void* W, const float* bias, void* out, int M, int Nout, int K,
                  int dtype, int act, as_stream_t stream);

int as_linear_small_fwd(const float* x, int ldx, const float* W, const float* bias, float* out, int ldo, int M, int Nout, int K,
                        int act, as_stream_t stream);

size_t as_linear_sk_workspace_bytes(int M, int Nout, int K);
int as_linear_sk_fwd(const void* x, const void* W, const float* bias, void* out, int M, int Nout, int K, int dtype, int act,
                     void* ws, size_t ws_bytes, as_stream_t stream);

int as_deconv2x2_fwd(const void* x, const void* W4, const float* bias4, void* out, int M, int w, int cin, int cout,
                     int dtype, int act, as_stream_t stream);

int as_qkv_fwd(const void* x , const void* Wqkv , const float* bqkv ,
               void* q, void* k, void* vt, int B, int N, int D, int h, int dtype, as_stream_t stream);

size_t as_sdpa_fwd_workspace_bytes(int B, int N, int h, int dtype);
int as_sdpa_fwd(const void* q, const void* k, const void* vt, void* o, float* lse, void* workspace,
                size_t workspace_bytes, int B, int N, int h, int dtype, as_stream_t stream);

size_t as_sdpa_bwd_workspace_bytes(int B, int N, int h, int dtype);
int as_sdpa_bwd(const void* q, const void* k, const void* vt, const void* o, const void* d_o, const float* lse,
                void* dqkv, void* workspace, size_t workspace_bytes, int B, int N, int h, int dtype,
                as_stream_t stream);

int as_attn_fwd(const void* x, const void* Wqkv, const float* bqkv, const void* Wproj, const float* bproj,
                void* out , float* lse, void* q, void* k, void* vt, void* o, void* workspace,
                size_t workspace_bytes , int B, int N, int D, int h,
                int dtype, as_stream_t stream);

size_t as_attn_bwd_workspace_bytes(int B, int N, int D, int h, int dtype);
int as_attn_bwd(const void* x, const void* Wqkv, const void* Wproj, const void* dout, const void* q, const void* k,
                const void* vt, const void* o, const float* lse, void* dx, void* dWqkv, float* dbqkv, void* dWproj,
                float* dbproj, void* workspace, size_t workspace_bytes, int B, int N, int D, int h, int dtype,
                as_stream_t stream);

int as_window_attn_fwd(const void* qkv, const float* bqkv, const float* table, void* out, float* attn_out, int B, int H,
                       int W, int C, int h, int ws, int shift, int dtype, as_stream_t stream);

int as_add_layernorm(const float* x_in, const void* delta, const float* gamma, const float* beta, float eps,
                     float* x_out, void* y_out, int M, int D, int dtype, as_stream_t stream);
int as_add_layernorm_scaled(const float* x_in, const void* delta, const float* gamma, const float* beta, float eps,
                            float* x_out, void* y_out, int M, int D, int dtype, const float* delta_scale,
                            int rows_per_scale, as_stream_t stream);

int as_linear_gelu_fwd(const void* x, const void* W, const float* bias, void* out, void* pre, int M, int Nout, int K,
                       int dtype, as_stream_t stream);
int as_linear_dgelu_fwd(const void* x, const void* W, const void* pre, void* out, int M, int Nout, int K, int dtype,
                        as_stream_t stream);

size_t as_linear_splitk_workspace_bytes(int M, int Nout, int K);
int as_linear_splitk_fwd(const void* x, const void* W, void* out, int M, int Nout, int K, int dtype, int out_f32,
                         void* workspace, size_t workspace_bytes, as_stream_t stream);

size_t as_linear_bwd_workspace_bytes(int M, int Nout, int K);
int as_linear_bwd(const void* x, const void* W, const void* dy, void* dx, void* dW, float* db, int M, int Nout, int K,
                  int dtype, int dw_f32, void* workspace, size_t workspace_bytes, as_stream_t stream);
int as_linear_bwd_dgelu(const void* x, const void* W, const void* dy, const void* pre, void* dx, void* dW, float* db, int M,
                        int Nout, int K, int dtype, int dw_f32, void* workspace, size_t workspace_bytes, as_stream_t stream);

int as_maxpool_nhwc(const float* x, float* out, int B, int H, int W, int C, int k, long long x_batch_stride,
                    as_stream_t stream);

int as_assemble_tokens(const void* emb, const float* table, float* out, int B, int Np, int N, int D, int dtype,
                       as_stream_t stream);

size_t as_add_layernorm_bwd_workspace_bytes(int M, int D);
int as_add_layernorm_bwd(const float* x, const void* dy, const float* dx_res, const float* gamma, float eps, float* dx_out,
                         void* ddelta_out, float* dgamma, float* dbeta, void* workspace, size_t workspace_bytes, int M, int D,
                         int dtype, as_stream_t stream);
int as_add_layernorm_bwd_scaled(const float* x, const void* dy, const float* dx_res, const float* gamma, float eps,
                                float* dx_out, void* ddelta_out, float* dgamma, float* dbeta, void* workspace,
                                size_t workspace_bytes, int M, int D, int dtype, const float* delta_scale,
                                int rows_per_scale, as_stream_t stream);

size_t as_window_attn_bwd_workspace_bytes(int B, int H, int W, int h, int ws);
int as_window_attn_bwd(const void* qkv, const float* bqkv, const float* table, const void* d_out, void* dqkv,
                       float* dtable, float* dbqkv_pad, void* workspace, size_t workspace_bytes, int B, int H, int W,
                       int C, int h, int ws, int shift, int dtype, as_stream_t stream);

int as_attn_mean_rows(const void* q, const void* k, const float* lse, float* out, int B, int N, int h,
                      int row0, int nrows, int dtype, as_stream_t stream);

size_t as_rollout_rfrag_bytes(int B, int N, int dtype);
int as_rollout_pack(const float* R, void* rf, int B, int N, int T, int dtype, as_stream_t stream);
size_t as_rollout_step_workspace_bytes(int B, int N, int T);
int as_rollout_top(const void* q, const void* k, const float* lse, float* R_out, void* rf_out, int B, int N, int h,
                   int T, int dtype, as_stream_t stream);
int as_rollout_step(const void* q, const void* k, const float* lse, const float* R_in, const void* rf_in,
                    float* R_out, void* rf_out, void* workspace, size_t workspace_bytes, int B, int N, int h, int T,
                    int dtype, as_stream_t stream);


int as_ccl_2d(const uint8_t* img , int32_t* labels , int M, int H, int W,
              as_stream_t stream);

size_t as_cam_boxes_workspace_bytes(int M, int Hp, int Wp, int up);
int as_cam_boxes(const float* cams , const float* points , float cam_thr,
                 float area_ratio, int M, int Hp, int Wp, int up, float* boxes, int32_t* status,
                 float* cams_up, float* minmax, void* ws, size_t ws_bytes, as_stream_t stream);

size_t as_cam_sample_masks_workspace_bytes(int G, int Hp, int Wp, int up);
int as_cam_sample_masks(const float* cams , const int32_t* map_idx ,
                        const float* minmax , int G, int Hp, int Wp, int up, float thr_bg, float thr_fg,
                        uint8_t* masks, int32_t* counts, void* ws, size_t ws_bytes, as_stream_t stream);

size_t as_mask_candidates_workspace_bytes(int G, int H, int W);
int as_mask_candidates(const float* map_fg, const float* map_bg, const int32_t* crops, float pos_thr, float neg_thr,
                       float mask_thr, int k, uint8_t* pos, uint8_t* neg, uint8_t* pseudo, int32_t* counts, void* ws,
                       size_t ws_bytes, int G, int H, int W, as_stream_t stream);

int as_part_stats(const float* maps, const float* rois, const int32_t* owner, float stride, float* out_c,
                  int32_t* out_yx, int32_t* out_area, uint8_t* out_inside, int M, int Hp, int Wp, as_stream_t stream);

int as_part_select(const int32_t* area, const uint8_t* inside, const int32_t* ngroups, const float* c, const int32_t* yx,
                   const int64_t* labels, const float* feat_tok, int G, int P, int C, int Wp, int num_points, float* coords,
                   float* coords_org, int64_t* out_labels, int64_t* labels_org, int64_t* corres, float* feats,
                   int32_t* sel_slot, int32_t* split, as_stream_t stream);

int as_filter_parts(const float* sim , const float* fg_inter , float sim_thr, float pos_thr,
                    uint8_t* keep , int G, int P, int Np, as_stream_t stream);

int as_draw_distinct(const int32_t* counts, int count_stride_g, int count_stride_k, const float* u ,
                     int32_t* rank_pos , int32_t* rank_neg, uint8_t* is_pos, int32_t* flag, int G, int M, int K,
                     as_stream_t stream);

int as_mt_sample_ranks(int32_t* state , const int32_t* counts , int32_t* ranks , int32_t* flag,
                       int S, int K, as_stream_t stream);
int as_mt_perm_ranks(int32_t* state , const int32_t* counts2 , int32_t* ranks , int32_t* flag,
                     int G, int K, as_stream_t stream);

int as_merge_plan(const uint8_t* keep, const uint8_t* link, int32_t* groups, int32_t* ngroups, int G, int P,
                  as_stream_t stream);

int as_semantic_prestage(const float* map_fg, float thr, int k, int G, int Hp, int Wp, int up, float* fg_inter,
                         uint8_t* mask, int32_t* counts, as_stream_t stream);

size_t as_cosine_shift_workspace_bytes(int B, int C, int Hp, int Wp, int G, int P);
int as_cosine_shift(const float* feat, const int32_t* box_patch, const int32_t* obj_img, const float* prot_in,
                    float* prot_out, double tau0, double temp, int n_shift, float* sim_out, int32_t* assign_out,
                    float* tau_out, void* ws, size_t ws_bytes, int B, int C, int Hp, int Wp, int G, int P,
                    as_stream_t stream);
int as_cosine_shift_strided(const float* feat, long long feat_batch_stride, const int32_t* box_patch, const int32_t* obj_img,
                            const float* prot_in, float* prot_out, double tau0, double temp, int n_shift, float* sim_out,
                            int32_t* assign_out, float* tau_out, void* ws, size_t ws_bytes, int B, int C, int Hp, int Wp, int G,
                            int P, as_stream_t stream);

size_t as_refine_similarity_workspace_bytes(int C, int Np, int Gp);
int as_refine_similarity(const float* feat, const float* seeds, const int32_t* boxes, int G, int Gp,
                         int refine_times, float tau, int n_select, float* maps, float* seeds_out, void* ws,
                         size_t ws_bytes, int C, int Hp, int Wp, as_stream_t stream);

size_t as_instance_maps_workspace_bytes(int L, int G);
int as_instance_maps(const float* sim_fg, const float* sim_bg, int L, int G, int Gp, int Hp, int Wp, int up,
                     float* map_fg, float* map_bg, void* ws, size_t ws_bytes, as_stream_t stream);

size_t as_crop_threshold_erode_workspace_bytes(int M, int H, int W);
int as_crop_threshold_erode(const float* maps , const int32_t* crops, float thr, int relative, int k,
                            uint8_t* mask , int32_t* counts , void* ws, size_t ws_bytes, int M, int H,
                            int W, as_stream_t stream);

int as_mask_count(const uint8_t* mask, int32_t* counts, int M, int HW, as_stream_t stream);

size_t as_rank_select_workspace_bytes(int M, int HW);
int as_rank_select(const uint8_t* mask , const int32_t* ranks , int32_t* out , void* ws,
                   size_t ws_bytes, int M, int HW, int K, as_stream_t stream);
int as_rank_select_xy(const uint8_t* mask , const int32_t* ranks , int64_t* out_xy , void* ws,
                      size_t ws_bytes, int M, int HW, int K, int W, int yx_order, as_stream_t stream);

int as_merge_parts(const float* prot, const uint8_t* keep, float thr, float* merged , int32_t* ngroups ,
                   int32_t* flag, int G, int P, int C, int slots, as_stream_t stream);

int as_select_median_boxes(const float* boxes , const int32_t* meta , int Lc, int stride,
                           const int64_t* pick_in, int64_t* pick , float* chosen , int32_t* map_idx , int32_t* box_patch ,
                           int32_t* box_int , const int32_t* status, int32_t* bad, int n, as_stream_t stream);

int as_rank_draw_xy(const uint8_t* mask , int mode, const float* u , int32_t* flag,
                    int64_t* out_xy , int64_t* patch_out , int patch_div, int patch_w, int64_t patch_base,
                    int row_rot, void* ws, size_t ws_bytes, int M, int HW, int K, int W, int yx_order, as_stream_t stream);

int as_small_attn_fwd(const void* qkv, void* out, float* lse, int Bp, int N, int h, int d, int dtype, as_stream_t stream);
size_t as_small_attn_bwd_workspace_bytes(int Bp, int N, int h);
int as_small_attn_bwd(const void* qkv, const void* out, const void* d_out, const float* lse, void* dqkv, void* workspace,
                      size_t workspace_bytes, int Bp, int N, int h, int d, int dtype, as_stream_t stream);

int as_roi_align_fwd(const float* feat, const float* rois, float* out, int B, int H, int W, int C, int R, int out_size,
                     float spatial_scale, int sampling_ratio, int aligned, as_stream_t stream);
int as_roi_align_bwd(const float* dout, const float* rois, float* dfeat, int B, int H, int W, int C, int R, int out_size,
                     float spatial_scale, int sampling_ratio, int aligned, as_stream_t stream);

int as_chamfer_2d_fwd(const float* xyz1, const float* xyz2, float* dist1, float* dist2, int32_t* idx1, int32_t* idx2,
                      int B, int n, int m, as_stream_t stream);
int as_chamfer_2d_bwd(const float* xyz1, const float* xyz2, const float* gdist1, const float* gdist2, const int32_t* idx1,
                      const int32_t* idx2, float* gxyz1, float* gxyz2, int B, int n, int m, as_stream_t stream);


size_t as_nms_workspace_bytes(int n);
int as_nms(const float* boxes_sorted, int n, float iou_thr, int max_keep, long long* keep_idx, int* count, void* workspace,
           size_t workspace_bytes, as_stream_t stream);

int as_paste_masks(const float* src, const long long* labels, const float* boxes, void* out, int n, int K, int h, int w,
                   int H, int W, int apply_sigmoid, int out_mode, float thr, as_stream_t stream);

int as_rle_tile(int* rows_per_segment, int* cols_per_workgroup);
size_t as_rle_workspace_bytes(int n, int H, int W);
int as_rle_count(const void* masks, int n, int H, int W, uint32_t* totals, void* workspace, size_t workspace_bytes,
                 as_stream_t stream);
int as_rle_encode(const void* masks, int n, int H, int W, const uint32_t* totals, void* workspace, size_t workspace_bytes,
                  uint32_t* pos, size_t pos_capacity, void* str, size_t str_capacity, unsigned long long* lens,
                  as_stream_t stream);

typedef struct {
  const float* cls;
  const float* reg;
  int H, W, stride_x, stride_y;
} as_rpn_level;
size_t as_rpn_candidates_workspace_bytes(int B, int C);
int as_rpn_candidates(const as_rpn_level* levels, int L, int B, int A, const float* base_anchors, const float* img_shapes,
                      int nms_pre, float min_bbox_size, const float* means_stds, float max_ratio, int C, float* cand_box,
                      float* cand_nms_box, float* cand_score, int32_t* cand_level, int32_t* cand_index, int32_t* cand_count,
                      void* workspace, size_t workspace_bytes, as_stream_t stream);

size_t as_rpn_assign_workspace_bytes(int B, int T, int sum_g);
int as_rpn_assign(const as_rpn_level* levels, int L, int B, int A, const float* base_anchors, const float* gt_boxes,
                  const int32_t* gt_offsets, int sum_g, int max_g, const int32_t* shapes, float pos_iou_thr, float neg_iou_thr,
                  float min_pos_iou, int match_low_quality, int allowed_border, int32_t* assigned, float* max_iou,
                  int32_t* counts, void* workspace, size_t workspace_bytes, as_stream_t stream);
int as_rpn_sample(int B, int T, int sum_g, int num, const int32_t* assigned, const int32_t* plan, const int32_t* ranks,
                  const void* workspace, size_t workspace_bytes, int32_t* inds, as_stream_t stream);
int as_rpn_targets(const as_rpn_level* levels, int L, int B, int A, const float* base_anchors, const float* gt_boxes,
                   const int32_t* gt_offsets, int sum_g, const int32_t* assigned, const int32_t* pos_inds, int inds_stride,
                   int num, const float* means_stds, int32_t* pos_gt, float* pos_delta, as_stream_t stream);

#ifdef __cplusplus
}
#endif
#endif
```

Before: 350.5.

## Fuse tap bf16 cast into add-layernorm and write rollout rows in place

The add-layernorm kernel now optionally writes a compute-dtype copy of the patch tokens for FPN taps, so the separate slice-and-cast before the deconv FPN branch goes away and that FPN branch can start right after the tap. Rollout gains a top-rows kernel that gathers selected point-token rows directly, plus strided step variants that write every layer's result into one preallocated [B, L, G, N] tensor, replacing per-layer allocations and stacking. This adds code paths and a new default (non-legacy) rollout route, which changes output layout and risks semantic mismatch with the old path.

```diff
diff --git a/attentionshift_amd/_lib.py b/attentionshift_amd/_lib.py
--- a/attentionshift_amd/_lib.py
+++ b/attentionshift_amd/_lib.py
@@ -32,6 +32,8 @@
     "as_add_layernorm_bwd": (_c_int, [_c_void_p] * 4 + [ctypes.c_float] + [_c_void_p] * 5 + [_c_size_t] + [_c_int] * 3 + [_c_void_p]),
     "as_add_layernorm": (_c_int, [_c_void_p] * 4 + [ctypes.c_float] + [_c_void_p] * 2 + [_c_int] * 3 + [_c_void_p]),
     "as_add_layernorm_scaled": (_c_int, [_c_void_p] * 4 + [ctypes.c_float] + [_c_void_p] * 2 + [_c_int] * 3 + [_c_void_p, _c_int, _c_void_p]),
+    "as_add_layernorm_tap": (_c_int, [_c_void_p] * 4 + [ctypes.c_float] + [_c_void_p] * 2 + [_c_int] * 3 + [_c_void_p, _c_int, _c_void_p]
+                             + [_c_int] * 2 + [_c_void_p]),
     "as_add_layernorm_bwd_scaled": (_c_int, [_c_void_p] * 4 + [ctypes.c_float] + [_c_void_p] * 5 + [_c_size_t] + [_c_int] * 3
                                     + [_c_void_p, _c_int, _c_void_p]),
     "as_linear_splitk_workspace_bytes": (ctypes.c_size_t, [_c_int] * 3),
@@ -51,6 +53,9 @@
     "as_rollout_top": (_c_int, [_c_void_p] * 5 + [_c_int] * 5 + [_c_void_p]),
     "as_rollout_step_workspace_bytes": (_c_size_t, [_c_int] * 3),
     "as_rollout_step": (_c_int, [_c_void_p] * 8 + [_c_size_t] + [_c_int] * 5 + [_c_void_p]),
+    "as_rollout_top_rows": (_c_int, [_c_void_p] * 5 + [ctypes.c_longlong, _c_void_p] + [_c_int] * 6 + [_c_void_p]),
+    "as_rollout_step_strided": (_c_int, [_c_void_p] * 4 + [ctypes.c_longlong] + [_c_void_p] * 2 + [ctypes.c_longlong]
+                                + [_c_void_p] * 2 + [_c_size_t] + [_c_int] * 5 + [_c_void_p]),
     "as_ccl_2d": (_c_int, [_c_void_p] * 2 + [_c_int] * 3 + [_c_void_p]),
     "as_cam_boxes_workspace_bytes": (_c_size_t, [_c_int] * 4),
     "as_cam_boxes": (_c_int, [_c_void_p] * 2 + [_c_float] * 2 + [_c_int] * 4 + [_c_void_p] * 5 + [_c_size_t, _c_void_p]),
diff --git a/attentionshift_amd/backbone.py b/attentionshift_amd/backbone.py
--- a/attentionshift_amd/backbone.py
+++ b/attentionshift_amd/backbone.py
@@ -132,6 +132,7 @@
         self.with_point_head = with_point_head
         self.compute_dtype = compute_dtype
         self.defer_fpn = bool(unused.pop("defer_fpn", False))
+        self.fuse_tap_cast = True
         self._fpn_stream = None
         self._point_pack = None
         self.point_head_stream = bool(unused.pop("point_head_stream", False))
@@ -275,12 +276,12 @@
             return y
         return op(feat_nchw)
 
-    def _fpn(self, i, feat_nchw, tok):
-        B, D, hp, wp = feat_nchw.shape
+    def _fpn(self, i, feat_nchw, tok, tok_cd=None, hw=None):
         ops_ = [self.fpn1, self.fpn2, self.fpn3, self.fpn4]
         op = ops_[i]
+        B, D, hp, wp = (tok.shape[0], tok.shape[2], *hw) if feat_nchw is None else feat_nchw.shape
         if isinstance(op, nn.Sequential) and isinstance(op[0], nn.ConvTranspose2d):
-            x0 = tok.to(self.compute_dtype).reshape(B, hp, wp, D)
+            x0 = (tok.to(self.compute_dtype) if tok_cd is None else tok_cd).reshape(B, hp, wp, D)
             if len(op) == 4:
                 bn = op[1]
                 if isinstance(bn, nn.modules.batchnorm._BatchNorm) and not bn.training and bn.running_mean is not None \
@@ -365,12 +366,12 @@
             self._wcache["token_table"] = hit
         return hit[1]
 
-    def _block(self, blk, x, delta, keep_state, need_x, on_full=None, full_out=None, x_out=None):
+    def _block(self, blk, x, delta, keep_state, need_x, on_full=None, full_out=None, x_out=None, tap_np=None):
         cd = self.compute_dtype
-        x, y = ops.add_layernorm(x, delta, blk.norm1.weight, blk.norm1.bias, blk.norm1.eps, cd,
-                                 x_out=full_out if delta is not None else None)
+        x, y, *tok_cd = ops.add_layernorm(x, delta, blk.norm1.weight, blk.norm1.bias, blk.norm1.eps, cd,
+                                          x_out=full_out if delta is not None else None, tap_np=tap_np)
         if on_full is not None:
-            on_full(x)
+            on_full(x, *tok_cd)
         a, st = ops.attention_fwd(y, self._w(blk.attn.qkv.weight),
                                   None if blk.attn.qkv.bias is None else blk.attn.qkv.bias.float(),
                                   self._w(blk.attn.proj.weight), blk.attn.proj.bias.float(), self.num_heads,
@@ -449,8 +450,14 @@
         if not grad_path:
             x = x.contiguous()
 
-        def take_tap(xf):
+        taps_cd = []
+        fpn_early = {}
+
+        def take_tap(xf, tok_cd=None):
             taps.append(xf[:, 1:-T])
+            taps_cd.append(tok_cd)
+            if tok_cd is not None:
+                fpn_early[len(taps) - 1] = self._fpn(len(taps) - 1, None, taps[-1], tok_cd, hw=(hp, wp))
             tap = xf[:, 1:, :][:, :-T].permute(0, 2, 1).unflatten(2, (hp, wp))
             if grad_path:
                 features.append(tap if os.environ.get("AS_TAP_VIEW", "1") != "0" else tap.contiguous())
@@ -465,6 +472,11 @@
             return store[0][k]
 
         tap_due = False
+        fpn_ops = [self.fpn1, self.fpn2, self.fpn3, self.fpn4] if self.with_fpn else []
+
+        def wants_cd(k):
+            return (self.fuse_tap_cast and k < len(fpn_ops) and not self.defer_fpn and self.compute_dtype != torch.float32
+                    and x.is_cuda and isinstance(fpn_ops[k], nn.Sequential) and isinstance(fpn_ops[k][0], nn.ConvTranspose2d))
         nblk = len(self.blocks)
         self._train_shadow = {}
         if grad_path and self.compute_dtype != torch.float32 and not os.environ.get("AS_NO_PARAM_SHADOW"):
@@ -493,7 +505,8 @@
                                            take_tap if tap_due else None,
                                            full_out=tap_slot(len(features)) if tap_due and x.dtype == torch.float32 else None,
                                            x_out=tap_slot(len(features) + int(tap_due)) if last_tap and x.dtype == torch.float32
-                                           else None)
+                                           else None,
+                                           tap_np=hp * wp if tap_due and wants_cd(len(features)) else None)
                 tap_due = i in self.out_indices and i != nblk - 1
                 if i in self.out_indices and i == nblk - 1:
                     take_tap(x)
@@ -510,7 +523,8 @@
         elif self.with_fpn and self.defer_fpn and x.is_cuda:
             features = DeferredFPN(self, features, taps)
         elif self.with_fpn:
-            features = [self._fpn(i, features[i], taps[i]) for i in range(len(features))]
+            features = [fpn_early[i] if i in fpn_early else self._fpn(i, features[i], taps[i], taps_cd[i])
+                        for i in range(len(features))]
         point_tokens = x[:, -T:]
         out = dict(org_feats=org_features, feature=features if isinstance(features, DeferredFPN) else tuple(features),
                    point_tokens=point_tokens)
diff --git a/attentionshift_amd/csrc/layernorm.hip b/attentionshift_amd/csrc/layernorm.hip
--- a/attentionshift_amd/csrc/layernorm.hip
+++ b/attentionshift_amd/csrc/layernorm.hip
@@ -6,11 +6,17 @@
 __global__ __launch_bounds__(256) void add_layernorm_kernel(const float* __restrict__ x_in, const T* __restrict__ delta,
                                                             const float* __restrict__ gamma, const float* __restrict__ beta,
                                                             float* __restrict__ x_out, T* __restrict__ y_out, int M, int D,
-                                                            float eps, const float* __restrict__ dscale, int rps) {
+                                                            float eps, const float* __restrict__ dscale, int rps,
+                                                            T* __restrict__ tap_out, int rpi, int Np) {
   const int row = blockIdx.x * 4 + (threadIdx.x >> 6), lane = threadIdx.x & 63;
   if (row >= M) return;
   const size_t base = (size_t)row * D;
   const float ds = dscale != nullptr ? dscale[row / rps] : 1.0f;
+  T* tap = nullptr;
+  if (tap_out != nullptr) {
+    const int n = row % rpi;
+    if (n >= 1 && n <= Np) tap = tap_out + ((size_t)(row / rpi) * Np + (n - 1)) * D;
+  }
   float v[VPL][4];
   float s = 0.0f;
 #pragma unroll
@@ -48,6 +54,16 @@
     const int c = (i * 64 + lane) * 4;
     if (c < D) {
       if (x_out != nullptr) *reinterpret_cast<float4*>(x_out + base + c) = make_float4(v[i][0], v[i][1], v[i][2], v[i][3]);
+      if (tap != nullptr) {
+        if constexpr (sizeof(T) == 2) {
+          bf16x4 w4;
+#pragma unroll
+          for (int t = 0; t < 4; ++t) w4[t] = (__bf16)v[i][t];
+          *reinterpret_cast<bf16x4*>(tap + c) = w4;
+        } else {
+          *reinterpret_cast<float4*>(tap + c) = make_float4(v[i][0], v[i][1], v[i][2], v[i][3]);
+        }
+      }
       if (y_out != nullptr) {
         const float4 g = *reinterpret_cast<const float4*>(gamma + c);
         const float4 b = *reinterpret_cast<const float4*>(beta + c);
@@ -62,12 +78,12 @@
 
 template <typename T>
 int launch_add_ln(const float* x_in, const void* delta, const float* gamma, const float* beta, float* x_out, void* y_out,
-                  int M, int D, float eps, const float* dscale, int rps, hipStream_t s) {
+                  int M, int D, float eps, const float* dscale, int rps, void* tap_out, int rpi, int Np, hipStream_t s) {
   const int vpl = as_ceil_div(D, 256);
   dim3 grid(as_ceil_div(M, 4));
 #define AS_LN(V)                                                                                                   \
   hipLaunchKernelGGL((add_layernorm_kernel<T, V>), grid, dim3(256), 0, s, x_in, (const T*)delta, gamma, beta, x_out, \
-                     (T*)y_out, M, D, eps, dscale, rps)
+                     (T*)y_out, M, D, eps, dscale, rps, (T*)tap_out, rpi, Np)
   switch (vpl) {
     case 1: AS_LN(1); break;
     case 2: AS_LN(2); break;
@@ -303,13 +319,26 @@
 extern "C" int as_add_layernorm_scaled(const float* x_in, const void* delta, const float* gamma, const float* beta, float eps,
                                        float* x_out, void* y_out, int M, int D, int dtype, const float* delta_scale,
                                        int rows_per_scale, as_stream_t stream) {
-  AS_REQUIRE(x_in && (x_out || y_out), AS_E_BADARG, "as_add_layernorm: null pointer");
+  return as_add_layernorm_tap(x_in, delta, gamma, beta, eps, x_out, y_out, M, D, dtype, delta_scale, rows_per_scale, nullptr, 1,
+                              0, stream);
+}
+
+extern "C" int as_add_layernorm_tap(const float* x_in, const void* delta, const float* gamma, const float* beta, float eps,
+                                    float* x_out, void* y_out, int M, int D, int dtype, const float* delta_scale,
+                                    int rows_per_scale, void* tap_out, int rows_per_image, int Np, as_stream_t stream) {
+  AS_REQUIRE(x_in && (x_out || y_out || tap_out), AS_E_BADARG, "as_add_layernorm: null pointer");
+  AS_REQUIRE(!tap_out || (rows_per_image > 0 && M % rows_per_image == 0 && Np > 0 && Np < rows_per_image), AS_E_BADARG,
+             "as_add_layernorm_tap: need M %% rows_per_image == 0 and 0 < Np < rows_per_image (M=%d rows_per_image=%d Np=%d)", M,
+             rows_per_image, Np);
   AS_REQUIRE(rows_per_scale > 0 && (!delta_scale || delta), AS_E_BADARG, "as_add_layernorm: delta_scale needs delta, rows_per_scale > 0");
   AS_REQUIRE(!y_out || (gamma && beta), AS_E_BADARG, "as_add_layernorm: y_out needs gamma and beta");
   AS_REQUIRE(M > 0 && D > 0 && D % 4 == 0, AS_E_BADARG, "as_add_layernorm: need M > 0 and D %% 4 == 0 (D=%d)", D);
   hipStream_t s = (hipStream_t)stream;
-  if (dtype == AS_BF16) return launch_add_ln<__bf16>(x_in, delta, gamma, beta, x_out, y_out, M, D, eps, delta_scale, rows_per_scale, s);
-  if (dtype == AS_F32) return launch_add_ln<float>(x_in, delta, gamma, beta, x_out, y_out, M, D, eps, delta_scale, rows_per_scale, s);
+  const int rpi = tap_out ? rows_per_image : 1;
+  if (dtype == AS_BF16)
+    return launch_add_ln<__bf16>(x_in, delta, gamma, beta, x_out, y_out, M, D, eps, delta_scale, rows_per_scale, tap_out, rpi, Np, s);
+  if (dtype == AS_F32)
+    return launch_add_ln<float>(x_in, delta, gamma, beta, x_out, y_out, M, D, eps, delta_scale, rows_per_scale, tap_out, rpi, Np, s);
   AS_REQUIRE(false, AS_E_UNSUPPORTED, "as_add_layernorm: dtype %d", dtype);
 }
 
diff --git a/attentionshift_amd/csrc/rollout.hip b/attentionshift_amd/csrc/rollout.hip
--- a/attentionshift_amd/csrc/rollout.hip
+++ b/attentionshift_amd/csrc/rollout.hip
@@ -59,7 +59,7 @@
 __global__ __launch_bounds__(RO_NT) void attn_mean_rows_kernel(const T* __restrict__ q, const T* __restrict__ k,
                                                                const float* __restrict__ lse,
                                                                float* __restrict__ out, T* __restrict__ rf_out, int B,
-                                                               int N, int Npad, int h, int row0, int nrows) {
+                                                               int N, int Npad, int h, int row0, int nrows, size_t out_bs) {
   const int lane = threadIdx.x & 63, wave = threadIdx.x >> 6;
   const int li = lane & 31, half = lane >> 5;
   const int jb = blockIdx.x * 4 + wave, ib = blockIdx.y, b = blockIdx.z;
@@ -74,8 +74,74 @@
     float v = p[r];
     if (TOP) v = 0.5f * (v + ((row0 + i) == j ? 1.0f : 0.0f));
     const bool live = i < nrows && j < N;
-    if (live) out[((size_t)b * nrows + i) * N + j] = v;
+    if (live) out[(size_t)b * out_bs + (size_t)i * N + j] = v;
     if (rf_out != nullptr && i < 128) rf_out[rf_slot(b, nkb, i, j)] = from_f32<T>(live ? v : 0.0f);
+  }
+}
+
+template <typename T>
+__global__ __launch_bounds__(RO_NT) void rollout_top_rows_kernel(const T* __restrict__ q, const T* __restrict__ k,
+                                                                 const float* __restrict__ lse, const long long* __restrict__ sel,
+                                                                 float* __restrict__ out, T* __restrict__ rf_out, int B, int N,
+                                                                 int Npad, int h, int Tp, int G, size_t out_bs) {
+  extern __shared__ __attribute__((aligned(16))) char smem[];
+  __shared__ int srow[32];
+  float* slab = reinterpret_cast<float*>(smem);
+  const int tid = threadIdx.x, lane = tid & 63, wave = tid >> 6;
+  const int li = lane & 31, half = lane >> 5;
+  const int j0 = blockIdx.x * 32, i0 = blockIdx.y * 32, b = blockIdx.z;
+  if (tid < 32) {
+    const long long t = sel[(size_t)b * G + min(i0 + tid, G - 1)];
+    srow[tid] = N - Tp + (int)(t < 0 ? 0 : (t > Tp - 1 ? Tp - 1 : t));
+  }
+  __syncthreads();
+  const int irow = srow[li];
+  const int jrow = min(j0 + li, N - 1);
+  int arow[16];
+#pragma unroll
+  for (int r = 0; r < 16; ++r) arow[r] = srow[acc_row(r, half)];
+  Frag<T> fa[4], fb[4], na[4], nb[4];
+  float lr[16], nl[16];
+  auto fetch = [&](int hh, Frag<T> (&a)[4], Frag<T> (&bb)[4], float (&l)[16]) {
+    const size_t bh = (size_t)b * h + min(hh, h - 1);
+#pragma unroll
+    for (int ks = 0; ks < 4; ++ks) {
+      a[ks].load16B(q + qf_frag(bh, Npad, irow, ks, half));
+      bb[ks].load16B(k + (bh * Npad + jrow) * HD + ks * 16 + half * 8);
+    }
+#pragma unroll
+    for (int r = 0; r < 16; ++r) l[r] = lse[bh * N + arow[r]];
+  };
+  if (wave < h) fetch(wave, fa, fb, lr);
+  for (int hh = wave; hh < h; hh += 4) {
+    if (hh + 4 < h) fetch(hh + 4, na, nb, nl);
+    f32x16 s;
+#pragma unroll
+    for (int r = 0; r < 16; ++r) s[r] = 0.0f;
+#pragma unroll
+    for (int ks = 0; ks < 4; ++ks) s = mma32(fa[ks], fb[ks], s);
+#pragma unroll
+    for (int r = 0; r < 16; ++r) slab[((size_t)hh * 16 + r) * 64 + lane] = __builtin_amdgcn_exp2f(s[r] - lr[r] * LOG2E);
+#pragma unroll
+    for (int ks = 0; ks < 4; ++ks) { fa[ks] = na[ks]; fb[ks] = nb[ks]; }
+#pragma unroll
+    for (int r = 0; r < 16; ++r) lr[r] = nl[r];
+  }
+  __syncthreads();
+  const float inv_h = 1.0f / (float)h;
+  const int j = j0 + li;
+  const int nkb = (N + 31) / 32;
+#pragma unroll
+  for (int x = 0; x < 4; ++x) {
+    const int r = wave * 4 + x;
+    float pbar = 0.0f;
+    for (int hh = 0; hh < h; ++hh) pbar += slab[((size_t)hh * 16 + r) * 64 + lane];
+    pbar *= inv_h;
+    const int il = acc_row(r, half), i = i0 + il;
+    const float v = 0.5f * (pbar + (srow[il] == j ? 1.0f : 0.0f));
+    const bool live = i < G && j < N;
+    if (live) out[(size_t)b * out_bs + (size_t)i * N + j] = v;
+    if (rf_out != nullptr) rf_out[rf_slot(b, nkb, i, j)] = from_f32<T>(live ? v : 0.0f);
   }
 }
 
@@ -93,7 +159,7 @@
                                                               const float* __restrict__ Rin, const T* __restrict__ rf_in,
                                                               float* __restrict__ Rout, T* __restrict__ rf_out,
                                                               float* __restrict__ part, int B, int N, int Npad, int h,
-                                                              int Trows, int nsplit, int xbufs) {
+                                                              int Trows, int nsplit, int xbufs, size_t rin_bs, size_t rout_bs) {
   extern __shared__ __attribute__((aligned(16))) char smem[];
   constexpr bool PREFETCH = sizeof(T) == 2;
   const int tid = threadIdx.x, lane = tid & 63, wave = tid >> 6;
@@ -221,9 +287,9 @@
       }
       float v = 0.0f;
       if (live) {
-        const size_t idx = ((size_t)b * Trows + i) * N + j;
-        v = 0.5f * (acc[r] + Rin[idx]);
-        Rout[idx] = v;
+        const size_t idx = (size_t)i * N + j;
+        v = 0.5f * (acc[r] + Rin[(size_t)b * rin_bs + idx]);
+        Rout[(size_t)b * rout_bs + idx] = v;
       }
       if (rf_out != nullptr) rf_out[rf_slot(b, nkb, i, j)] = from_f32<T>(v);
     }
@@ -262,7 +328,7 @@
                                                                  const float* __restrict__ Rin, const T* __restrict__ rf_in,
                                                                  float* __restrict__ Rout, T* __restrict__ rf_out,
                                                                  float* __restrict__ part, int B, int N, int Npad, int h,
-                                                                 int Trows, int nsplit) {
+                                                                 int Trows, int nsplit, size_t rin_bs, size_t rout_bs) {
   extern __shared__ __attribute__((aligned(16))) char smem[];
   const int tid = threadIdx.x, lane = tid & 63, wave = tid >> 6;
   const int li = lane & 31, half = lane >> 5;
@@ -385,9 +451,9 @@
       }
       float v = 0.0f;
       if (live) {
-        const size_t idx = ((size_t)b * Trows + i) * N + j;
-        v = 0.5f * (mine[r] + Rin[idx]);
-        Rout[idx] = v;
+        const size_t idx = (size_t)i * N + j;
+        v = 0.5f * (mine[r] + Rin[(size_t)b * rin_bs + idx]);
+        Rout[(size_t)b * rout_bs + idx] = v;
       }
       if (rf_out != nullptr) rf_out[rf_slot(b, nkb, i, j)] = from_f32<T>(v);
     }
@@ -604,7 +670,7 @@
 template <typename T>
 __global__ __launch_bounds__(64) void rollout_finish_kernel(const float* __restrict__ part, const float* __restrict__ Rin,
                                                             float* __restrict__ Rout, T* __restrict__ rf_out, int B, int N,
-                                                            int Trows, int nsplit) {
+                                                            int Trows, int nsplit, size_t rin_bs, size_t rout_bs) {
   const int nkb = (N + 31) / 32;
   const int j = blockIdx.x * 64 + threadIdx.x, i = blockIdx.y, b = blockIdx.z;
   if (j >= nkb * 32) return;
@@ -613,15 +679,17 @@
     const size_t idx = ((size_t)b * Trows + i) * N + j;
     float a = 0.0f;
     for (int sp = 0; sp < nsplit; ++sp) a += part[(size_t)sp * B * Trows * N + idx];
-    v = 0.5f * (a + Rin[idx]);
-    Rout[idx] = v;
+    const size_t off = (size_t)i * N + j;
+    v = 0.5f * (a + Rin[(size_t)b * rin_bs + off]);
+    Rout[(size_t)b * rout_bs + off] = v;
   }
   if (rf_out != nullptr) rf_out[rf_slot(b, nkb, i, j)] = from_f32<T>(v);
 }
 
 template <typename T>
 int launch_rollout_step2(const void* q, const void* k, const float* lse, const float* Rin, const void* rf_in, float* Rout,
-                         void* rf_out, float* part, int nsplit, int B, int N, int h, int Trows, hipStream_t s) {
+                         void* rf_out, float* part, int nsplit, int B, int N, int h, int Trows, size_t rin_bs, size_t rout_bs,
+                         hipStream_t s) {
   const int Npad = as_round_up(N, 64);
   const int hpw = as_ceil_div(h, 4);
   dim3 grid(as_ceil_div(N, 32), B, nsplit);
@@ -634,7 +702,7 @@
     (void)hipFuncSetAttribute((const void*)rollout_step2_kernel<T, HPW>, hipFuncAttributeMaxDynamicSharedMemorySize, \
                               (int)lds);                                                                       \
     hipLaunchKernelGGL((rollout_step2_kernel<T, HPW>), grid, dim3(RO_NT), lds, s, (const T*)q, (const T*)k, lse, Rin, \
-                       (const T*)rf_in, Rout, (T*)rf_out, part, B, N, Npad, h, Trows, nsplit, xbufs);          \
+                       (const T*)rf_in, Rout, (T*)rf_out, part, B, N, Npad, h, Trows, nsplit, xbufs, rin_bs, rout_bs); \
   } while (0)
   if (sizeof(T) == 2 && h % R4_HPG == 0 && part != nullptr && nsplit == R4_MAXPARTS && !rollout_force_v3()) {
     const int ng = h / R4_HPG;
@@ -652,7 +720,7 @@
     AS_CHECK_LAUNCH("rollout_step4");
     dim3 fg(as_ceil_div(as_ceil_div(N, 32) * 32, 64), as_round_up(Trows, 32), B);
     hipLaunchKernelGGL((rollout_finish_kernel<T>), fg, dim3(64), 0, s, (const float*)part, Rin, Rout, (T*)rf_out, B, N,
-                       Trows, ks * ng);
+                       Trows, ks * ng, rin_bs, rout_bs);
     AS_CHECK_LAUNCH("rollout_finish");
     return AS_OK;
   }
@@ -660,7 +728,7 @@
     const size_t lds3 = (size_t)h * 32 * Kj2<T>::PITCH;
     (void)hipFuncSetAttribute((const void*)rollout_step3_kernel<T>, hipFuncAttributeMaxDynamicSharedMemorySize, (int)lds3);
     hipLaunchKernelGGL((rollout_step3_kernel<T>), grid, dim3(RO_NT), lds3, s, (const T*)q, (const T*)k, lse, Rin,
-                       (const T*)rf_in, Rout, (T*)rf_out, part, B, N, Npad, h, Trows, nsplit);
+                       (const T*)rf_in, Rout, (T*)rf_out, part, B, N, Npad, h, Trows, nsplit, rin_bs, rout_bs);
   } else {
   switch (hpw) {
     case 1: AS_RO2(1); break;
@@ -675,7 +743,7 @@
   if (nsplit > 1) {
     dim3 fg(as_ceil_div(as_ceil_div(N, 32) * 32, 64), as_round_up(Trows, 32), B);
     hipLaunchKernelGGL((rollout_finish_kernel<T>), fg, dim3(64), 0, s, (const float*)part, Rin, Rout, (T*)rf_out, B, N,
-                       Trows, nsplit);
+                       Trows, nsplit, rin_bs, rout_bs);
     AS_CHECK_LAUNCH("rollout_finish");
   }
   return AS_OK;
@@ -690,16 +758,30 @@
 
 template <typename T>
 int launch_mean_rows(const void* q, const void* k, const float* lse, float* out, void* rf_out, int B, int N, int h,
-                     int row0, int nrows, bool top, hipStream_t s) {
+                     int row0, int nrows, bool top, size_t out_bs, hipStream_t s) {
   const int Npad = as_round_up(N, 64);
   dim3 grid(as_ceil_div(as_ceil_div(N, 32), 4), as_ceil_div(nrows, 32), B);
   if (top)
     hipLaunchKernelGGL((attn_mean_rows_kernel<T, true>), grid, dim3(RO_NT), 0, s, (const T*)q, (const T*)k, lse,
-                       out, (T*)rf_out, B, N, Npad, h, row0, nrows);
+                       out, (T*)rf_out, B, N, Npad, h, row0, nrows, out_bs);
   else
     hipLaunchKernelGGL((attn_mean_rows_kernel<T, false>), grid, dim3(RO_NT), 0, s, (const T*)q, (const T*)k, lse,
-                       out, (T*)rf_out, B, N, Npad, h, row0, nrows);
+                       out, (T*)rf_out, B, N, Npad, h, row0, nrows, out_bs);
   AS_CHECK_LAUNCH("attn_mean_rows");
+  return AS_OK;
+}
+
+template <typename T>
+int launch_top_rows(const void* q, const void* k, const float* lse, const long long* sel, float* out, void* rf_out, int B, int N,
+                    int h, int Tp, int G, size_t out_bs, hipStream_t s) {
+  const int Npad = as_round_up(N, 64);
+  const size_t lds = (size_t)h * 16 * 64 * sizeof(float);
+  AS_REQUIRE(lds <= 64 * 1024, AS_E_UNSUPPORTED, "as_rollout_top_rows: h=%d heads (max 16)", h);
+  dim3 grid(as_ceil_div(N, 32), as_ceil_div(G, 32), B);
+  (void)hipFuncSetAttribute((const void*)rollout_top_rows_kernel<T>, hipFuncAttributeMaxDynamicSharedMemorySize, (int)lds);
+  hipLaunchKernelGGL((rollout_top_rows_kernel<T>), grid, dim3(RO_NT), lds, s, (const T*)q, (const T*)k, lse, sel, out, (T*)rf_out,
+                     B, N, Npad, h, Tp, G, out_bs);
+  AS_CHECK_LAUNCH("rollout_top_rows");
   return AS_OK;
 }
 
@@ -716,18 +798,32 @@
   AS_REQUIRE(B > 0 && N > 0 && h > 0 && row0 >= 0 && nrows > 0 && row0 + nrows <= N, AS_E_BADARG,
              "as_attn_mean_rows: bad row range %d+%d of %d", row0, nrows, N);
   hipStream_t s = (hipStream_t)stream;
-  if (dtype == AS_BF16) return launch_mean_rows<__bf16>(q, k, lse, out, nullptr, B, N, h, row0, nrows, false, s);
-  if (dtype == AS_F32) return launch_mean_rows<float>(q, k, lse, out, nullptr, B, N, h, row0, nrows, false, s);
+  if (dtype == AS_BF16) return launch_mean_rows<__bf16>(q, k, lse, out, nullptr, B, N, h, row0, nrows, false, (size_t)nrows * N, s);
+  if (dtype == AS_F32) return launch_mean_rows<float>(q, k, lse, out, nullptr, B, N, h, row0, nrows, false, (size_t)nrows * N, s);
   AS_REQUIRE(false, AS_E_UNSUPPORTED, "as_attn_mean_rows: dtype %d", dtype);
 }
 
 extern "C" int as_rollout_top(const void* q, const void* k, const float* lse, float* R_out, void* rf_out, int B, int N,
                               int h, int T, int dtype, as_stream_t stream) {
+  return as_rollout_top_rows(q, k, lse, nullptr, R_out, (long long)T * N, rf_out, B, N, h, T, T, dtype, stream);
+}
+
+extern "C" int as_rollout_top_rows(const void* q, const void* k, const float* lse, const long long* rows, float* R_out,
+                                   long long r_out_stride, void* rf_out, int B, int N, int h, int T, int G, int dtype,
+                                   as_stream_t stream) {
   AS_REQUIRE(q && k && lse && R_out, AS_E_BADARG, "as_rollout_top: null pointer");
   AS_REQUIRE(B > 0 && h > 0 && T > 0 && T <= N && T <= 128, AS_E_BADARG, "as_rollout_top: bad sizes N=%d T=%d", N, T);
+  AS_REQUIRE(G > 0 && G <= 128 && (rows || G == T) && r_out_stride >= (long long)G * N, AS_E_BADARG,
+             "as_rollout_top_rows: bad selection G=%d (T=%d) or image stride %lld", G, T, r_out_stride);
   hipStream_t s = (hipStream_t)stream;
-  if (dtype == AS_BF16) return launch_mean_rows<__bf16>(q, k, lse, R_out, rf_out, B, N, h, N - T, T, true, s);
-  if (dtype == AS_F32) return launch_mean_rows<float>(q, k, lse, R_out, rf_out, B, N, h, N - T, T, true, s);
+  const size_t bs = (size_t)r_out_stride;
+  if (rows != nullptr) {
+    if (dtype == AS_BF16) return launch_top_rows<__bf16>(q, k, lse, rows, R_out, rf_out, B, N, h, T, G, bs, s);
+    if (dtype == AS_F32) return launch_top_rows<float>(q, k, lse, rows, R_out, rf_out, B, N, h, T, G, bs, s);
+  } else {
+    if (dtype == AS_BF16) return launch_mean_rows<__bf16>(q, k, lse, R_out, rf_out, B, N, h, N - T, T, true, bs, s);
+    if (dtype == AS_F32) return launch_mean_rows<float>(q, k, lse, R_out, rf_out, B, N, h, N - T, T, true, bs, s);
+  }
   AS_REQUIRE(false, AS_E_UNSUPPORTED, "as_rollout_top: dtype %d", dtype);
 }
 
@@ -764,8 +860,18 @@
 extern "C" int as_rollout_step(const void* q, const void* k, const float* lse, const float* R_in, const void* rf_in,
                                float* R_out, void* rf_out, void* workspace, size_t workspace_bytes, int B, int N, int h,
                                int T, int dtype, as_stream_t stream) {
+  return as_rollout_step_strided(q, k, lse, R_in, (long long)T * N, rf_in, R_out, (long long)T * N, rf_out, workspace,
+                                 workspace_bytes, B, N, h, T, dtype, stream);
+}
+
+extern "C" int as_rollout_step_strided(const void* q, const void* k, const float* lse, const float* R_in, long long r_in_stride,
+                                       const void* rf_in, float* R_out, long long r_out_stride, void* rf_out, void* workspace,
+                                       size_t workspace_bytes, int B, int N, int h, int T, int dtype, as_stream_t stream) {
   AS_REQUIRE(q && k && lse && R_in && rf_in && R_out && R_in != R_out && rf_in != rf_out, AS_E_BADARG,
              "as_rollout_step: null/aliased pointer");
+  AS_REQUIRE(r_in_stride >= (long long)T * N && r_out_stride >= (long long)T * N, AS_E_BADARG,
+             "as_rollout_step: image strides %lld / %lld below T * N", r_in_stride, r_out_stride);
+  const size_t rin_bs = (size_t)r_in_stride, rout_bs = (size_t)r_out_stride;
   AS_REQUIRE(B > 0 && h > 0 && h <= 16 && T > 0 && T <= N && T <= 128, AS_E_BADARG,
              "as_rollout_step: bad sizes N=%d T=%d h=%d", N, T, h);
   hipStream_t s = (hipStream_t)stream;
@@ -775,7 +881,8 @@
   const int ns = stream4 ? R4_MAXPARTS : (have_ws ? rollout_nsplit(B, N) : 1);
   float* part = ns > 1 ? (float*)workspace : nullptr;
   if (dtype == AS_BF16)
-    return launch_rollout_step2<__bf16>(q, k, lse, R_in, rf_in, R_out, rf_out, part, ns, B, N, h, T, s);
-  if (dtype == AS_F32) return launch_rollout_step2<float>(q, k, lse, R_in, rf_in, R_out, rf_out, part, ns, B, N, h, T, s);
+    return launch_rollout_step2<__bf16>(q, k, lse, R_in, rf_in, R_out, rf_out, part, ns, B, N, h, T, rin_bs, rout_bs, s);
+  if (dtype == AS_F32)
+    return launch_rollout_step2<float>(q, k, lse, R_in, rf_in, R_out, rf_out, part, ns, B, N, h, T, rin_bs, rout_bs, s);
   AS_REQUIRE(false, AS_E_UNSUPPORTED, "as_rollout_step: dtype %d", dtype);
 }
diff --git a/attentionshift_amd/ops.py b/attentionshift_amd/ops.py
--- a/attentionshift_amd/ops.py
+++ b/attentionshift_amd/ops.py
@@ -250,7 +250,7 @@
     return delta_scale, x.shape[1]
 
 
-def add_layernorm(x, delta, gamma, beta, eps, out_dtype, want_x=True, want_y=True, delta_scale=None, x_out=None):
+def add_layernorm(x, delta, gamma, beta, eps, out_dtype, want_x=True, want_y=True, delta_scale=None, x_out=None, tap_np=None):
     lib = _lib.load()
     D = x.shape[-1]
     x2 = x.reshape(-1, D)
@@ -269,9 +269,16 @@
     y = torch.empty(x2.shape, device=x.device, dtype=out_dtype) if want_y else None
     dt = AS_BF16 if out_dtype == torch.bfloat16 else AS_F32
     sc, rps = _scale_arg(delta_scale, x, delta)
+    xo = x if (delta is None or not want_x) else x_out.reshape(x.shape)
+    if tap_np is not None:
+        if x.dim() != 3 or not 0 < tap_np < x.shape[1]:
+            raise AttnShiftError("add_layernorm: tap_np needs x [B, N, D] with 0 < tap_np < N")
+        tap = torch.empty(x.shape[0], tap_np, D, device=x.device, dtype=out_dtype)
+        _lib.check(lib.as_add_layernorm_tap(_p(x2), _p(delta), _p(gamma), _p(beta), float(eps), _p(x_out), _p(y), x2.shape[0], D,
+                                            dt, _p(sc), rps, _p(tap), x.shape[1], tap_np, _stream()), "as_add_layernorm_tap")
+        return (xo if want_x else None), (None if y is None else y.reshape(x.shape)), tap
     _lib.check(lib.as_add_layernorm_scaled(_p(x2), _p(delta), _p(gamma), _p(beta), float(eps), _p(x_out), _p(y), x2.shape[0], D,
                                            dt, _p(sc), rps, _stream()), "as_add_layernorm")
-    xo = x if (delta is None or not want_x) else x_out.reshape(x.shape)
     return (xo if want_x else None), (None if y is None else y.reshape(x.shape))
 
 
@@ -486,12 +493,34 @@
     return out
 
 
-def rollout_rows(states, num_point_tokens, rows=None, use_workspace=True):
+def rollout_rows(states, num_point_tokens, rows=None, use_workspace=True, legacy=False):
     lib = _lib.load()
     top = states[-1]
     T = int(num_point_tokens)
     dev, dt = top.q.device, _dt(top.q)
     nbytes = lib.as_rollout_rfrag_bytes(top.B, top.N, dt)
+    if not legacy:
+        B, N, Lc = top.B, top.N, len(states)
+        if rows is not None:
+            if rows.dim() != 2 or rows.shape[0] != B or rows.shape[1] == 0:
+                raise AttnShiftError("rollout_rows: rows must be [B, G] with G > 0")
+            rows = rows.contiguous()
+            _chk(rows, dtype=torch.int64)
+        G = T if rows is None else rows.shape[1]
+        out = torch.empty(B, Lc, G, N, device=dev, dtype=torch.float32)
+        bs = Lc * G * N
+        rf = torch.empty(nbytes, device=dev, dtype=torch.uint8) if Lc > 1 else None
+        _lib.check(lib.as_rollout_top_rows(_p(top.q), _p(top.k), _p(top.lse), _p(rows), _p(out), bs, _p(rf), B, N, top.h, T, G,
+                                           dt, _stream()), "as_rollout_top_rows")
+        wbytes = lib.as_rollout_step_workspace_bytes(B, N, G) if (Lc > 1 and use_workspace) else 0
+        ws = torch.empty(wbytes, device=dev, dtype=torch.uint8) if wbytes else None
+        for n, st in enumerate(reversed(states[:-1])):
+            rfn = torch.empty_like(rf) if n + 2 < Lc else None
+            _lib.check(lib.as_rollout_step_strided(_p(st.q), _p(st.k), _p(st.lse), _p(out[:, n]), bs, _p(rf), _p(out[:, n + 1]), bs,
+                                                   _p(rfn), _p(ws), wbytes, st.B, st.N, st.h, G, dt, _stream()),
+                       "as_rollout_step_strided")
+            rf = rfn
+        return out
     outs = []
     R = torch.empty(top.B, T, top.N, device=dev, dtype=torch.float32)
     lower = list(reversed(states[:-1]))
diff --git a/include/attnshift.h b/include/attnshift.h
--- a/include/attnshift.h
+++ b/include/attnshift.h
@@ -72,6 +72,9 @@
 int as_add_layernorm_scaled(const float* x_in, const void* delta, const float* gamma, const float* beta, float eps,
                             float* x_out, void* y_out, int M, int D, int dtype, const float* delta_scale,
                             int rows_per_scale, as_stream_t stream);
+int as_add_layernorm_tap(const float* x_in, const void* delta, const float* gamma, const float* beta, float eps,
+                         float* x_out, void* y_out, int M, int D, int dtype, const float* delta_scale, int rows_per_scale,
+                         void* tap_out, int rows_per_image, int Np, as_stream_t stream);
 
 int as_linear_gelu_fwd(const void* x, const void* W, const float* bias, void* out, void* pre, int M, int Nout, int K,
                        int dtype, as_stream_t stream);
@@ -119,6 +122,12 @@
 int as_rollout_step(const void* q, const void* k, const float* lse, const float* R_in, const void* rf_in,
                     float* R_out, void* rf_out, void* workspace, size_t workspace_bytes, int B, int N, int h, int T,
                     int dtype, as_stream_t stream);
+int as_rollout_top_rows(const void* q, const void* k, const float* lse, const long long* rows, float* R_out,
+                        long long r_out_stride, void* rf_out, int B, int N, int h, int T, int G, int dtype,
+                        as_stream_t stream);
+int as_rollout_step_strided(const void* q, const void* k, const float* lse, const float* R_in, long long r_in_stride,
+                            const void* rf_in, float* R_out, long long r_out_stride, void* rf_out, void* workspace,
+                            size_t workspace_bytes, int B, int N, int h, int T, int dtype, as_stream_t stream);
 
 
 int as_ccl_2d(const uint8_t* img , int32_t* labels , int M, int H, int W,
```

After: 347.9. About the same (-0.7%).
